# DecaYale/SYN3R

Measured on AMD Instinct MI355X. Metric: llff_3view_train_loop_iters_per_sec, higher is better.
Workload: dtype f32 raster / f16 UNet (f32 accumulate); 1 GPU; LLFF fern-like 3-view block: 50 raster fwd+bwd iters (l1 loss) (200000 Gaussians, 1920x1080, SH3) + 1 SVD (step,pass): CFG UNet fwd [2,14,8,72,128] f16 + fused Euler step; frames=14, parallelism=scene-parallel x1

## Files before the change

include/syn3r_hip.h:

```cpp
#ifndef SYN3R_HIP_H
#define SYN3R_HIP_H

#include <stddef.h>
#include <stdint.h>

#ifdef __cplusplus
extern "C" {
#endif

#define SYN3R_OK 0
#define SYN3R_E_INVALID (-1)
#define SYN3R_E_WORKSPACE (-2)
#define SYN3R_E_HIP (-3)

#define SYN3R_F32 0
#define SYN3R_F16 1

const char* syn3r_last_error(void);
int syn3r_version(void);
const char* syn3r_arch(void);

int syn3r_trace_enable(int on);
void* syn3r_trace_session(void);
int syn3r_trace_attach(void* session);
int syn3r_trace_filter(const char* substrings);
int syn3r_trace_report(char* buf, size_t cap);


size_t syn3r_inverse_warp_workspace_bytes(int nb);
int syn3r_inverse_warp(const float* img, const float* depth, const float* depth_pseudo,
                       const float* pose12, const float* pose21, const float* K, const float* Kinv,
                       float bandwidth, int nb, int H, int W,
                       float* warped_img, float* warped_depth, uint8_t* mask_warp, uint8_t* mask_depth,
                       uint8_t* mask, float* warped_masked_img, uint8_t* mask_inv,
                       uint8_t* mask_depth_strict, uint8_t* mask_reproj, float* soft_mask_reproj,
                       float* reproj_error, void* workspace, size_t workspace_bytes, void* stream);

int syn3r_reproj_error(const float* depth1, const float* depth2, const float* T12, const float* T21,
                       const float* K1, const float* K1inv, const float* K2, int H, int W, float* err,
                       void* stream);

int syn3r_warp_post(const uint8_t* mask_reproj, const float* warped_img, const float* soft_mask_reproj,
                    int n, int H, int W, int h, int w, uint8_t* ero, float* cond_image, float* cond_ori,
                    float* soft, float* masks, float* soft_pool, void* stream);

int syn3r_fuse_uncertainty(const float* cond_ori, const float* gs_images, const float* soft, int n, int H, int W,
                           int h, int w, float* uncertainty, float* cond_image, float* masks, void* stream);

size_t syn3r_forward_warp_workspace_bytes(int H, int W);
int syn3r_forward_warp(const double* frame1, const uint8_t* mask1, const double* depth1, const double* T,
                       const double* K1inv, const double* K2, int H, int W, uint8_t* warped, uint8_t* mask2,
                       double* flow12, void* workspace, size_t workspace_bytes, void* stream);


size_t syn3r_step_workspace_bytes(int F, int C, int h, int w);
int syn3r_step_interp(const void* model_output, int vdtype, const void* sample, int sdtype,
                      const float* cond, const float* mask, const double* lambda_row, float sigma,
                      float dt, float c_out, float denom, float sqrt_sigma, float lr, int compute_grad,
                      void* prev_sample, float* pred_x0, float* grad, int F, int C, int h, int w,
                      void* workspace, size_t workspace_bytes, void* stream);

int syn3r_step_replace(const void* model_output, int vdtype, const void* sample, int sdtype,
                       const float* cond, const float* mask, const double* lambda_row, float sigma,
                       float dt, float c_out, float denom, void* prev_sample, float* pred_x0,
                       int F, int C, int h, int w, void* workspace, size_t workspace_bytes, void* stream);

size_t syn3r_raster_geom_bytes(int N);
size_t syn3r_raster_image_bytes(int H, int W);
size_t syn3r_raster_binning_bytes(long long P);

int syn3r_raster_preprocess(int N, int sh_degree, int sh_coeffs, const float* means3D, const float* scales,
                            const float* rotations, const float* opacities, const float* shs,
                            const float* confidence, float scale_modifier, const float* viewmatrix,
                            const float* projmatrix, const float* campos, float tanfovx, float tanfovy, int H,
                            int W, int* radii, void* geom, size_t geom_bytes, long long* num_rendered_host,
                            void* stream);
int syn3r_raster_preprocess_raw(int N, int sh_degree, int sh_coeffs, const float* means3D, const float* log_scales,
                                const float* raw_rotations, const float* opacity_logits, const float* shs,
                                const float* confidence, float scale_modifier, const float* viewmatrix,
                                const float* projmatrix, const float* campos, float tanfovx, float tanfovy, int H,
                                int W, int* radii, void* geom, size_t geom_bytes, long long* num_rendered_host,
                                void* stream);

int syn3r_raster_render(int N, int H, int W, const float* bg, const int* radii, void* geom, size_t geom_bytes,
                        void* binning, size_t binning_bytes, void* image, size_t image_bytes, long long P,
                        float* out_color, float* out_depth, float* out_alpha, unsigned** point_list_out,
                        void* stream);

size_t syn3r_raster_backward_workspace_bytes(int N);
int syn3r_raster_backward(int N, int sh_degree, int sh_coeffs, long long P, const float* means3D,
                          const float* scales, const float* rotations, const float* opacities, const float* shs,
                          const float* confidence, float scale_modifier, const float* viewmatrix,
                          const float* projmatrix, const float* campos, float tanfovx, float tanfovy, int H, int W,
                          const float* bg, const int* radii, void* geom, size_t geom_bytes,
                          const unsigned* point_list, void* image, size_t image_bytes, const float* dL_dcolor,
                          const float* dL_ddepth, const float* dL_dalpha, float* dL_dmeans3D, float* dL_dscales,
                          float* dL_drotations, float* dL_dopacities, float* dL_dshs, float* dL_dmeans2D,
                          float* dL_dconfidence, void* workspace, size_t workspace_bytes, void* stream);
int syn3r_raster_backward_raw(int N, int sh_degree, int sh_coeffs, long long P, const float* means3D,
                              const float* log_scales, const float* raw_rotations, const float* opacity_logits,
                              const float* shs, const float* confidence, float scale_modifier, const float* viewmatrix,
                              const float* projmatrix, const float* campos, float tanfovx, float tanfovy, int H, int W,
                              const float* bg, const int* radii, void* geom, size_t geom_bytes,
                              const unsigned* point_list, void* image, size_t image_bytes, const float* dL_dcolor,
                              const float* dL_ddepth, const float* dL_dalpha, float* dL_dmeans3D, float* dL_dlog_scales,
                              float* dL_draw_rotations, float* dL_dopacity_logits, float* dL_dshs, float* dL_dmeans2D,
                              float* dL_dconfidence, void* workspace, size_t workspace_bytes, void* stream);

size_t syn3r_sort_pairs_workspace_bytes(long long n);
int syn3r_sort_pairs(unsigned long long* keys, unsigned* vals, unsigned long long* keys_tmp, unsigned* vals_tmp,
                     long long n, int nbits, void* workspace, size_t workspace_bytes, int* result_in_tmp,
                     void* stream);


int syn3r_gemm_f16(const void* A, long long lda, const void* W, void* out, long long ldc, const void* bias,
                   const void* rowvec, long long ldrv, int rows_per_vec, int rv_group_rows, const void* residual, long long ldr,
                   const void* aux, long long ldaux, float s_acc, float s_res, float s_aux, int M, int N, int K,
                   void* gn_partials, size_t gn_partials_bytes, int* gn_written, void* stream);

int syn3r_gemm_2src_supported(int M, int N, int K1, int K2, long long lda1, long long lda2);
int syn3r_gemm_2src_f16(const void* A1, long long lda1, int K1, const void* A2, long long lda2, int K2, const void* W,
                        void* out, long long ldc, const void* bias, int M, int N, void* gn_partials, size_t gn_partials_bytes,
                        int* gn_written, void* stream);

int syn3r_gemm_set_tile(int bm);

int syn3r_gemm_set_splitk_workspace(void* workspace, size_t bytes);

int syn3r_gemm_geglu_f16(const void* A, long long lda, const void* Wpacked, const void* bias_packed, void* out,
                         long long ldc, int M, int D, int K, void* stream);

size_t syn3r_feedforward_workspace_bytes(int M, int D);
int syn3r_feedforward_f16(const void* x, long long ldx, const void* w1_packed, const void* b1_packed, int D,
                          const void* w2, const void* b2, void* out, long long ldc, const void* residual,
                          long long ldr, const void* aux, long long ldaux, float s_acc, float s_res, float s_aux,
                          int M, int C_in, int C_out, void* workspace, size_t workspace_bytes, void* stream);

int syn3r_feedforward_p64_supported(int M, int D, int C_in);
int syn3r_feedforward_p64_f16(const void* x, long long ldx, const void* w1_packed64, const void* b1_packed64, int D,
                              const void* w2, const void* b2, void* out, long long ldc, const void* residual,
                              long long ldr, const void* aux, long long ldaux, float s_acc, float s_res, float s_aux,
                              int M, int C_in, int C_out, void* workspace, size_t workspace_bytes, void* stream);

int syn3r_feedforward_fused_f16(const void* x, long long ldx, const void* w1_chunked, const void* b1_chunked, int D,
                                const void* w2, const void* b2, void* out, long long ldc, const void* residual,
                                long long ldr, const void* aux, long long ldaux, float s_acc, float s_res, float s_aux,
                                int M, int C, void* stream);

int syn3r_feedforward_fused_ln_f16(const void* x, long long ldx, const void* ln_gamma, const void* ln_beta, float ln_eps,
                                   const void* w1_chunked, const void* b1_chunked, int D, const void* w2, const void* b2,
                                   void* out, long long ldc, const void* residual, long long ldr, const void* aux,
                                   long long ldaux, float s_acc, float s_res, float s_aux, int M, int C, void* stream);

int syn3r_feedforward_fused_addln_f16(const void* x, long long ldx, const void* addvec, int rows_per_vec, const void* ln_gamma,
                                      const void* ln_beta, float ln_eps, const void* w1_chunked, const void* b1_chunked, int D,
                                      const void* w2, const void* b2, void* out, long long ldc, const void* aux, long long ldaux,
                                      float s_acc, float s_res, float s_aux, int M, int C, void* stream);

int syn3r_layernorm_linear320_f16(const void* x, long long ldx, const void* ln_gamma, const void* ln_beta, float ln_eps,
                                  const void* W, void* out, long long ldc, int M, int N, int C, void* stream);

int syn3r_conv2d3x3_f16(const void* X, const void* W, void* out, long long ldc, const void* bias,
                        const void* rowvec, long long ldrv, int rows_per_vec, const void* residual, long long ldr,
                        float s_acc, float s_res, int NB, int Hi, int Wi, int Cin, int Cout, int stride, int upsample,
                        int pad_lo, void* gn_partials, size_t gn_partials_bytes, int* gn_written, void* stream);

int syn3r_tconv3_f16(const void* X, const void* W, void* out, long long ldc, const void* bias, const void* rowvec,
                     long long ldrv, int rows_per_vec, const void* residual, long long ldr, float s_acc, float s_res,
                     int B, int F, int HW, int Cin, int Cout, void* gn_partials, size_t gn_partials_bytes, int* gn_written,
                     void* stream);

int syn3r_attention_f16(const void* q, const void* k, const void* v, long long ld, void* out, long long ldo,
                        int nseq, int S, int heads, void* stream);

int syn3r_attention_temporal_f16(const void* q, const void* k, const void* v, long long ld, void* out,
                                 long long ldo, int B, int F, int HW, int heads, void* stream);

size_t syn3r_groupnorm_workspace_bytes(int samples, int rows);
int syn3r_groupnorm_f16(const void* x, void* y, int samples, int rows, int C, const void* gamma, const void* beta,
                        float eps, int silu, void* workspace, size_t workspace_bytes, void* stream);
int syn3r_groupnorm_2src_f16(const void* x1, int C1, const void* x2, int C2, void* y, int samples, int rows,
                             const void* gamma, const void* beta, float eps, int silu, void* workspace,
                             size_t workspace_bytes, void* stream);
size_t syn3r_gn_partials_bytes(int M, int N);
int syn3r_groupnorm_pre_f16(const void* x1, int C1, const void* part1, const void* x2, int C2, const void* part2, void* y,
                            int samples, int rows, const void* gamma, const void* beta, float eps, int silu,
                            void* workspace, size_t workspace_bytes, void* stream);

int syn3r_layernorm_f16(const void* x, void* y, void* xsum, const void* addvec, int rows_per_vec, long long M,
                        int C, const void* gamma, const void* beta, float eps, void* stream);

int syn3r_geglu_f16(const void* x, void* y, long long M, int D, void* stream);

int syn3r_softmax_rows_f16(const void* x, void* y, long long M, int N, long long ld, float scale, void* stream);

int syn3r_time_conv_out(const void* x, long long ldx, const float* w, const float* bias, float* out, int B, int F,
                        long long HW, void* stream);


size_t syn3r_l1_loss_workspace_bytes(long long n);
int syn3r_l1_loss(const float* image, const float* target, long long n, float weight, float* loss, void* ws,
                  size_t ws_bytes, void* stream);
int syn3r_l1_loss_backward(const float* image, const float* target, long long n, float weight,
                           const float* grad_loss, float* grad_image, void* stream);

int syn3r_image_mse(const float* image, const float* target, long long n, float* mse, void* ws, size_t ws_bytes,
                    void* stream);

size_t syn3r_photo_loss_workspace_bytes(int C, int H, int W);
int syn3r_photo_loss(const float* image, const float* target, int C, int H, int W, float lambda_dssim, float weight,
                     float* loss3, void* ws, size_t ws_bytes, void* stream);
int syn3r_photo_loss_backward(const float* image, const float* target, int C, int H, int W, float lambda_dssim,
                              float weight, const float* grad_loss, const void* ws, float* grad_image, void* stream);
int syn3r_photo_loss_step(const float* image, const float* target, int C, int H, int W, float lambda_dssim, float weight,
                          const float* grad_loss, float* loss3, float* grad_image, void* ws, size_t ws_bytes, void* stream);

#define SYN3R_DCORR_MIN 0
#define SYN3R_DCORR_A 1
#define SYN3R_DCORR_B 2
size_t syn3r_depth_corr_loss_workspace_bytes(long long n);
int syn3r_depth_corr_loss(const float* depth, const float* prior, long long n, float weight, float offset, int mode, float* parts,
                          void* ws, size_t ws_bytes, void* stream);
int syn3r_depth_corr_loss_backward(const float* depth, const float* prior, long long n, float weight, float offset, int mode,
                                   const float* grad_loss, const void* ws, size_t ws_bytes, float* grad_depth, void* stream);
int syn3r_depth_corr_loss_step(const float* depth, const float* prior, long long n, float weight, float offset, int mode,
                               const float* grad_loss, float* parts, float* grad_depth, void* ws, size_t ws_bytes, void* stream);

int syn3r_adam_step(float* param, const float* grad, float* exp_avg, float* exp_avg_sq, long long n, float lr,
                    float beta1, float beta2, float eps, int step, void* stream);
int syn3r_adam_step_multi(int count, float* const* params, const float* const* grads, float* const* exp_avgs,
                          float* const* exp_avg_sqs, const long long* numels, const float* lrs, float beta1, float beta2,
                          const float* epss, const int* steps, void* stream);

int syn3r_gaussian_activate(int N, const float* log_scales, const float* rotations, const float* opacity_logits, float* scales,
                            float* rotations_n, float* opacities, void* stream);
int syn3r_gaussian_activate_backward(int N, const float* rotations, const float* scales, const float* rotations_n,
                                     const float* opacities, const float* d_scales, const float* d_rotations_n,
                                     const float* d_opacities, float* d_log_scales, float* d_rotations, float* d_opacity_logits,
                                     void* stream);

int syn3r_densification_stats(int N, const int* radii, const float* viewspace_grad, float* grad_accum, float* denom,
                              float* max_radii, void* stream);

size_t syn3r_knn3_workspace_bytes(int n);
int syn3r_knn3_mean_dist2(const float* points, int n, float* out, void* ws, size_t ws_bytes, void* stream);

size_t syn3r_knn3_graph_workspace_bytes(int n);
int syn3r_knn3_graph(const float* points, int n, float* dist2, int* index, void* ws, size_t ws_bytes, void* stream);

size_t syn3r_gaussian_unpool_workspace_bytes(int n);
int syn3r_gaussian_unpool_count(const float* dist2, const float* log_scales, int n, float score_thresh, float log_scale_thresh,
                                int* count, void* ws, size_t ws_bytes, void* stream);
int syn3r_gaussian_unpool_emit(const float* xyz, const float* log_scales, const float* opacity_logits, const float* confidence,
                               const int* index, int n, int n_sources, int capacity, float* out_xyz, float* out_log_scales,
                               float* out_opacity_logits, float* out_rotations, float* out_confidence, const void* ws,
                               size_t ws_bytes, void* stream);

int syn3r_conv2d3x3_act_f16(const void* X, const void* W, void* out, const void* bias, int relu, const void* relu_mask,
                            int NB, int Hi, int Wi, int Cin, int Cout, void* stream);
int syn3r_lpips_image_f16(const float* img, int H, int W, void* out, void* stream);
int syn3r_lpips_image_bwd(const void* grad64, int H, int W, float loss_scale, float* d_img, void* stream);
int syn3r_maxpool2_f16(const void* x, int H, int W, int C, void* y, void* stream);
int syn3r_maxpool2_bwd_f16(const void* x, const void* gy, int H, int W, int C, void* gx, void* stream);
size_t syn3r_lpips_layer_workspace_bytes(long long P, int C);
int syn3r_lpips_layer_f16(const void* a, const void* b, const float* w, long long P, int C, int accumulate, float* value,
                          void* ws, size_t ws_bytes, void* stream);
int syn3r_lpips_layer_bwd_f16(const void* a, const void* b, const float* w, long long P, int C, float gscale, int accumulate,
                              void* grad_a, void* stream);
int syn3r_conv2d3x3_split_f16(const void* X, const void* W, void* out, long long ld_out, const void* bias, int relu, int split_out,
                              const void* relu_mask, long long ld_mask, int NB, int Hi, int Wi, int Cin, int Cout, void* stream);
int syn3r_lpips_image_split_f16(const float* img, int H, int W, void* out, void* stream);
int syn3r_maxpool2_split_f16(const void* x, int H, int W, int C, void* y, void* stream);
int syn3r_maxpool2_bwd_split_f16(const void* x, const void* gy, int H, int W, int C, void* gx, void* stream);
int syn3r_lpips_layer_split_f16(const void* a, const void* b, const float* w, long long P, int C, int accumulate, float* value,
                                void* ws, size_t ws_bytes, void* stream);
int syn3r_lpips_layer_bwd_split_f16(const void* a, const void* b, const float* w, long long P, int C, float gscale, int accumulate,
                                    void* grad_a, void* stream);

size_t syn3r_pcd_outlier_workspace_bytes(int n);
int syn3r_pcd_statistical_outlier(const double* points, int n, int nb_neighbors, double std_ratio, double* avg_dist,
                                  unsigned char* keep, double* stats, void* ws, size_t ws_bytes, void* stream);

int syn3r_flow_cycle_mask(const float* flow_fw, const float* flow_bw, int n, int H, int W, float thresh, float* mask, float* dist,
                          void* stream);

typedef struct syn3r_unet syn3r_unet;
int syn3r_unet_create(const char* weights_dir, const char* variant, syn3r_unet** out);
int syn3r_unet_destroy(syn3r_unet* unet);
size_t syn3r_unet_workspace_bytes(syn3r_unet* unet, int B, int F, int h, int w, int ehs_rows);
int syn3r_unet_forward(syn3r_unet* unet, const void* sample, double timestep, const void* encoder_hidden_states, int ehs_rows,
                       const float* added_time_ids, void* out, int B, int F, int h, int w, int ctx_group, void* workspace,
                       size_t workspace_bytes, void* stream);

#ifdef __cplusplus
}
#endif
#endif
```

syn3r_amd/_lib.py:

```python
from __future__ import annotations

import ctypes as C
from pathlib import Path

import torch

_LIB_PATH = Path(__file__).resolve().parent / "lib" / "libsyn3r_hip.so"
_lib = None

c_f = C.c_float
c_i = C.c_int
c_p = C.c_void_p
c_sz = C.c_size_t
c_ll = C.c_longlong
c_d = C.c_double

F32, F16 = 0, 1

SIGNATURES = {
    "syn3r_last_error": (C.c_char_p, []),
    "syn3r_version": (c_i, []),
    "syn3r_arch": (C.c_char_p, []),
    "syn3r_trace_enable": (c_i, [c_i]),
    "syn3r_trace_filter": (c_i, [C.c_char_p]),
    "syn3r_trace_report": (c_i, [C.c_char_p, c_sz]),
    "syn3r_trace_session": (c_p, []),
    "syn3r_trace_attach": (c_i, [c_p]),
    "syn3r_inverse_warp_workspace_bytes": (c_sz, [c_i]),
    "syn3r_inverse_warp": (c_i, [c_p, c_p, c_p, c_p, c_p, c_p, c_p, c_f, c_i, c_i, c_i,
                                 c_p, c_p, c_p, c_p, c_p, c_p, c_p, c_p, c_p, c_p, c_p, c_p, c_sz, c_p]),
    "syn3r_reproj_error": (c_i, [c_p, c_p, c_p, c_p, c_p, c_p, c_p, c_i, c_i, c_p, c_p]),
    "syn3r_warp_post": (c_i, [c_p, c_p, c_p, c_i, c_i, c_i, c_i, c_i, c_p, c_p, c_p, c_p, c_p, c_p, c_p]),
    "syn3r_fuse_uncertainty": (c_i, [c_p, c_p, c_p, c_i, c_i, c_i, c_i, c_i, c_p, c_p, c_p, c_p]),
    "syn3r_forward_warp_workspace_bytes": (c_sz, [c_i, c_i]),
    "syn3r_forward_warp": (c_i, [c_p, c_p, c_p, c_p, c_p, c_p, c_i, c_i, c_p, c_p, c_p, c_p, c_sz, c_p]),
    "syn3r_step_workspace_bytes": (c_sz, [c_i, c_i, c_i, c_i]),
    "syn3r_step_interp": (c_i, [c_p, c_i, c_p, c_i, c_p, c_p, c_p, c_f, c_f, c_f, c_f, c_f, c_f, c_i,
                                c_p, c_p, c_p, c_i, c_i, c_i, c_i, c_p, c_sz, c_p]),
    "syn3r_step_replace": (c_i, [c_p, c_i, c_p, c_i, c_p, c_p, c_p, c_f, c_f, c_f, c_f,
                                 c_p, c_p, c_i, c_i, c_i, c_i, c_p, c_sz, c_p]),
    "syn3r_raster_geom_bytes": (c_sz, [c_i]),
    "syn3r_raster_image_bytes": (c_sz, [c_i, c_i]),
    "syn3r_raster_binning_bytes": (c_sz, [c_ll]),
    "syn3r_raster_preprocess": (c_i, [c_i, c_i, c_i, c_p, c_p, c_p, c_p, c_p, c_p, c_f, c_p, c_p, c_p, c_f, c_f,
                                      c_i, c_i, c_p, c_p, c_sz, C.POINTER(c_ll), c_p]),
    "syn3r_raster_preprocess_raw": (c_i, [c_i, c_i, c_i, c_p, c_p, c_p, c_p, c_p, c_p, c_f, c_p, c_p, c_p, c_f, c_f,
                                          c_i, c_i, c_p, c_p, c_sz, C.POINTER(c_ll), c_p]),
    "syn3r_raster_render": (c_i, [c_i, c_i, c_i, c_p, c_p, c_p, c_sz, c_p, c_sz, c_p, c_sz, c_ll, c_p, c_p, c_p,
                                  C.POINTER(c_p), c_p]),
    "syn3r_raster_backward_workspace_bytes": (c_sz, [c_i]),
    "syn3r_raster_backward": (c_i, [c_i, c_i, c_i, c_ll, c_p, c_p, c_p, c_p, c_p, c_p, c_f, c_p, c_p, c_p, c_f, c_f,
                                    c_i, c_i, c_p, c_p, c_p, c_sz, c_p, c_p, c_sz, c_p, c_p, c_p, c_p, c_p, c_p, c_p,
                                    c_p, c_p, c_p, c_p, c_sz, c_p]),
    "syn3r_raster_backward_raw": (c_i, [c_i, c_i, c_i, c_ll, c_p, c_p, c_p, c_p, c_p, c_p, c_f, c_p, c_p, c_p, c_f, c_f,
                                        c_i, c_i, c_p, c_p, c_p, c_sz, c_p, c_p, c_sz, c_p, c_p, c_p, c_p, c_p, c_p, c_p,
                                        c_p, c_p, c_p, c_p, c_sz, c_p]),
    "syn3r_sort_pairs_workspace_bytes": (c_sz, [c_ll]),
    "syn3r_sort_pairs": (c_i, [c_p, c_p, c_p, c_p, c_ll, c_i, c_p, c_sz, C.POINTER(c_i), c_p]),
    "syn3r_gaussian_activate": (c_i, [c_i, c_p, c_p, c_p, c_p, c_p, c_p, c_p]),
    "syn3r_gaussian_activate_backward": (c_i, [c_i, c_p, c_p, c_p, c_p, c_p, c_p, c_p, c_p, c_p, c_p, c_p]),
    "syn3r_densification_stats": (c_i, [c_i, c_p, c_p, c_p, c_p, c_p, c_p]),
    "syn3r_gemm_f16": (c_i, [c_p, c_ll, c_p, c_p, c_ll, c_p, c_p, c_ll, c_i, c_i, c_p, c_ll, c_p, c_ll, c_f, c_f, c_f,
                             c_i, c_i, c_i, c_p, c_sz, C.POINTER(c_i), c_p]),
    "syn3r_gemm_set_tile": (c_i, [c_i]),
    "syn3r_gemm_geglu_f16": (c_i, [c_p, c_ll, c_p, c_p, c_p, c_ll, c_i, c_i, c_i, c_p]),
    "syn3r_feedforward_workspace_bytes": (c_sz, [c_i, c_i]),
    "syn3r_feedforward_f16": (c_i, [c_p, c_ll, c_p, c_p, c_i, c_p, c_p, c_p, c_ll, c_p, c_ll, c_p, c_ll, c_f, c_f, c_f,
                                    c_i, c_i, c_i, c_p, c_sz, c_p]),
    "syn3r_feedforward_p64_f16": (c_i, [c_p, c_ll, c_p, c_p, c_i, c_p, c_p, c_p, c_ll, c_p, c_ll, c_p, c_ll, c_f, c_f, c_f,
                                    c_i, c_i, c_i, c_p, c_sz, c_p]),
    "syn3r_feedforward_p64_supported": (c_i, [c_i, c_i, c_i]),
    "syn3r_feedforward_fused_f16": (c_i, [c_p, c_ll, c_p, c_p, c_i, c_p, c_p, c_p, c_ll, c_p, c_ll, c_p, c_ll, c_f, c_f, c_f,
                                          c_i, c_i, c_p]),
    "syn3r_feedforward_fused_ln_f16": (c_i, [c_p, c_ll, c_p, c_p, c_f, c_p, c_p, c_i, c_p, c_p, c_p, c_ll, c_p, c_ll, c_p, c_ll,
                                             c_f, c_f, c_f, c_i, c_i, c_p]),
    "syn3r_feedforward_fused_addln_f16": (c_i, [c_p, c_ll, c_p, c_i, c_p, c_p, c_f, c_p, c_p, c_i, c_p, c_p, c_p, c_ll, c_p, c_ll,
                                                c_f, c_f, c_f, c_i, c_i, c_p]),
    "syn3r_layernorm_linear320_f16": (c_i, [c_p, c_ll, c_p, c_p, c_f, c_p, c_p, c_ll, c_i, c_i, c_i, c_p]),
    "syn3r_conv2d3x3_f16": (c_i, [c_p, c_p, c_p, c_ll, c_p, c_p, c_ll, c_i, c_p, c_ll, c_f, c_f,
                                  c_i, c_i, c_i, c_i, c_i, c_i, c_i, c_i, c_p, c_sz, C.POINTER(c_i), c_p]),
    "syn3r_tconv3_f16": (c_i, [c_p, c_p, c_p, c_ll, c_p, c_p, c_ll, c_i, c_p, c_ll, c_f, c_f,
                               c_i, c_i, c_i, c_i, c_i, c_p, c_sz, C.POINTER(c_i), c_p]),
    "syn3r_attention_f16": (c_i, [c_p, c_p, c_p, c_ll, c_p, c_ll, c_i, c_i, c_i, c_p]),
    "syn3r_attention_temporal_f16": (c_i, [c_p, c_p, c_p, c_ll, c_p, c_ll, c_i, c_i, c_i, c_i, c_p]),
    "syn3r_groupnorm_workspace_bytes": (c_sz, [c_i, c_i]),
    "syn3r_groupnorm_f16": (c_i, [c_p, c_p, c_i, c_i, c_i, c_p, c_p, c_f, c_i, c_p, c_sz, c_p]),
    "syn3r_groupnorm_2src_f16": (c_i, [c_p, c_i, c_p, c_i, c_p, c_i, c_i, c_p, c_p, c_f, c_i, c_p, c_sz, c_p]),
    "syn3r_groupnorm_pre_f16": (c_i, [c_p, c_i, c_p, c_p, c_i, c_p, c_p, c_i, c_i, c_p, c_p, c_f, c_i, c_p, c_sz, c_p]),
    "syn3r_gn_partials_bytes": (c_sz, [c_i, c_i]),
    "syn3r_gemm_2src_supported": (c_i, [c_i, c_i, c_i, c_i, c_ll, c_ll]),
    "syn3r_gemm_2src_f16": (c_i, [c_p, c_ll, c_i, c_p, c_ll, c_i, c_p, c_p, c_ll, c_p, c_i, c_i, c_p, c_sz, C.POINTER(c_i), c_p]),
    "syn3r_layernorm_f16": (c_i, [c_p, c_p, c_p, c_p, c_i, c_ll, c_i, c_p, c_p, c_f, c_p]),
    "syn3r_geglu_f16": (c_i, [c_p, c_p, c_ll, c_i, c_p]),
    "syn3r_softmax_rows_f16": (c_i, [c_p, c_p, c_ll, c_i, c_ll, c_f, c_p]),
    "syn3r_time_conv_out": (c_i, [c_p, c_ll, c_p, c_p, c_p, c_i, c_i, c_ll, c_p]),
    "syn3r_l1_loss_workspace_bytes": (c_sz, [c_ll]),
    "syn3r_l1_loss": (c_i, [c_p, c_p, c_ll, c_f, c_p, c_p, c_sz, c_p]),
    "syn3r_l1_loss_backward": (c_i, [c_p, c_p, c_ll, c_f, c_p, c_p, c_p]),
    "syn3r_image_mse": (c_i, [c_p, c_p, c_ll, c_p, c_p, c_sz, c_p]),
    "syn3r_photo_loss_workspace_bytes": (c_sz, [c_i, c_i, c_i]),
    "syn3r_photo_loss": (c_i, [c_p, c_p, c_i, c_i, c_i, c_f, c_f, c_p, c_p, c_sz, c_p]),
    "syn3r_photo_loss_backward": (c_i, [c_p, c_p, c_i, c_i, c_i, c_f, c_f, c_p, c_p, c_p, c_p]),
    "syn3r_photo_loss_step": (c_i, [c_p, c_p, c_i, c_i, c_i, c_f, c_f, c_p, c_p, c_p, c_p, c_sz, c_p]),
    "syn3r_depth_corr_loss_workspace_bytes": (c_sz, [c_ll]),
    "syn3r_depth_corr_loss": (c_i, [c_p, c_p, c_ll, c_f, c_f, c_i, c_p, c_p, c_sz, c_p]),
    "syn3r_depth_corr_loss_backward": (c_i, [c_p, c_p, c_ll, c_f, c_f, c_i, c_p, c_p, c_sz, c_p, c_p]),
    "syn3r_depth_corr_loss_step": (c_i, [c_p, c_p, c_ll, c_f, c_f, c_i, c_p, c_p, c_p, c_p, c_sz, c_p]),
    "syn3r_adam_step": (c_i, [c_p, c_p, c_p, c_p, c_ll, c_f, c_f, c_f, c_f, c_i, c_p]),
    "syn3r_adam_step_multi": (c_i, [c_i, c_p, c_p, c_p, c_p, c_p, c_p, c_f, c_f, c_p, c_p, c_p]),
    "syn3r_knn3_workspace_bytes": (c_sz, [c_i]),
    "syn3r_knn3_mean_dist2": (c_i, [c_p, c_i, c_p, c_p, c_sz, c_p]),
    "syn3r_knn3_graph_workspace_bytes": (c_sz, [c_i]),
    "syn3r_knn3_graph": (c_i, [c_p, c_i, c_p, c_p, c_p, c_sz, c_p]),
    "syn3r_gaussian_unpool_workspace_bytes": (c_sz, [c_i]),
    "syn3r_gaussian_unpool_count": (c_i, [c_p, c_p, c_i, c_f, c_f, c_p, c_p, c_sz, c_p]),
    "syn3r_gaussian_unpool_emit": (c_i, [c_p, c_p, c_p, c_p, c_p, c_i, c_i, c_i, c_p, c_p, c_p, c_p, c_p, c_p, c_sz, c_p]),
    "syn3r_conv2d3x3_act_f16": (c_i, [c_p, c_p, c_p, c_p, c_i, c_p, c_i, c_i, c_i, c_i, c_i, c_p]),
    "syn3r_lpips_image_f16": (c_i, [c_p, c_i, c_i, c_p, c_p]),
    "syn3r_lpips_image_bwd": (c_i, [c_p, c_i, c_i, c_f, c_p, c_p]),
    "syn3r_maxpool2_f16": (c_i, [c_p, c_i, c_i, c_i, c_p, c_p]),
    "syn3r_maxpool2_bwd_f16": (c_i, [c_p, c_p, c_i, c_i, c_i, c_p, c_p]),
    "syn3r_lpips_layer_workspace_bytes": (c_sz, [c_ll, c_i]),
    "syn3r_lpips_layer_f16": (c_i, [c_p, c_p, c_p, c_ll, c_i, c_i, c_p, c_p, c_sz, c_p]),
    "syn3r_lpips_layer_bwd_f16": (c_i, [c_p, c_p, c_p, c_ll, c_i, c_f, c_i, c_p, c_p]),
    "syn3r_conv2d3x3_split_f16": (c_i, [c_p, c_p, c_p, c_ll, c_p, c_i, c_i, c_p, c_ll, c_i, c_i, c_i, c_i, c_i, c_p]),
    "syn3r_lpips_image_split_f16": (c_i, [c_p, c_i, c_i, c_p, c_p]),
    "syn3r_maxpool2_split_f16": (c_i, [c_p, c_i, c_i, c_i, c_p, c_p]),
    "syn3r_maxpool2_bwd_split_f16": (c_i, [c_p, c_p, c_i, c_i, c_i, c_p, c_p]),
    "syn3r_lpips_layer_split_f16": (c_i, [c_p, c_p, c_p, c_ll, c_i, c_i, c_p, c_p, c_sz, c_p]),
    "syn3r_lpips_layer_bwd_split_f16": (c_i, [c_p, c_p, c_p, c_ll, c_i, c_f, c_i, c_p, c_p]),
    "syn3r_pcd_outlier_workspace_bytes": (c_sz, [c_i]),
    "syn3r_pcd_statistical_outlier": (c_i, [c_p, c_i, c_i, c_d, c_p, c_p, c_p, c_p, c_sz, c_p]),
    "syn3r_flow_cycle_mask": (c_i, [c_p, c_p, c_i, c_i, c_i, c_f, c_p, c_p, c_p]),
    "syn3r_gemm_set_splitk_workspace": (c_i, [c_p, c_sz]),
    "syn3r_unet_create": (c_i, [C.c_char_p, C.c_char_p, C.POINTER(c_p)]),
    "syn3r_unet_destroy": (c_i, [c_p]),
    "syn3r_unet_workspace_bytes": (c_sz, [c_p, c_i, c_i, c_i, c_i, c_i]),
    "syn3r_unet_forward": (c_i, [c_p, c_p, c_d, c_p, c_i, c_p, c_p, c_i, c_i, c_i, c_i, c_i, c_p, c_sz, c_p]),
}


class Syn3rError(RuntimeError):
    pass


def lib_path() -> Path:
    return _LIB_PATH


def set_library_path(path) -> None:
    global _LIB_PATH
    if _lib is not None:
        raise Syn3rError("set_library_path() after the library was loaded")
    _LIB_PATH = Path(path).resolve()


def load():
    global _lib
    if _lib is not None:
        return _lib
    if not _LIB_PATH.exists():
        raise Syn3rError(
            f"{_LIB_PATH} is missing: build it with `python -m syn3r_amd.build` "
            "(there is no CPU fallback for the SYN3R hot path)")
    lib = C.CDLL(str(_LIB_PATH))
    for name, (res, args) in SIGNATURES.items():
        fn = getattr(lib, name)
        fn.restype = res
        fn.argtypes = args
    _lib = lib
    return lib


def check(rc: int, what: str) -> None:
    if rc != 0:
        msg = load().syn3r_last_error().decode("utf-8", "replace")
        raise Syn3rError(f"{what} failed (code {rc}): {msg}")


def require_gpu(*tensors: torch.Tensor) -> torch.device:
    dev = None
    for t in tensors:
        if t is None:
            continue
        if not t.is_cuda:
            raise Syn3rError("syn3r_amd HIP path needs tensors on a HIP device (no CPU fallback); "
                             f"got a tensor on {t.device}")
        if dev is None:
            dev = t.device
        elif t.device != dev:
            raise Syn3rError(f"tensors on different devices: {dev} vs {t.device}")
    if dev is None:
        raise Syn3rError("no tensors given")
    return dev


def ptr(t: torch.Tensor | None) -> int | None:
    if t is None:
        return None
    if not t.is_contiguous():
        raise Syn3rError("non-contiguous tensor passed to the C-ABI")
    return t.data_ptr()


def stream_ptr(dev: torch.device) -> int:
    return torch.cuda.current_stream(dev).cuda_stream


def dtype_tag(t: torch.Tensor) -> int:
    if t.dtype == torch.float16:
        return F16
    if t.dtype == torch.float32:
        return F32
    raise Syn3rError(f"unsupported dtype {t.dtype}")


def host_f32(values) -> "C.Array":
    flat = [float(v) for v in values]
    return (C.c_float * len(flat))(*flat)


def host_f64(values) -> "C.Array":
    flat = [float(v) for v in values]
    return (C.c_double * len(flat))(*flat)


_ws_cache: dict = {}


def workspace(dev: torch.device, nbytes: int, tag: str = "") -> torch.Tensor:
    key = (dev.index, torch.cuda.current_stream(dev).cuda_stream, tag)
    buf = _ws_cache.get(key)
    if buf is None or buf.numel() < nbytes:
        buf = torch.empty(max(int(nbytes), 256), dtype=torch.uint8, device=dev)
        _ws_cache[key] = buf
    return buf


_active_trace = None


def join_active_trace() -> None:
    load().syn3r_trace_attach(_active_trace)


class kernel_trace:

    def __init__(self, only: str = "", detail: bool = False):
        self.only = only
        self.detail = detail

    def __enter__(self):
        global _active_trace
        lib = load()
        lib.syn3r_trace_filter(self.only.encode())
        lib.syn3r_trace_enable(2 if self.detail else 1)
        _active_trace = lib.syn3r_trace_session()
        self.result = {}
        return self

    def __exit__(self, *exc):
        global _active_trace
        lib = load()
        _active_trace = None
        lib.syn3r_trace_enable(0)
        buf = C.create_string_buffer(1 << 18)
        lib.syn3r_trace_report(buf, len(buf))
        for line in buf.value.decode().splitlines():
            name, calls, ms = line.rsplit(" ", 2)
            self.result[name] = (int(calls), float(ms))
        return False
```

syn3r_amd/csrc/raster_bin.hip:

```cpp
#include "common.h"
#include "raster_common.h"

using namespace syn3r;

namespace syn3r {

size_t binning_bytes(long long P) {
    size_t n = (size_t)(P > 0 ? P : 1);
    return 2 * align256(n * 8) + 2 * align256(n * 4) + sort_scratch_bytes(n) + 256;
}

BinningState carve_binning(void* buf, long long P) {
    size_t n = (size_t)(P > 0 ? P : 1);
    char* p = (char*)buf;
    BinningState b;
    b.keys_a = (unsigned long long*)p; p += align256(n * 8);
    b.keys_b = (unsigned long long*)p; p += align256(n * 8);
    b.vals_a = (unsigned*)p; p += align256(n * 4);
    b.vals_b = (unsigned*)p; p += align256(n * 4);
    b.sort_scratch = p;
    return b;
}

}

namespace {

__global__ void __launch_bounds__(256) k_dup_tiles(int N, const unsigned* __restrict__ order,
                                                   const float* __restrict__ means2D, const int* __restrict__ radii,
                                                   const unsigned* __restrict__ offsets, int gx, int gy,
                                                   unsigned* __restrict__ keys, unsigned* __restrict__ vals,
                                                   unsigned cap, unsigned* __restrict__ header,
                                                   uint2* __restrict__ ranges, int tiles) {
    const int i = blockIdx.x * 256 + threadIdx.x;
    for (int t = i; t < tiles; t += gridDim.x * 256) ranges[t] = make_uint2(0u, 0u);
    const int lane = threadIdx.x & 63;
    const bool valid = i < N;
    unsigned id = valid ? order[i] : 0u;
    int r = valid ? radii[id] : 0;
    int x0 = 0, y0 = 0, x1 = 0, y1 = 0;
    if (r > 0) tile_rect(means2D[2 * (size_t)id], means2D[2 * (size_t)id + 1], r, gx, gy, x0, y0, x1, y1);
    const int w = x1 - x0;
    const unsigned cnt = (unsigned)(w * (y1 - y0));
    const unsigned incl = wave_scan_incl(cnt);
    const unsigned local = incl - cnt;
    const unsigned total = __shfl(incl, 63, 64);
    const int first = blockIdx.x * 256 + (threadIdx.x & ~63);
    const unsigned base = first < N ? offsets[first] : 0u;
    const float inv_w = w > 0 ? 1.0f / (float)w : 0.0f;
    for (unsigned t = 0; t < total; t += 64) {
        const unsigned p = t + lane;
        int j = 0;
#pragma unroll
        for (int step = 32; step > 0; step >>= 1) {
            unsigned lc = __shfl(local, j + step, 64);
            if (lc <= p) j += step;
        }
        const unsigned k = p - __shfl(local, j, 64);
        const int xj = __shfl(x0, j, 64), yj = __shfl(y0, j, 64), wj = __shfl(w, j, 64);
        const float iwj = __shfl(inv_w, j, 64);
        const unsigned idj = __shfl(id, j, 64);
        if (p < total) {
            const int ty = (int)(((float)k + 0.5f) * iwj);
            int tyc = ty;
            if ((unsigned)(tyc * wj) > k) --tyc;
            else if ((unsigned)((tyc + 1) * wj) <= k) ++tyc;
            const int tx = (int)k - tyc * wj;
            const unsigned o = base + p;
            if (o < cap) {
                keys[o] = (unsigned)((yj + tyc) * gx + xj + tx);
                vals[o] = idj;
            } else {
                header[1] = 1u;
            }
        }
    }
}

__global__ void __launch_bounds__(256) k_tile_ranges(long long P_cap, const unsigned* __restrict__ header,
                                                     const unsigned* __restrict__ keys,
                                                     uint2* __restrict__ ranges) {
    long long P = (long long)header[0];
    if (P > P_cap) P = P_cap;
    long long i = (long long)blockIdx.x * 256 + threadIdx.x;
    if (i >= P) return;
    unsigned cur = keys[i];
    if (i == 0) ranges[cur].x = 0;
    else {
        unsigned prev = keys[i - 1];
        if (cur != prev) {
            ranges[prev].y = (unsigned)i;
            ranges[cur].x = (unsigned)i;
        }
    }
    if (i == P - 1) ranges[cur].y = (unsigned)P;
}

constexpr int kBinThreads = 512;
constexpr int kOffThreads = 1024;
#ifndef SYN3R_MAX_SUPER
#define SYN3R_MAX_SUPER 512
#endif
constexpr int kMaxSuper = SYN3R_MAX_SUPER;

struct BinPlan { int ss, sgx, sgy, nsuper, rounds, nchunks; bool ok; };
inline BinPlan bin_plan(int N, int gx, int gy) {
    BinPlan b;
    for (b.ss = 0; b.ss <= 3; ++b.ss) {
        const int side = 1 << b.ss;
        b.sgx = (gx + side - 1) / side; b.sgy = (gy + side - 1) / side;
        b.nsuper = b.sgx * b.sgy;
        if (b.nsuper <= kMaxSuper) break;
    }
    if (b.ss > 3) b.ss = 3;
    b.ok = b.nsuper <= kMaxSuper;
    const int max_chunks = b.ok ? (int)(kBinCounters / (size_t)b.nsuper) : 1;
    const int units = (N + kBinThreads - 1) / kBinThreads;
    b.rounds = (units + max_chunks - 1) / max_chunks;
    if (b.rounds < 1) b.rounds = 1;
    b.nchunks = (units + b.rounds - 1) / b.rounds;
    return b;
}

inline bool hier_binning(int N, int gx, int gy) {
    static const int on = tune_env("SYN3R_BIN_HIER", 1);
    return on != 0 && bin_plan(N, gx, gy).ok;
}

struct BinRect { int x0, y0, x1, y1; };
__device__ __forceinline__ BinRect bin_rect(int i, int N, const float* __restrict__ means2D, const int* __restrict__ radii, int gx, int gy) {
    BinRect r; r.x0 = r.y0 = r.x1 = r.y1 = 0;
    if (i < N) {
        const int rad = radii[i];
        if (rad > 0) tile_rect(means2D[2 * (size_t)i], means2D[2 * (size_t)i + 1], rad, gx, gy, r.x0, r.y0, r.x1, r.y1);
    }
    return r;
}
__device__ __forceinline__ unsigned short clip_rect(const BinRect& q, int sx, int sy, int ss) {
    const int bx = sx << ss, by = sy << ss, side = 1 << ss;
    const int rx0 = max(q.x0 - bx, 0), rx1 = min(q.x1 - bx, side), ry0 = max(q.y0 - by, 0), ry1 = min(q.y1 - by, side);
    return (unsigned short)(rx0 | (rx1 << 4) | (ry0 << 8) | (ry1 << 12));
}

__global__ void __launch_bounds__(kBinThreads) k_super_count(int N, const float* __restrict__ means2D, const int* __restrict__ radii,
                                                             int gx, int gy, int ss, int sgx, int nsuper, int rounds, int nchunks,
                                                             unsigned* __restrict__ counters, unsigned* __restrict__ header) {
    __shared__ unsigned tot[kMaxSuper];
    for (int s = threadIdx.x; s < nsuper; s += kBinThreads) tot[s] = 0u;
    __syncthreads();
    int pairs = 0;
    for (int r = 0; r < rounds; ++r) {
        const int i = (blockIdx.x * rounds + r) * kBinThreads + threadIdx.x;
        const BinRect q = bin_rect(i, N, means2D, radii, gx, gy);
        if (q.x1 > q.x0 && q.y1 > q.y0) {
            pairs += (q.x1 - q.x0) * (q.y1 - q.y0);
            const int side1 = (1 << ss) - 1, sx0 = q.x0 >> ss, sx1 = (q.x1 + side1) >> ss, sy0 = q.y0 >> ss, sy1 = (q.y1 + side1) >> ss;
            for (int sy = sy0; sy < sy1; ++sy)
                for (int sx = sx0; sx < sx1; ++sx) atomicAdd(&tot[sy * sgx + sx], 1u);
        }
    }
    __syncthreads();
    for (int s = threadIdx.x; s < nsuper; s += kBinThreads) counters[(size_t)blockIdx.x * nsuper + s] = tot[s];
    __shared__ unsigned pairs_s;
    if (threadIdx.x == 0) pairs_s = 0u;
    __syncthreads();
    pairs = wave_sum_i(pairs);
    if ((threadIdx.x & 63) == 0 && pairs) atomicAdd(&pairs_s, (unsigned)pairs);
    __syncthreads();
    if (threadIdx.x == 0 && pairs_s) atomicAdd(&header[3], pairs_s);
}

__global__ void __launch_bounds__(kBinThreads) k_super_append(int N, const float* __restrict__ depths, const float* __restrict__ means2D,
                                                              const int* __restrict__ radii, int gx, int gy, int ss, int sgx, int nsuper,
                                                              int rounds, int nchunks, const unsigned* __restrict__ counters,
                                                              unsigned* __restrict__ sstart, unsigned cap,
                                                              unsigned long long* __restrict__ skeys, unsigned* __restrict__ header) {
    __shared__ unsigned run[kMaxSuper];
    __shared__ unsigned tot_s[kMaxSuper], pre_s[kMaxSuper];
    __shared__ unsigned part_tot[kMaxSuper > kBinThreads ? kMaxSuper : kBinThreads], part_pre[kMaxSuper > kBinThreads ? kMaxSuper : kBinThreads];
    const int lane = threadIdx.x & 63, wv = threadIdx.x >> 6;
    {
        const int PARTS = max(1, min(8, kBinThreads / nsuper));
        const int per = (nchunks + PARTS - 1) / PARTS;
        for (int w = threadIdx.x; w < nsuper * PARTS; w += kBinThreads) {
            const int s_ = w % nsuper, part = w / nsuper;
            const int c0 = part * per, c1 = min(nchunks, c0 + per);
            unsigned tot = 0, pre = 0;
            constexpr int UN = 32;
            for (int cb = c0; cb < c1; cb += UN) {
                unsigned c[UN];
#pragma unroll
                for (int u = 0; u < UN; ++u) c[u] = cb + u < c1 ? counters[(size_t)(cb + u) * nsuper + s_] : 0u;
#pragma unroll
                for (int u = 0; u < UN; ++u) { tot += c[u]; pre += cb + u < (int)blockIdx.x ? c[u] : 0u; }
            }
            part_tot[w] = tot; part_pre[w] = pre;
        }
        __syncthreads();
        for (int s_ = threadIdx.x; s_ < nsuper; s_ += kBinThreads) {
            unsigned tot = 0, pre = 0;
            for (int k = 0; k < PARTS; ++k) { tot += part_tot[k * nsuper + s_]; pre += part_pre[k * nsuper + s_]; }
            tot_s[s_] = tot; pre_s[s_] = pre;
        }
        __syncthreads();
        if (wv == 0) {
            constexpr int PER = kMaxSuper / 64;
            unsigned c[PER], sum = 0;
#pragma unroll
            for (int k = 0; k < PER; ++k) { const int s_ = lane * PER + k; c[k] = s_ < nsuper ? tot_s[s_] : 0u; sum += c[k]; }
            const unsigned incl = wave_scan_incl(sum);
            unsigned ex = incl - sum;
#pragma unroll
            for (int k = 0; k < PER; ++k) {
                const int s_ = lane * PER + k;
                if (s_ < nsuper) {
                    run[s_] = ex + pre_s[s_];
                    if (blockIdx.x == 0) sstart[s_] = ex;
                }
                ex += c[k];
            }
            if (blockIdx.x == 0 && lane == 63) { sstart[nsuper] = incl; header[2] = incl; }
        }
        __syncthreads();
    }
    for (int r = 0; r < rounds; ++r) {
        const int i = (blockIdx.x * rounds + r) * kBinThreads + threadIdx.x;
        const BinRect q = bin_rect(i, N, means2D, radii, gx, gy);
        if (q.x1 > q.x0 && q.y1 > q.y0) {
            const unsigned long long key = ((unsigned long long)__float_as_uint(depths[i]) << 32) | (unsigned)i;
            const int side1 = (1 << ss) - 1, sx0 = q.x0 >> ss, sx1 = (q.x1 + side1) >> ss, sy0 = q.y0 >> ss, sy1 = (q.y1 + side1) >> ss;
            for (int sy = sy0; sy < sy1; ++sy)
                for (int sx = sx0; sx < sx1; ++sx) {
                    const unsigned o = atomicAdd(&run[sy * sgx + sx], 1u);
                    if (o < cap) skeys[o] = key;
                    else header[1] = 1u;
                }
        }
    }
}

__device__ __forceinline__ void super_range(int s, const unsigned* __restrict__ sstart, unsigned cap, unsigned& b, unsigned& e) {
    b = min(sstart[s], cap); e = min(sstart[s + 1], cap);
}

constexpr int kSortLds = 4096;
constexpr int kSuperSortThreads = 1024;
__device__ __forceinline__ void cmpx(unsigned long long& a, unsigned long long& b) { if (a > b) { const unsigned long long t = a; a = b; b = t; } }
__device__ __forceinline__ int pair_lo(int t, int j) { return (t << 1) - (t & (j - 1)); }
__device__ __forceinline__ void bitonic_dists(unsigned long long* buf, int m, int j) {
    for (; j >= 2; j >>= 2) {
        const int jh = j >> 1;
        for (int t = threadIdx.x; t < (m >> 2); t += kSuperSortThreads) {
            const int e0 = pair_lo(pair_lo(t, jh), j);
            unsigned long long a = buf[e0], b = buf[e0 + jh], c = buf[e0 + j], d = buf[e0 + j + jh];
            cmpx(a, c); cmpx(b, d);
            cmpx(a, b); cmpx(c, d);
            buf[e0] = a; buf[e0 + jh] = b; buf[e0 + j] = c; buf[e0 + j + jh] = d;
        }
        __syncthreads();
    }
    if (j == 1) {
        for (int t = threadIdx.x; t < (m >> 1); t += kSuperSortThreads) cmpx(buf[2 * t], buf[2 * t + 1]);
        __syncthreads();
    }
}
__device__ __forceinline__ void bitonic_merge(unsigned long long* buf, int m, int k) {
    if (k == 2) {
        for (int t = threadIdx.x; t < (m >> 1); t += kSuperSortThreads) cmpx(buf[2 * t], buf[2 * t + 1]);
        __syncthreads();
        return;
    }
    const int q = k >> 2;
    for (int t = threadIdx.x; t < (m >> 2); t += kSuperSortThreads) {
        const int off = t & (q - 1), blk = (t - off) << 2;
        const int ia = blk + off, ib = ia + q, ird = blk + (k - 1 - off), irc = ird - q;
        unsigned long long a = buf[ia], b = buf[ib], c = buf[irc], d = buf[ird];
        cmpx(a, d); cmpx(b, c);
        cmpx(a, b); cmpx(c, d);
        buf[ia] = a; buf[ib] = b; buf[irc] = c; buf[ird] = d;
    }
    __syncthreads();
    bitonic_dists(buf, m, q >> 1);
}

__device__ __forceinline__ bool rect_has(unsigned r, int rx, int ry) {
    return rx >= (int)(r & 15u) && rx < (int)((r >> 4) & 15u) && ry >= (int)((r >> 8) & 15u) && ry < (int)(r >> 12);
}

constexpr int kBinUnroll = 8;
__device__ __forceinline__ void tile_quarter(unsigned b, unsigned e, int q, unsigned& qb, unsigned& qe) {
    const unsigned len = (e - b + 3u) / 4u;
    qb = min(e, b + (unsigned)q * len); qe = min(e, qb + len);
}

__device__ __forceinline__ void super_tile_counts(int sx, int sy, int ss, int gx, int gy, unsigned n, const unsigned short* srect_b,
                                                  unsigned* __restrict__ tcount) {
    const int lane = threadIdx.x & 63, wv = threadIdx.x >> 6, side = 1 << ss;
    const unsigned len = (n + 3u) / 4u;
    for (int it = wv; it < side * side * 4; it += kSuperSortThreads / 64) {
        const int ti = it >> 2, q = it & 3;
        const int rx = ti & (side - 1), ry = ti >> ss;
        const int tx = (sx << ss) + rx, ty = (sy << ss) + ry;
        if (tx >= gx || ty >= gy) continue;
        const unsigned lo = min(n, (unsigned)q * len), hi = min(n, lo + len);
        unsigned cnt = 0;
        for (unsigned i0 = lo; i0 < hi; i0 += 256) {
            unsigned short r[4];
#pragma unroll
            for (int u = 0; u < 4; ++u) r[u] = srect_b[min(i0 + u * 64 + lane, hi - 1u)];
#pragma unroll
            for (int u = 0; u < 4; ++u) cnt += (i0 + u * 64 + lane < hi && rect_has(r[u], rx, ry)) ? 1u : 0u;
        }
#pragma unroll
        for (int o = 32; o > 0; o >>= 1) cnt += __shfl_xor(cnt, o, 64);
        if (lane == 0) tcount[4 * ((size_t)ty * gx + tx) + q] = cnt;
    }
}

__global__ void __launch_bounds__(kSuperSortThreads, 8) k_super_sort(int N, const float* __restrict__ means2D, const int* __restrict__ radii,
                                                                  int gx, int gy, int ss, int sgx, const unsigned* __restrict__ sstart, unsigned cap,
                                                                  unsigned long long* __restrict__ skeys, unsigned* __restrict__ sid,
                                                                  unsigned short* __restrict__ srect, unsigned* __restrict__ tcount) {
    extern __shared__ __attribute__((aligned(16))) unsigned long long sk[];
    const int s_ = blockIdx.x, sx = s_ % sgx, sy = s_ / sgx;
    unsigned b, e;
    super_range(s_, sstart, cap, b, e);
    const int n = (int)(e - b);
    if (n == 0) { super_tile_counts(sx, sy, ss, gx, gy, 0u, srect, tcount); return; }
    unsigned long long* gk = skeys + b;
    const unsigned long long INF = ~0ull;
    int m = 1;
    while (m < n) m <<= 1;
    const unsigned long long* sorted;
    if (m <= kSortLds) {
        for (int i = threadIdx.x; i < m; i += kSuperSortThreads) sk[i] = i < n ? gk[i] : INF;
        __syncthreads();
        for (int k = 2; k <= m; k <<= 1) bitonic_merge(sk, m, k);
        sorted = sk;
    } else {
        for (int p0 = 0; p0 < n; p0 += kSortLds) {
            for (int i = threadIdx.x; i < kSortLds; i += kSuperSortThreads) sk[i] = p0 + i < n ? gk[p0 + i] : INF;
            __syncthreads();
            for (int k = 2; k <= kSortLds; k <<= 1) bitonic_merge(sk, kSortLds, k);
            for (int i = threadIdx.x; i < kSortLds; i += kSuperSortThreads) if (p0 + i < n) gk[p0 + i] = sk[i];
            __syncthreads();
        }
        for (int k = kSortLds << 1; k <= m; k <<= 1) {
            const int h = k >> 1;
            for (int t = threadIdx.x; t < (m >> 1); t += kSuperSortThreads) {
                const int off = t & (h - 1), l = pair_lo(t, h), r = l - off + (k - 1 - off);
                if (r < n) { unsigned long long a = gk[l], c = gk[r]; if (a > c) { gk[l] = c; gk[r] = a; } }
            }
            __syncthreads();
            for (int j = k >> 2; j >= kSortLds; j >>= 1) {
                for (int t = threadIdx.x; t < (m >> 1); t += kSuperSortThreads) {
                    const int l = pair_lo(t, j), r = l + j;
                    if (r < n) { unsigned long long a = gk[l], c = gk[r]; if (a > c) { gk[l] = c; gk[r] = a; } }
                }
                __syncthreads();
            }
            for (int p0 = 0; p0 < n; p0 += kSortLds) {
                for (int i = threadIdx.x; i < kSortLds; i += kSuperSortThreads) sk[i] = p0 + i < n ? gk[p0 + i] : INF;
                __syncthreads();
                bitonic_dists(sk, kSortLds, kSortLds >> 1);
                for (int i = threadIdx.x; i < kSortLds; i += kSuperSortThreads) if (p0 + i < n) gk[p0 + i] = sk[i];
                __syncthreads();
            }
        }
        sorted = gk;
    }
    if (sorted == sk) {
        unsigned short clip[kSortLds / kSuperSortThreads];
#pragma unroll
        for (int u = 0; u < kSortLds / kSuperSortThreads; ++u) {
            const int i = threadIdx.x + u * kSuperSortThreads;
            clip[u] = 0;
            if (i < n) {
                const unsigned id = (unsigned)sk[i];
                const BinRect q = bin_rect((int)id, N, means2D, radii, gx, gy);
                clip[u] = clip_rect(q, sx, sy, ss);
                sid[b + i] = id;
                srect[b + i] = clip[u];
            }
        }
        __syncthreads();
        unsigned short* sr = (unsigned short*)sk;
#pragma unroll
        for (int u = 0; u < kSortLds / kSuperSortThreads; ++u) {
            const int i = threadIdx.x + u * kSuperSortThreads;
            if (i < n) sr[i] = clip[u];
        }
        __syncthreads();
        super_tile_counts(sx, sy, ss, gx, gy, (unsigned)n, sr, tcount);
        return;
    }
    for (int i = threadIdx.x; i < n; i += kSuperSortThreads) {
        const unsigned id = (unsigned)sorted[i];
        const BinRect q = bin_rect((int)id, N, means2D, radii, gx, gy);
        sid[b + i] = id;
        srect[b + i] = clip_rect(q, sx, sy, ss);
    }
    __syncthreads();
    super_tile_counts(sx, sy, ss, gx, gy, (unsigned)n, srect + b, tcount);
}

__global__ void __launch_bounds__(kOffThreads) k_tile_offsets(int tiles, const unsigned* __restrict__ tcount, unsigned cap,
                                                              uint2* __restrict__ ranges, unsigned* __restrict__ header,
                                                              unsigned* __restrict__ tile_order) {
    __shared__ unsigned smem[kOffThreads / 64 + 1];
    __shared__ unsigned bh[256];
    if (tile_order) { for (int k = threadIdx.x; k < 256; k += kOffThreads) bh[k] = 0u; __syncthreads(); }
    constexpr int PER = 8;
    unsigned carry = 0;
    for (int start = 0; start < tiles; start += kOffThreads * PER) {
        const int t0 = start + threadIdx.x * PER;
        unsigned c[PER], sum = 0;
#pragma unroll
        for (int k = 0; k < PER; ++k) {
            c[k] = 0u;
            if (t0 + k < tiles) { const uint4 q4 = ((const uint4*)tcount)[t0 + k]; c[k] = (q4.x + q4.y) + (q4.z + q4.w); }
            sum += c[k];
        }
        unsigned total;
        unsigned ex = block_exclusive_scan<kOffThreads / 64>(sum, smem, total) + carry;
#pragma unroll
        for (int k = 0; k < PER; ++k) {
            if (t0 + k < tiles) ranges[t0 + k] = c[k] ? make_uint2(min(ex, cap), min(ex + c[k], cap)) : make_uint2(0u, 0u);
            if (tile_order && t0 + k < tiles) atomicAdd(&bh[255u - min(255u, c[k] >> 5)], 1u);
            ex += c[k];
        }
        carry += total;
    }
    if (tile_order) {
        __syncthreads();
        if (threadIdx.x < 64) {
            const int l = threadIdx.x;
            unsigned c[4], sum = 0;
#pragma unroll
            for (int k = 0; k < 4; ++k) { c[k] = bh[4 * l + k]; sum += c[k]; }
            unsigned ex = wave_scan_incl(sum) - sum;
#pragma unroll
            for (int k = 0; k < 4; ++k) { bh[4 * l + k] = ex; ex += c[k]; }
        }
        __syncthreads();
        for (int t = threadIdx.x; t < tiles; t += kOffThreads) {
            const uint4 q4 = ((const uint4*)tcount)[t];
            const unsigned c = (q4.x + q4.y) + (q4.z + q4.w);
            tile_order[atomicAdd(&bh[255u - min(255u, c >> 5)], 1u)] = (unsigned)t;
        }
    }
    if (threadIdx.x == 0) {
        const bool over = carry > cap || header[2] > cap;
        header[0] = over ? max(carry, max(header[3], header[2])) : carry;
        if (over) header[1] = 1u;
    }
}

__global__ void __launch_bounds__(256) k_tile_write(int gx, int tiles, int ss, int sgx, const unsigned* __restrict__ sstart, unsigned cap,
                                                    const unsigned* __restrict__ sid, const unsigned short* __restrict__ srect,
                                                    const uint2* __restrict__ ranges, const unsigned* __restrict__ tcount,
                                                    unsigned* __restrict__ point_list) {
    const int t = blockIdx.x, q = threadIdx.x >> 6, lane = threadIdx.x & 63;
    const int tx = t % gx, ty = t / gx;
    unsigned b, e;
    super_range((ty >> ss) * sgx + (tx >> ss), sstart, cap, b, e);
    tile_quarter(b, e, q, b, e);
    const int rx = tx & ((1 << ss) - 1), ry = ty & ((1 << ss) - 1);
    const unsigned long long lt = (1ull << lane) - 1ull;
    const uint4 q4 = ((const uint4*)tcount)[t];
    unsigned pos = ranges[t].x + (q > 0 ? q4.x : 0u) + (q > 1 ? q4.y : 0u) + (q > 2 ? q4.z : 0u);
    for (unsigned i0 = b; i0 < e; i0 += 64 * kBinUnroll) {
        unsigned short r[kBinUnroll];
        unsigned id[kBinUnroll];
#pragma unroll
        for (int u = 0; u < kBinUnroll; ++u) {
            const unsigned i = i0 + u * 64 + lane;
            r[u] = i < e ? srect[i] : (unsigned short)0;
            id[u] = i < e ? sid[i] : 0u;
        }
#pragma unroll
        for (int u = 0; u < kBinUnroll; ++u) {
            const bool hit = rect_has(r[u], rx, ry);
            const unsigned long long m = __ballot(hit);
            if (hit) {
                const unsigned o = pos + (unsigned)__popcll(m & lt);
                if (o < cap) point_list[o] = id[u];
            }
            pos += (unsigned)__popcll(m);
        }
    }
}

int bits_for(unsigned v) { int b = 0; while (v) { ++b; v >>= 1; } return b; }

}

namespace syn3r {

bool raster_tiles_ordered(int N, int gx, int gy) {
    static const int order_env = tune_env("SYN3R_TILE_ORDER", 1);
    return order_env != 0 && hier_binning(N, gx, gy);
}

int raster_bin_prepare(const GeomState& g, int N, int gx, int gy, bool want_count, hipStream_t stream) {
    if (!hier_binning(N, gx, gy)) {
        int in_b = 0;
        int rc = argsort_depth_u32(g.dkeys_a, g.order_a, g.dkeys_b, g.order_b, (size_t)N, g.sort_scratch, stream, &in_b);
        if (rc) return rc;
        if ((in_b ? g.order_b : g.order_a) != g.order) { set_error("raster_preprocess: unexpected argsort parity"); return SYN3R_E_INVALID; }
        return exclusive_scan_u32(g.tiles_touched, g.point_offsets, (size_t)N, g.header, g.scan_scratch, stream, g.order);
    }
    if (want_count) return exclusive_scan_u32(g.tiles_touched, g.point_offsets, (size_t)N, g.header, g.scan_scratch, stream);
    return SYN3R_OK;
}

int raster_bin_lists(const GeomState& g, const ImageState& im, const BinningState& bn, const int* radii, int N, int gx, int gy,
                     long long P, hipStream_t stream, unsigned** point_list_out, const unsigned** tile_order_out) {
    const size_t tiles = (size_t)gx * gy;
    unsigned* point_list = bn.vals_a;
    unsigned* tile_order = nullptr;
    if (P == 0) {
        if (int rc = check_hip(hipMemsetAsync(im.ranges, 0, tiles * 8, stream), "memset ranges")) return rc;
    } else if (hier_binning(N, gx, gy)) {
        SYN3R_REQUIRE(P < (1ll << 30), "raster_render: pair capacity %lld: the super-tile sort indexes a list with 31-bit integers (2^30 pairs at most)", P);
        const BinPlan bp = bin_plan(N, gx, gy);
        unsigned* counters = im.bin_counters;
        unsigned* sid = bn.vals_b;
        unsigned short* srect = (unsigned short*)bn.keys_a;
        unsigned* sstart = counters + kBinCounters;
        unsigned long long* skeys = bn.keys_b;
        static DevOnce once;
        if (int rc = set_max_lds(once, (const void*)k_super_sort, kSortLds * 8, "hipFuncSetAttribute(super_sort)")) return rc;
        SYN3R_LAUNCH(k_super_count, dim3(bp.nchunks), dim3(kBinThreads), 0, stream, N, (const float*)g.means2D, radii, gx, gy, bp.ss, bp.sgx,
                     bp.nsuper, bp.rounds, bp.nchunks, counters, g.header);
        SYN3R_LAUNCH(k_super_append, dim3(bp.nchunks), dim3(kBinThreads), 0, stream, N, (const float*)g.depths, (const float*)g.means2D, radii,
                     gx, gy, bp.ss, bp.sgx, bp.nsuper, bp.rounds, bp.nchunks, (const unsigned*)counters, sstart, (unsigned)P, skeys, g.header);
        SYN3R_LAUNCH(k_super_sort, dim3(bp.nsuper), dim3(kSuperSortThreads), kSortLds * 8, stream, N, (const float*)g.means2D, radii, gx, gy,
                     bp.ss, bp.sgx, (const unsigned*)sstart, (unsigned)P, skeys, sid, srect, im.tile_counts);
        if (raster_tiles_ordered(N, gx, gy)) tile_order = im.tile_order;
        SYN3R_LAUNCH(k_tile_offsets, dim3(1), dim3(kOffThreads), 0, stream, (int)tiles, (const unsigned*)im.tile_counts, (unsigned)P,
                     im.ranges, g.header, tile_order);
        SYN3R_LAUNCH(k_tile_write, dim3((unsigned)tiles), dim3(256), 0, stream, gx, (int)tiles, bp.ss, bp.sgx,
                     (const unsigned*)sstart, (unsigned)P, (const unsigned*)sid, (const unsigned short*)srect,
                     (const uint2*)im.ranges, (const unsigned*)im.tile_counts, point_list);
    } else {
        unsigned* tk_a = (unsigned*)bn.keys_a;
        unsigned* tk_b = (unsigned*)bn.keys_b;
        SYN3R_LAUNCH(k_dup_tiles, dim3(ceil_div(N, 256)), dim3(256), 0, stream, N, g.order, g.means2D, radii,
                           g.point_offsets, gx, gy, tk_a, bn.vals_a, (unsigned)P, g.header, im.ranges, (int)tiles);
        int in_b = 0;
        int rc = sort_pairs_by_tile_u32(tk_a, bn.vals_a, tk_b, bn.vals_b, (size_t)P, bits_for((unsigned)tiles - 1),
                                        bn.sort_scratch, stream, &in_b, g.header);
        if (rc) return rc;
        const unsigned* keys = in_b ? tk_b : tk_a;
        point_list = in_b ? bn.vals_b : bn.vals_a;
        SYN3R_LAUNCH(k_tile_ranges, dim3(ceil_div(P, 256)), dim3(256), 0, stream, P, g.header, keys, im.ranges);
    }
    *point_list_out = point_list;
    *tile_order_out = tile_order;
    return SYN3R_OK;
}

}
```

syn3r_amd/csrc/raster_common.h:

```cpp
#pragma once
#include <hip/hip_runtime.h>
#include <stdint.h>
#include <stddef.h>

namespace syn3r {

constexpr int kTileX = 16;
constexpr int kTileY = 16;
constexpr int kTilePix = kTileX * kTileY;
constexpr float kNearClip = 0.2f;
constexpr float kFovGuard = 1.3f;
constexpr float kLowPass = 0.3f;
constexpr float kAlphaMin = 1.0f / 255.0f;
constexpr float kAlphaMax = 0.99f;
constexpr float kTransmittanceMin = 1e-4f;
constexpr float kLog2e = 1.4426950408889634f;

struct alignas(16) Splat {
    float x, y;
    float cxx, cxy, cyy;
    float opacity;
    float r, g, b;
    float depth;
    float pad0, pad1;
};
static_assert(sizeof(Splat) == 48, "Splat must be 48 bytes");

struct GeomState {
    unsigned* header;
    float* depths;
    float* means2D;
    float* cov3D;
    float* conic_opacity;
    float* rgb;
    unsigned* clamped;
    unsigned* tiles_touched;
    unsigned* point_offsets;
    Splat* splats;
    unsigned* dkeys_a;
    unsigned* dkeys_b;
    unsigned* order_a;
    unsigned* order_b;
    unsigned* order;
    void* sort_scratch;
    void* scan_scratch;
};

#ifndef SYN3R_BIN_COUNTERS
#define SYN3R_BIN_COUNTERS 65536
#endif
constexpr size_t kBinCounters = SYN3R_BIN_COUNTERS;
constexpr size_t kMaxSuperSlots = 4096;
struct ImageState {
    uint2* ranges;
    unsigned* n_contrib;
    float* final_T;
    unsigned* tile_counts;
    unsigned* bin_counters;
    unsigned* tile_order;
};

struct BinningState {
    unsigned long long* keys_a;
    unsigned long long* keys_b;
    unsigned* vals_a;
    unsigned* vals_b;
    void* sort_scratch;
};

inline size_t align256(size_t x) { return (x + 255) & ~(size_t)255; }

size_t scan_scratch_bytes(size_t n);
size_t sort_scratch_bytes(size_t n);
int exclusive_scan_u32(const unsigned* in, unsigned* out, size_t n, unsigned* total_out, void* scratch,
                       hipStream_t stream, const unsigned* perm = nullptr);
int argsort_depth_u32(unsigned* keys_a, unsigned* vals_a, unsigned* keys_b, unsigned* vals_b, size_t n, void* scratch,
                      hipStream_t stream, int* result_in_b);
int sort_pairs_by_tile_u32(unsigned* keys_a, unsigned* vals_a, unsigned* keys_b, unsigned* vals_b, size_t n, int nbits,
                           void* scratch, hipStream_t stream, int* result_in_b, const unsigned* n_dev);
int radix_sort_pairs(unsigned long long* keys_a, unsigned* vals_a, unsigned long long* keys_b, unsigned* vals_b,
                     size_t n, int nbits, void* scratch, hipStream_t stream, int* result_in_b,
                     const unsigned* n_dev = nullptr);

struct Camera {
    float view[16];
    float proj[16];
    float campos[3];
    float tanfovx, tanfovy, focal_x, focal_y;
    int H, W, grid_x, grid_y;
};

size_t geom_bytes(int N);
bool raster_tiles_ordered(int N, int gx, int gy);
size_t image_bytes(int H, int W);
size_t binning_bytes(long long P);
GeomState carve_geom(void* buf, int N);
void raster_fill_camera(Camera& cam, const float* view, const float* proj, const float* campos, float tanfovx, float tanfovy, int H, int W);
ImageState carve_image(void* buf, int H, int W);
BinningState carve_binning(void* buf, long long P);

int raster_bin_prepare(const GeomState& g, int N, int gx, int gy, bool want_count, hipStream_t stream);
int raster_bin_lists(const GeomState& g, const ImageState& im, const BinningState& bn, const int* radii, int N, int gx, int gy,
                     long long P, hipStream_t stream, unsigned** point_list, const unsigned** tile_order);

#ifdef __HIPCC__
__device__ __forceinline__ bool splat_reaches_rect(float mx, float my, float A, float B, float C, float op, float x0,
                                                   float x1, float y0, float y1) {
    if (!(A > 0.0f && C > 0.0f)) return true;
    const float thr = 2.0f * __logf(255.0f * op);
    const float dx0 = x0 - mx, dx1 = x1 - mx, dy0 = y0 - my, dy1 = y1 - my;
    const bool inx = dx0 <= 0.0f && dx1 >= 0.0f, iny = dy0 <= 0.0f && dy1 >= 0.0f;
    float qmin = 0.0f;
    if (!(inx && iny)) {
        qmin = 3.0e38f;
        if (!inx) {
            const float dx = dx0 > 0.0f ? dx0 : dx1;
            const float dy = fminf(fmaxf(-B * dx / C, dy0), dy1);
            qmin = A * dx * dx + 2.0f * B * dx * dy + C * dy * dy;
        }
        if (!iny) {
            const float dy = dy0 > 0.0f ? dy0 : dy1;
            const float dx = fminf(fmaxf(-B * dy / A, dx0), dx1);
            qmin = fminf(qmin, A * dx * dx + 2.0f * B * dx * dy + C * dy * dy);
        }
    }
    return qmin <= thr + (1.0e-3f + 1.0e-4f * thr);
}

__device__ __forceinline__ void tile_rect(float px, float py, int radius, int gx, int gy, int& x0, int& y0, int& x1,
                                          int& y1) {
    x0 = min(gx, max(0, (int)((px - radius) / kTileX)));
    y0 = min(gy, max(0, (int)((py - radius) / kTileY)));
    x1 = min(gx, max(0, (int)((px + radius + kTileX - 1) / kTileX)));
    y1 = min(gy, max(0, (int)((py + radius + kTileY - 1) / kTileY)));
}

typedef float f2 __attribute__((ext_vector_type(2)));
__device__ __forceinline__ f2 splat2(float s) { return (f2){s, s}; }
constexpr int kBlendThreads = 128;
struct BlendFrame {
    int px, py0, py1;
    bool in0, in1;
    float fx;
    f2 fy;
};
struct BlendHalf { float sx0, sx1, sy0, sy1; };
__device__ __forceinline__ BlendFrame blend_frame(unsigned tile, int wq, int lane, int H, int W, int gx) {
    const int tx = tile % gx, ty = tile / gx;
    const int lx = lane & 15, ly = wq * 8 + (lane >> 4);
    BlendFrame f;
    f.px = tx * kTileX + lx; f.py0 = ty * kTileY + ly; f.py1 = f.py0 + 4;
    f.in0 = f.px < W && f.py0 < H; f.in1 = f.px < W && f.py1 < H;
    f.fx = (float)f.px;
    f.fy = (f2){(float)f.py0, (float)f.py1};
    return f;
}
__device__ __forceinline__ BlendHalf blend_half(unsigned tile, int wq, int gx) {
    const int tx = tile % gx, ty = tile / gx;
    BlendHalf h;
    h.sx0 = (float)(tx * kTileX); h.sx1 = h.sx0 + 15.0f;
    h.sy0 = (float)(ty * kTileY + wq * 8); h.sy1 = h.sy0 + 7.0f;
    return h;
}
__device__ __forceinline__ void stage_splat(float4* sm, int slot, const float4& n0, const float4& n1, const float4& n2) {
    sm[slot * 3 + 0] = n0;
    sm[slot * 3 + 1] = n1;
    sm[slot * 3 + 2] = n2;
}
struct BlendEval { float dx; f2 dy, power, G; };
__device__ __forceinline__ BlendEval blend_eval(const float4& a, const float4& b, const BlendFrame& f) {
    BlendEval e;
    e.dx = a.x - f.fx;
    e.dy = splat2(a.y) - f.fy;
    const float hxx = -0.5f * a.z * e.dx * e.dx, bxy = a.w * e.dx;
    e.power = (-0.5f * b.x) * e.dy * e.dy - bxy * e.dy + hxx;
    const f2 pl = e.power * kLog2e;
    e.G = (f2){__builtin_amdgcn_exp2f(pl.x), __builtin_amdgcn_exp2f(pl.y)};
    return e;
}

constexpr float SH_C0 = 0.28209479177387814f;
constexpr float SH_C1 = 0.4886025119029199f;
static __constant__ float SH_C2[5] = {1.0925484305920792f, -1.0925484305920792f, 0.31539156525252005f,
                                      -1.0925484305920792f, 0.5462742152960396f};
static __constant__ float SH_C3[7] = {-0.5900435899266435f, 2.890611442640554f, -0.4570457994644658f, 0.3731763325901154f,
                                      -0.4570457994644658f, 1.445305721320277f, -0.5900435899266435f};
struct Rot3 { float R00, R01, R02, R10, R11, R12, R20, R21, R22; };
__device__ __forceinline__ Rot3 quat_rotation(float4 q) {
    const float qr = q.x, qx = q.y, qy = q.z, qz = q.w;
    Rot3 o;
    o.R00 = 1.f - 2.f * (qy * qy + qz * qz); o.R01 = 2.f * (qx * qy - qr * qz); o.R02 = 2.f * (qx * qz + qr * qy);
    o.R10 = 2.f * (qx * qy + qr * qz); o.R11 = 1.f - 2.f * (qx * qx + qz * qz); o.R12 = 2.f * (qy * qz - qr * qx);
    o.R20 = 2.f * (qx * qz - qr * qy); o.R21 = 2.f * (qy * qz + qr * qx); o.R22 = 1.f - 2.f * (qx * qx + qy * qy);
    return o;
}
struct EwaRows { float tx, ty, T00, T01, T02, T10, T11, T12; };
__device__ __forceinline__ EwaRows ewa_rows(const Camera& cam, float t_x, float t_y, float t_z) {
    const float limx = kFovGuard * cam.tanfovx, limy = kFovGuard * cam.tanfovy;
    EwaRows o;
    o.tx = fminf(limx, fmaxf(-limx, t_x / t_z)) * t_z;
    o.ty = fminf(limy, fmaxf(-limy, t_y / t_z)) * t_z;
    const float J00 = cam.focal_x / t_z, J02 = -(cam.focal_x * o.tx) / (t_z * t_z);
    const float J11 = cam.focal_y / t_z, J12 = -(cam.focal_y * o.ty) / (t_z * t_z);
    const float* v = cam.view;
    o.T00 = J00 * v[0] + J02 * v[2]; o.T01 = J00 * v[4] + J02 * v[6]; o.T02 = J00 * v[8] + J02 * v[10];
    o.T10 = J11 * v[1] + J12 * v[2]; o.T11 = J11 * v[5] + J12 * v[6]; o.T12 = J11 * v[9] + J12 * v[10];
    return o;
}

#ifdef SYN3R_RASTER_STATS
#define RASTER_STAT(arr, i, n) do { if (lane == 0) atomicAdd(&arr[i], (unsigned long long)(n)); } while (0)
#else
#define RASTER_STAT(arr, i, n)
#endif
#endif

}
```

syn3r_amd/csrc/raster_fwd.hip:

```cpp
#include "common.h"
#include "raster_common.h"

using namespace syn3r;

namespace syn3r {

size_t geom_bytes(int N) {
    size_t n = (size_t)N;
    size_t b = 256;
    b += align256(n * 4);
    b += align256(n * 8);
    b += align256(n * 24);
    b += align256(n * 16);
    b += align256(n * 12);
    b += align256(n * 4);
    b += align256(n * 4);
    b += align256(n * 4);
    b += align256(n * sizeof(Splat));
    b += 4 * align256(n * 4);
    b += align256(sort_scratch_bytes(n));
    b += scan_scratch_bytes(n);
    return b;
}

GeomState carve_geom(void* buf, int N) {
    size_t n = (size_t)N;
    char* p = (char*)buf;
    GeomState g;
    g.header = (unsigned*)p; p += 256;
    g.depths = (float*)p; p += align256(n * 4);
    g.means2D = (float*)p; p += align256(n * 8);
    g.cov3D = (float*)p; p += align256(n * 24);
    g.conic_opacity = (float*)p; p += align256(n * 16);
    g.rgb = (float*)p; p += align256(n * 12);
    g.clamped = (unsigned*)p; p += align256(n * 4);
    g.tiles_touched = (unsigned*)p; p += align256(n * 4);
    g.point_offsets = (unsigned*)p; p += align256(n * 4);
    g.splats = (Splat*)p; p += align256(n * sizeof(Splat));
    g.dkeys_a = (unsigned*)p; p += align256(n * 4);
    g.dkeys_b = (unsigned*)p; p += align256(n * 4);
    g.order_a = (unsigned*)p; p += align256(n * 4);
    g.order_b = (unsigned*)p; p += align256(n * 4);
    g.order = g.order_a;
    g.sort_scratch = p; p += align256(sort_scratch_bytes(n));
    g.scan_scratch = p;
    return g;
}

size_t image_bytes(int H, int W) {
    size_t tiles = (size_t)((W + kTileX - 1) / kTileX) * ((H + kTileY - 1) / kTileY);
    size_t px = (size_t)H * W;
    return align256(tiles * 8) + align256(px * 4) + align256(px * 4) + align256(tiles * 16) + align256((kBinCounters + kMaxSuperSlots) * 4) + align256(tiles * 4);
}

ImageState carve_image(void* buf, int H, int W) {
    size_t tiles = (size_t)((W + kTileX - 1) / kTileX) * ((H + kTileY - 1) / kTileY);
    size_t px = (size_t)H * W;
    char* p = (char*)buf;
    ImageState s;
    s.ranges = (uint2*)p; p += align256(tiles * 8);
    s.n_contrib = (unsigned*)p; p += align256(px * 4);
    s.final_T = (float*)p; p += align256(px * 4);
    s.tile_counts = (unsigned*)p; p += align256(tiles * 16);
    s.bin_counters = (unsigned*)p; p += align256((kBinCounters + kMaxSuperSlots) * 4);
    s.tile_order = (unsigned*)p;
    return s;
}


}

namespace {

__device__ __forceinline__ float3 xf43(const float* m, float3 p) {
    return make_float3(m[0] * p.x + m[4] * p.y + m[8] * p.z + m[12], m[1] * p.x + m[5] * p.y + m[9] * p.z + m[13],
                       m[2] * p.x + m[6] * p.y + m[10] * p.z + m[14]);
}
__device__ __forceinline__ float4 xf44(const float* m, float3 p) {
    return make_float4(m[0] * p.x + m[4] * p.y + m[8] * p.z + m[12], m[1] * p.x + m[5] * p.y + m[9] * p.z + m[13],
                       m[2] * p.x + m[6] * p.y + m[10] * p.z + m[14], m[3] * p.x + m[7] * p.y + m[11] * p.z + m[15]);
}

__device__ __forceinline__ float ndc2pix(float v, int S) { return ((v + 1.0f) * (float)S - 1.0f) * 0.5f; }

__device__ float3 sh_to_rgb(int D, int M, float3 pos, const float* campos, const float* __restrict__ sh,
                            unsigned& clamped) {
    float3 dir = make_float3(pos.x - campos[0], pos.y - campos[1], pos.z - campos[2]);
    float inv = 1.0f / sqrtf(dir.x * dir.x + dir.y * dir.y + dir.z * dir.z);
    dir.x *= inv; dir.y *= inv; dir.z *= inv;
    auto c = [&](int k) { return make_float3(sh[3 * k], sh[3 * k + 1], sh[3 * k + 2]); };
    auto mad = [](float3& a, float s, float3 b) { a.x += s * b.x; a.y += s * b.y; a.z += s * b.z; };
    float3 res = make_float3(0, 0, 0);
    mad(res, SH_C0, c(0));
    if (D > 0) {
        float x = dir.x, y = dir.y, z = dir.z;
        mad(res, -SH_C1 * y, c(1));
        mad(res, SH_C1 * z, c(2));
        mad(res, -SH_C1 * x, c(3));
        if (D > 1) {
            float xx = x * x, yy = y * y, zz = z * z, xy = x * y, yz = y * z, xz = x * z;
            mad(res, SH_C2[0] * xy, c(4));
            mad(res, SH_C2[1] * yz, c(5));
            mad(res, SH_C2[2] * (2.0f * zz - xx - yy), c(6));
            mad(res, SH_C2[3] * xz, c(7));
            mad(res, SH_C2[4] * (xx - yy), c(8));
            if (D > 2) {
                mad(res, SH_C3[0] * y * (3.0f * xx - yy), c(9));
                mad(res, SH_C3[1] * xy * z, c(10));
                mad(res, SH_C3[2] * y * (4.0f * zz - xx - yy), c(11));
                mad(res, SH_C3[3] * z * (2.0f * zz - 3.0f * xx - 3.0f * yy), c(12));
                mad(res, SH_C3[4] * x * (4.0f * zz - xx - yy), c(13));
                mad(res, SH_C3[5] * z * (xx - yy), c(14));
                mad(res, SH_C3[6] * x * (xx - 3.0f * yy), c(15));
            }
        }
    }
    res.x += 0.5f; res.y += 0.5f; res.z += 0.5f;
    clamped = (res.x < 0.0f ? 1u : 0u) | (res.y < 0.0f ? 2u : 0u) | (res.z < 0.0f ? 4u : 0u);
    return make_float3(fmaxf(res.x, 0.0f), fmaxf(res.y, 0.0f), fmaxf(res.z, 0.0f));
}

__global__ void __launch_bounds__(256) k_preprocess(int N, int D, int M, const float* __restrict__ means3D,
                                                    const float* __restrict__ scales,
                                                    const float* __restrict__ rots,
                                                    const float* __restrict__ opacities,
                                                    const float* __restrict__ shs, const float* __restrict__ conf,
                                                    float scale_mod, Camera cam, int* __restrict__ radii,
                                                    GeomState g, int raw) {
    int i = blockIdx.x * 256 + threadIdx.x;
    if (i >= N) return;
    if (i < 4) g.header[i] = 0u;
    radii[i] = 0;
    g.tiles_touched[i] = 0;
    g.dkeys_a[i] = 0xFFFFFFFFu;
    float3 p = make_float3(means3D[3 * i], means3D[3 * i + 1], means3D[3 * i + 2]);
    float3 t = xf43(cam.view, p);
    if (t.z <= kNearClip) return;
    float4 ph = xf44(cam.proj, p);
    float pw = 1.0f / (ph.w + 0.0000001f);
    float ndcx = ph.x * pw, ndcy = ph.y * pw;

    float s0 = scales[3 * i], s1 = scales[3 * i + 1], s2 = scales[3 * i + 2];
    float4 q4 = make_float4(rots[4 * i], rots[4 * i + 1], rots[4 * i + 2], rots[4 * i + 3]);
    if (raw) {
        s0 = act_exp(s0); s1 = act_exp(s1); s2 = act_exp(s2);
        q4 = act_quat(q4, act_quat_inv_norm(q4));
    }
    float sx = scale_mod * s0, sy = scale_mod * s1, sz = scale_mod * s2;
    const Rot3 k = quat_rotation(q4);
    float m00 = k.R00 * sx, m01 = k.R01 * sy, m02 = k.R02 * sz;
    float m10 = k.R10 * sx, m11 = k.R11 * sy, m12 = k.R12 * sz;
    float m20 = k.R20 * sx, m21 = k.R21 * sy, m22 = k.R22 * sz;
    float c0 = m00 * m00 + m01 * m01 + m02 * m02;
    float c1 = m00 * m10 + m01 * m11 + m02 * m12;
    float c2 = m00 * m20 + m01 * m21 + m02 * m22;
    float c3 = m10 * m10 + m11 * m11 + m12 * m12;
    float c4 = m10 * m20 + m11 * m21 + m12 * m22;
    float c5 = m20 * m20 + m21 * m21 + m22 * m22;
    float* cv = g.cov3D + 6 * (size_t)i;
    cv[0] = c0; cv[1] = c1; cv[2] = c2; cv[3] = c3; cv[4] = c4; cv[5] = c5;

    const EwaRows w = ewa_rows(cam, t.x, t.y, t.z);
    const float T00 = w.T00, T01 = w.T01, T02 = w.T02, T10 = w.T10, T11 = w.T11, T12 = w.T12;
    float a0 = c0 * T00 + c1 * T01 + c2 * T02, a1 = c1 * T00 + c3 * T01 + c4 * T02, a2 = c2 * T00 + c4 * T01 + c5 * T02;
    float b0 = c0 * T10 + c1 * T11 + c2 * T12, b1 = c1 * T10 + c3 * T11 + c4 * T12, b2 = c2 * T10 + c4 * T11 + c5 * T12;
    float cxx = T00 * a0 + T01 * a1 + T02 * a2 + kLowPass;
    float cxy = T00 * b0 + T01 * b1 + T02 * b2;
    float cyy = T10 * b0 + T11 * b1 + T12 * b2 + kLowPass;

    float det = cxx * cyy - cxy * cxy;
    if (det == 0.0f) return;
    float det_inv = 1.0f / det;
    float conx = cyy * det_inv, cony = -cxy * det_inv, conz = cxx * det_inv;
    float mid = 0.5f * (cxx + cyy);
    float sq = sqrtf(fmaxf(0.1f, mid * mid - det));
    float lambda1 = mid + sq, lambda2 = mid - sq;
    int radius = (int)ceilf(3.0f * sqrtf(fmaxf(lambda1, lambda2)));
    float px = ndc2pix(ndcx, cam.W), py = ndc2pix(ndcy, cam.H);
    int x0, y0, x1, y1;
    tile_rect(px, py, radius, cam.grid_x, cam.grid_y, x0, y0, x1, y1);
    int area = (x1 - x0) * (y1 - y0);
    if (area == 0) return;

    unsigned cl;
    float3 rgb = sh_to_rgb(D, M, p, cam.campos, shs + (size_t)i * M * 3, cl);
    float op = raw ? act_sigmoid(opacities[i]) : opacities[i];
    float cf = conf ? conf[i] : 1.0f;
    g.depths[i] = t.z;
    g.dkeys_a[i] = __float_as_uint(t.z);
    radii[i] = radius;
    g.means2D[2 * (size_t)i] = px;
    g.means2D[2 * (size_t)i + 1] = py;
    float* co = g.conic_opacity + 4 * (size_t)i;
    co[0] = conx; co[1] = cony; co[2] = conz; co[3] = op;
    g.rgb[3 * (size_t)i] = rgb.x; g.rgb[3 * (size_t)i + 1] = rgb.y; g.rgb[3 * (size_t)i + 2] = rgb.z;
    g.clamped[i] = cl;
    g.tiles_touched[i] = (unsigned)area;
    Splat s;
    s.x = px; s.y = py; s.cxx = conx; s.cxy = cony; s.cyy = conz; s.opacity = op * cf;
    s.r = rgb.x; s.g = rgb.y; s.b = rgb.z; s.depth = t.z; s.pad0 = 0.f; s.pad1 = 0.f;
    g.splats[i] = s;
}

constexpr int kFwdThreads = kBlendThreads;
#ifdef SYN3R_RASTER_STATS
__device__ unsigned long long g_fwd_stats[4];
#endif

__global__ void __launch_bounds__(kFwdThreads) k_render(int H, int W, int gx, int gy, const uint2* __restrict__ ranges,
                                                        const unsigned* __restrict__ point_list,
                                                        const Splat* __restrict__ splats, float bg0, float bg1,
                                                        float bg2, unsigned* __restrict__ n_contrib,
                                                        float* __restrict__ final_T, float* __restrict__ out_color,
                                                        float* __restrict__ out_depth, float* __restrict__ out_alpha,
                                                        const unsigned* __restrict__ tile_order) {
    __shared__ float4 sm[kFwdThreads * 3];
    const unsigned tile = tile_order ? tile_order[blockIdx.x] : xcd_remap(blockIdx.x, (unsigned)(gx * gy));
    const int wq = threadIdx.x >> 6, lane = threadIdx.x & 63;
    const BlendFrame f = blend_frame(tile, wq, lane, H, W, gx);
    const uint2 range = ranges[tile];
    const int total = (int)(range.y - range.x);
    const int rounds = (total + kFwdThreads - 1) / kFwdThreads;

    bool done0 = !f.in0, done1 = !f.in1;
    f2 T = (f2){1.0f, 1.0f}, Cr = (f2){0.f, 0.f}, Cg = Cr, Cb = Cr, Dp = Cr;
    unsigned last0 = 0, last1 = 0;
    int todo = total;
    const BlendHalf hf = blend_half(tile, wq, gx);
    float4 n0, n1, n2;
    bool have = false;
    auto fetch = [&](int rd) {
        const int idx = rd * kFwdThreads + threadIdx.x;
        have = idx < total;
        if (have) {
            const float4* src = (const float4*)(splats + point_list[range.x + idx]);
            n0 = src[0]; n1 = src[1]; n2 = src[2];
        }
    };
    fetch(0);
    for (int rd = 0; rd < rounds; ++rd, todo -= kFwdThreads) {
        if (__syncthreads_count(done0 && done1) == kFwdThreads) break;
        if (have) stage_splat(sm, threadIdx.x, n0, n1, n2);
        fetch(rd + 1);
        __syncthreads();
        const int cnt = min(kFwdThreads, todo);
        for (int c0 = 0; c0 < cnt; c0 += 64) {
            if (__ballot(!(done0 && done1)) == 0ull) break;
            bool hit = false;
            if (c0 + lane < cnt) {
                const float4 a = sm[(c0 + lane) * 3], b = sm[(c0 + lane) * 3 + 1];
                hit = splat_reaches_rect(a.x, a.y, a.z, a.w, b.x, b.y, hf.sx0, hf.sx1, hf.sy0, hf.sy1);
            }
            unsigned long long m = __ballot(hit);
            RASTER_STAT(g_fwd_stats, 0, min(64, cnt - c0));
            RASTER_STAT(g_fwd_stats, 1, __popcll(m));
            while (m) {
                const int j = c0 + (int)__builtin_ctzll(m);
                m &= m - 1;
                const float4 a = sm[j * 3], b = sm[j * 3 + 1], c = sm[j * 3 + 2];
                const BlendEval e = blend_eval(a, b, f);
                const f2 power = e.power, araw = b.y * e.G;
                const float al0 = fminf(kAlphaMax, araw.x), al1 = fminf(kAlphaMax, araw.y);
                const f2 w_raw = (f2){al0, al1} * T;
                const f2 test_T = T - w_raw;
                const bool c0_ = !done0 && power.x <= 0.0f && al0 >= kAlphaMin;
                const bool c1_ = !done1 && power.y <= 0.0f && al1 >= kAlphaMin;
                if (c0_ && test_T.x < kTransmittanceMin) done0 = true;
                if (c1_ && test_T.y < kTransmittanceMin) done1 = true;
                const bool t0 = c0_ && !done0, t1 = c1_ && !done1;
#ifdef SYN3R_RASTER_STATS
                { unsigned long long b0 = __ballot(t0), b1 = __ballot(t1); RASTER_STAT(g_fwd_stats, 2, (b0 | b1) != 0ull); RASTER_STAT(g_fwd_stats, 3, __popcll(b0) + __popcll(b1)); }
#endif
                const f2 w = (f2){t0 ? w_raw.x : 0.0f, t1 ? w_raw.y : 0.0f};
                Cr += b.z * w; Cg += b.w * w; Cb += c.x * w; Dp += c.y * w;
                T -= w;
                const unsigned here = (unsigned)(rd * kFwdThreads + j + 1);
                last0 = t0 ? here : last0;
                last1 = t1 ? here : last1;
            }
        }
    }
    const size_t hw = (size_t)H * W;
    if (f.in0) {
        const size_t pix = (size_t)f.py0 * W + f.px;
        final_T[pix] = T.x;
        n_contrib[pix] = last0;
        out_color[pix] = Cr.x + T.x * bg0;
        out_color[hw + pix] = Cg.x + T.x * bg1;
        out_color[2 * hw + pix] = Cb.x + T.x * bg2;
        out_depth[pix] = Dp.x;
        out_alpha[pix] = 1.0f - T.x;
    }
    if (f.in1) {
        const size_t pix = (size_t)f.py1 * W + f.px;
        final_T[pix] = T.y;
        n_contrib[pix] = last1;
        out_color[pix] = Cr.y + T.y * bg0;
        out_color[hw + pix] = Cg.y + T.y * bg1;
        out_color[2 * hw + pix] = Cb.y + T.y * bg2;
        out_depth[pix] = Dp.y;
        out_alpha[pix] = 1.0f - T.y;
    }
}

}

namespace syn3r {
void raster_fill_camera(Camera& cam, const float* view, const float* proj, const float* campos, float tanfovx,
                        float tanfovy, int H, int W) {
    for (int i = 0; i < 16; ++i) { cam.view[i] = view[i]; cam.proj[i] = proj[i]; }
    for (int i = 0; i < 3; ++i) cam.campos[i] = campos[i];
    cam.tanfovx = tanfovx; cam.tanfovy = tanfovy;
    cam.focal_x = W / (2.0f * tanfovx);
    cam.focal_y = H / (2.0f * tanfovy);
    cam.H = H; cam.W = W;
    cam.grid_x = (W + kTileX - 1) / kTileX;
    cam.grid_y = (H + kTileY - 1) / kTileY;
}
}

extern "C" size_t syn3r_raster_geom_bytes(int N) { return SYN3R_DIM_OK(N) ? geom_bytes(N) : 0; }
extern "C" size_t syn3r_raster_image_bytes(int H, int W) { return (SYN3R_SIDE_OK(H) && SYN3R_SIDE_OK(W)) ? image_bytes(H, W) : 0; }
extern "C" size_t syn3r_raster_binning_bytes(long long P) { return P >= 0 ? binning_bytes(P) : 0; }

static int raster_preprocess(int raw, int N, int sh_degree, int sh_coeffs, const float* means3D,
                             const float* scales, const float* rotations, const float* opacities,
                             const float* shs, const float* confidence, float scale_modifier,
                             const float* viewmatrix, const float* projmatrix, const float* campos,
                             float tanfovx, float tanfovy, int H, int W, int* radii, void* geom,
                             size_t geom_bytes_, long long* num_rendered_host, void* stream_) {
    SYN3R_REQUIRE(SYN3R_DIM_OK(N) && SYN3R_SIDE_OK(H) && SYN3R_SIDE_OK(W), "raster_preprocess: bad sizes N=%d H=%d W=%d", N, H, W);
    SYN3R_REQUIRE(sh_degree >= 0 && sh_degree <= 3, "raster_preprocess: sh_degree %d not in 0..3", sh_degree);
    SYN3R_REQUIRE(sh_coeffs >= (sh_degree + 1) * (sh_degree + 1) && sh_coeffs <= 1024,
                  "raster_preprocess: sh_degree %d needs >= %d coefficients, got %d", sh_degree,
                  (sh_degree + 1) * (sh_degree + 1), sh_coeffs);
    SYN3R_REQUIRE(means3D && scales && rotations && opacities && shs && viewmatrix && projmatrix && campos && radii,
                  "raster_preprocess: null argument");
    SYN3R_REQUIRE(tanfovx > 0 && tanfovy > 0, "raster_preprocess: bad field of view");
    if (!geom || geom_bytes_ < geom_bytes(N)) {
        set_error("raster_preprocess: geometry buffer %zu < %zu", geom_bytes_, geom_bytes(N));
        return SYN3R_E_WORKSPACE;
    }
    hipStream_t stream = (hipStream_t)stream_;
    GeomState g = carve_geom(geom, N);
    Camera cam;
    raster_fill_camera(cam, viewmatrix, projmatrix, campos, tanfovx, tanfovy, H, W);
    SYN3R_LAUNCH(k_preprocess, dim3(ceil_div(N, 256)), dim3(256), 0, stream, N, sh_degree, sh_coeffs, means3D,
                       scales, rotations, opacities, shs, confidence, scale_modifier, cam, radii, g, raw);
    int rc = raster_bin_prepare(g, N, cam.grid_x, cam.grid_y, num_rendered_host != nullptr, stream);
    if (rc) return rc;
    SYN3R_LAUNCH_CHECK("raster_preprocess launch");
    if (num_rendered_host) {
        unsigned total = 0;
        rc = check_hip(hipMemcpyAsync(&total, g.header, 4, hipMemcpyDeviceToHost, stream), "num_rendered copy");
        if (rc) return rc;
        rc = check_hip(hipStreamSynchronize(stream), "num_rendered sync");
        if (rc) return rc;
        *num_rendered_host = (long long)total;
    }
    return SYN3R_OK;
}

extern "C" int syn3r_raster_preprocess(int N, int sh_degree, int sh_coeffs, const float* means3D,
                                       const float* scales, const float* rotations, const float* opacities,
                                       const float* shs, const float* confidence, float scale_modifier,
                                       const float* viewmatrix, const float* projmatrix, const float* campos,
                                       float tanfovx, float tanfovy, int H, int W, int* radii, void* geom,
                                       size_t geom_bytes_, long long* num_rendered_host, void* stream_) {
    return raster_preprocess(0, N, sh_degree, sh_coeffs, means3D, scales, rotations, opacities, shs, confidence, scale_modifier,
                             viewmatrix, projmatrix, campos, tanfovx, tanfovy, H, W, radii, geom, geom_bytes_, num_rendered_host,
                             stream_);
}

extern "C" int syn3r_raster_preprocess_raw(int N, int sh_degree, int sh_coeffs, const float* means3D,
                                           const float* log_scales, const float* raw_rotations, const float* opacity_logits,
                                           const float* shs, const float* confidence, float scale_modifier,
                                           const float* viewmatrix, const float* projmatrix, const float* campos,
                                           float tanfovx, float tanfovy, int H, int W, int* radii, void* geom,
                                           size_t geom_bytes_, long long* num_rendered_host, void* stream_) {
    return raster_preprocess(1, N, sh_degree, sh_coeffs, means3D, log_scales, raw_rotations, opacity_logits, shs, confidence,
                             scale_modifier, viewmatrix, projmatrix, campos, tanfovx, tanfovy, H, W, radii, geom, geom_bytes_,
                             num_rendered_host, stream_);
}

extern "C" int syn3r_raster_render(int N, int H, int W, const float* bg, const int* radii, void* geom,
                                   size_t geom_bytes_, void* binning, size_t binning_bytes_, void* image,
                                   size_t image_bytes_, long long P, float* out_color, float* out_depth,
                                   float* out_alpha, unsigned** point_list_out, void* stream_) {
    SYN3R_REQUIRE(N > 0 && H > 0 && W > 0 && P >= 0 && P < (1ll << 31), "raster_render: bad sizes N=%d H=%d W=%d P=%lld",
                  N, H, W, P);
    SYN3R_REQUIRE(bg && radii && out_color && out_depth && out_alpha, "raster_render: null argument");
    if (!geom || geom_bytes_ < geom_bytes(N) || !image || image_bytes_ < image_bytes(H, W) || !binning ||
        binning_bytes_ < binning_bytes(P)) {
        set_error("raster_render: state buffer too small (geom %zu/%zu image %zu/%zu binning %zu/%zu)", geom_bytes_,
                  geom_bytes(N), image_bytes_, image_bytes(H, W), binning_bytes_, binning_bytes(P));
        return SYN3R_E_WORKSPACE;
    }
    hipStream_t stream = (hipStream_t)stream_;
    GeomState g = carve_geom(geom, N);
    ImageState im = carve_image(image, H, W);
    BinningState bn = carve_binning(binning, P);
    const int gx = (W + kTileX - 1) / kTileX, gy = (H + kTileY - 1) / kTileY;
    const size_t tiles = (size_t)gx * gy;
    unsigned* point_list = nullptr;
    const unsigned* tile_order = nullptr;
    if (int rc = raster_bin_lists(g, im, bn, radii, N, gx, gy, P, stream, &point_list, &tile_order)) return rc;
    SYN3R_LAUNCH(k_render, dim3((unsigned)tiles), dim3(kFwdThreads), 0, stream, H, W, gx, gy, im.ranges, point_list,
                       g.splats, bg[0], bg[1], bg[2], im.n_contrib, im.final_T, out_color, out_depth, out_alpha, tile_order);
    SYN3R_LAUNCH_CHECK("raster_render launch");
    if (point_list_out) *point_list_out = point_list;
    return SYN3R_OK;
}

#ifdef SYN3R_RASTER_STATS
extern "C" __attribute__((visibility("default"))) int syn3r_debug_fwd_stats(unsigned long long* out4, int reset) {
    int rc = (int)hipMemcpyFromSymbol(out4, HIP_SYMBOL(g_fwd_stats), sizeof(unsigned long long) * 4);
    if (reset) { unsigned long long z[4] = {0, 0, 0, 0}; rc |= (int)hipMemcpyToSymbol(HIP_SYMBOL(g_fwd_stats), z, sizeof(z)); }
    return rc;
}
#endif
```

syn3r_amd/csrc/train.hip:

```cpp
#include "common.h"

using namespace syn3r;

namespace {

constexpr int kThreads = 256;
constexpr int kMaxBlocks = 2048;

template <bool SQ>
__device__ __forceinline__ float dist_term(float d) { return SQ ? d * d : fabsf(d); }

template <bool SQ>
__global__ void __launch_bounds__(kThreads) k_l1_partial(const float* __restrict__ a, const float* __restrict__ b,
                                                        long long n, float* __restrict__ partial) {
    float s = 0.0f;
    const long long n4 = n >> 2;
    const float4* a4 = (const float4*)a;
    const float4* b4 = (const float4*)b;
    for (long long i = (long long)blockIdx.x * kThreads + threadIdx.x; i < n4; i += (long long)gridDim.x * kThreads) {
        float4 x = a4[i], y = b4[i];
        s += (dist_term<SQ>(x.x - y.x) + dist_term<SQ>(x.y - y.y)) + (dist_term<SQ>(x.z - y.z) + dist_term<SQ>(x.w - y.w));
    }
    if (blockIdx.x == 0) {
        long long i = (n4 << 2) + threadIdx.x;
        if (i < n) s += dist_term<SQ>(a[i] - b[i]);
    }
    s = wave_sum(s);
    __shared__ float ws[kThreads / 64];
    if ((threadIdx.x & 63) == 0) ws[threadIdx.x >> 6] = s;
    __syncthreads();
    if (threadIdx.x == 0) partial[blockIdx.x] = (ws[0] + ws[1]) + (ws[2] + ws[3]);
}

__global__ void __launch_bounds__(kThreads) k_l1_final(const float* __restrict__ partial, int nblocks, float scale,
                                                      float* __restrict__ loss) {
    double s = 0.0;
    for (int i = threadIdx.x; i < nblocks; i += kThreads) s += (double)partial[i];
    s = wave_sum_d(s);
    __shared__ double ws[kThreads / 64];
    if ((threadIdx.x & 63) == 0) ws[threadIdx.x >> 6] = s;
    __syncthreads();
    if (threadIdx.x == 0) *loss = (float)(((ws[0] + ws[1]) + (ws[2] + ws[3])) * (double)scale);
}

__global__ void __launch_bounds__(kThreads) k_l1_grad(const float* __restrict__ a, const float* __restrict__ b,
                                                     long long n, float scale, const float* __restrict__ go,
                                                     float* __restrict__ grad) {
    const float g = scale * (go ? *go : 1.0f);
    auto sgn = [g](float d) { return d > 0.0f ? g : (d < 0.0f ? -g : 0.0f); };
    const long long n4 = n >> 2;
    const float4* a4 = (const float4*)a;
    const float4* b4 = (const float4*)b;
    float4* g4 = (float4*)grad;
    for (long long i = (long long)blockIdx.x * kThreads + threadIdx.x; i < n4; i += (long long)gridDim.x * kThreads) {
        float4 x = a4[i], y = b4[i];
        g4[i] = make_float4(sgn(x.x - y.x), sgn(x.y - y.y), sgn(x.z - y.z), sgn(x.w - y.w));
    }
    if (blockIdx.x == 0) {
        long long i = (n4 << 2) + threadIdx.x;
        if (i < n) grad[i] = sgn(a[i] - b[i]);
    }
}

__global__ void __launch_bounds__(kThreads) k_adam(float* __restrict__ p, const float* __restrict__ g,
                                                  float* __restrict__ m, float* __restrict__ v, long long n,
                                                  float w1 , float beta2, float w2 ,
                                                  float bc2_sqrt, float eps, float neg_step) {
    long long i = (long long)blockIdx.x * kThreads + threadIdx.x;
    if (i >= n) return;
    const float gi = g[i];
    float mi = m[i], vi = v[i];
    mi = mi + w1 * (gi - mi);
    vi = vi * beta2 + (w2 * gi) * gi;
    const float denom = sqrtf(vi) / bc2_sqrt + eps;
    p[i] = p[i] + neg_step * (mi / denom);
    m[i] = mi;
    v[i] = vi;
}

constexpr int kAdamMulti = 8;
struct AdamTable {
    float* p[kAdamMulti]; const float* g[kAdamMulti]; float* m[kAdamMulti]; float* v[kAdamMulti];
    long long n[kAdamMulti];
    float neg_step[kAdamMulti], eps[kAdamMulti], bc2_sqrt[kAdamMulti];
    unsigned blk0[kAdamMulti + 1];
    int count;
    float w1, beta2, w2;
};
__global__ void __launch_bounds__(kThreads) k_adam_multi(AdamTable t) {
    int k = 0;
#pragma unroll
    for (int q = 1; q < kAdamMulti; ++q) k += (q < t.count && blockIdx.x >= t.blk0[q]) ? 1 : 0;
    const long long i = (long long)(blockIdx.x - t.blk0[k]) * kThreads + threadIdx.x;
    if (i >= t.n[k]) return;
    float* __restrict__ p = t.p[k]; const float* __restrict__ g = t.g[k]; float* __restrict__ m = t.m[k]; float* __restrict__ v = t.v[k];
    const float gi = g[i];
    float mi = m[i], vi = v[i];
    mi = mi + t.w1 * (gi - mi);
    vi = vi * t.beta2 + (t.w2 * gi) * gi;
    const float denom = sqrtf(vi) / t.bc2_sqrt[k] + t.eps[k];
    p[i] = p[i] + t.neg_step[k] * (mi / denom);
    m[i] = mi;
    v[i] = vi;
}

__global__ void __launch_bounds__(kThreads) k_activate(int N, const float* __restrict__ log_scale, const float* __restrict__ rot,
                                                       const float* __restrict__ logit, float* __restrict__ scale,
                                                       float* __restrict__ rot_n, float* __restrict__ opacity) {
    const int i = blockIdx.x * kThreads + threadIdx.x;
    if (i >= N) return;
#pragma unroll
    for (int c = 0; c < 3; ++c) scale[3 * i + c] = act_exp(log_scale[3 * i + c]);
    const float4 q = *(const float4*)(rot + 4 * i);
    *(float4*)(rot_n + 4 * i) = act_quat(q, act_quat_inv_norm(q));
    opacity[i] = act_sigmoid(logit[i]);
}

__global__ void __launch_bounds__(kThreads) k_activate_bwd(int N, const float* __restrict__ rot, const float* __restrict__ scale,
                                                           const float* __restrict__ rot_n, const float* __restrict__ opacity,
                                                           const float* __restrict__ d_scale, const float* __restrict__ d_rot_n,
                                                           const float* __restrict__ d_opacity, float* __restrict__ d_log_scale,
                                                           float* __restrict__ d_rot, float* __restrict__ d_logit) {
    const int i = blockIdx.x * kThreads + threadIdx.x;
    if (i >= N) return;
#pragma unroll
    for (int c = 0; c < 3; ++c) d_log_scale[3 * i + c] = d_scale[3 * i + c] * scale[3 * i + c];
    const float4 q = *(const float4*)(rot + 4 * i), h = *(const float4*)(rot_n + 4 * i), g = *(const float4*)(d_rot_n + 4 * i);
    *(float4*)(d_rot + 4 * i) = act_quat_bwd(h, g, act_quat_inv_norm(q));
    d_logit[i] = act_sigmoid_bwd(opacity[i], d_opacity[i]);
}

__global__ void __launch_bounds__(kThreads) k_densify_stats(int N, const int* __restrict__ radii, const float* __restrict__ vgrad,
                                                           float* __restrict__ accum, float* __restrict__ denom,
                                                           float* __restrict__ max_radii) {
    const int i = blockIdx.x * kThreads + threadIdx.x;
    if (i >= N) return;
    const int r = radii[i];
    if (r <= 0) return;
    const float gx = vgrad[3 * i], gy = vgrad[3 * i + 1];
    accum[i] += sqrtf(gx * gx + gy * gy);
    denom[i] += 1.0f;
    max_radii[i] = fmaxf(max_radii[i], (float)r);
}

constexpr int kWin = 11, kHalo = 5, kTile = 32, kReg = kTile + 2 * kHalo;
constexpr int kRun = 4, kSpan = kRun + kWin - 1;
constexpr int kLead = 8 - kHalo;
constexpr int kPhotoItems = kReg * (kTile / kRun);
constexpr int kPhotoThreads = 256;
struct SsimWindow { float g[kWin]; };
struct PhotoTile { int c, x0, y0; unsigned id; };
__device__ __forceinline__ PhotoTile photo_tile(int gx, int gy) {
    const unsigned nblk = gridDim.x, bid = blockIdx.x;
    const unsigned q = nblk / 8, r = nblk % 8, xcd = bid % 8, k = bid / 8;
    const unsigned t = (xcd < r ? xcd * (q + 1) : r * (q + 1) + (xcd - r) * q) + k;
    PhotoTile o;
    o.id = t;
    o.c = (int)(t / (unsigned)(gx * gy));
    const unsigned rem = t - (unsigned)o.c * (unsigned)(gx * gy);
    o.y0 = (int)(rem / (unsigned)gx) * kTile;
    o.x0 = (int)(rem % (unsigned)gx) * kTile;
    return o;
}
typedef float f2 __attribute__((ext_vector_type(2)));
__device__ __forceinline__ f2 fma2(f2 a, f2 b, f2 c) { return __builtin_elementwise_fma(a, b, c); }

__device__ __forceinline__ float block_sum_photo(float v, float* red) {
    v = wave_sum(v);
    if ((threadIdx.x & 63) == 0) red[threadIdx.x >> 6] = v;
    __syncthreads();
    float t = (red[0] + red[1]) + (red[2] + red[3]);
    __syncthreads();
    return t;
}

template <bool VEC>
__device__ __forceinline__ void photo_load20(float (&v)[20], const float* __restrict__ plane, int y, int x, int H, int W) {
    const bool row = y >= 0 && y < H;
    const float* src = plane + (size_t)min(max(y, 0), H - 1) * W;
    if constexpr (VEC) {
        float4 t[5];
#pragma unroll
        for (int q = 0; q < 5; ++q) t[q] = *(const float4*)(src + min(max(x + 4 * q, 0), W - 4));
#pragma unroll
        for (int q = 0; q < 5; ++q) {
            const bool in = row && x + 4 * q >= 0 && x + 4 * q < W;
            v[4 * q] = in ? t[q].x : 0.0f; v[4 * q + 1] = in ? t[q].y : 0.0f; v[4 * q + 2] = in ? t[q].z : 0.0f; v[4 * q + 3] = in ? t[q].w : 0.0f;
        }
    } else {
        float t[20];
#pragma unroll
        for (int e = 0; e < 20; ++e) t[e] = src[min(max(x + e, 0), W - 1)];
#pragma unroll
        for (int e = 0; e < 20; ++e) v[e] = (row && x + e >= 0 && x + e < W) ? t[e] : 0.0f;
    }
}

template <bool VEC>
__global__ void __launch_bounds__(kPhotoThreads) k_photo_fwd(const float* __restrict__ img, const float* __restrict__ gt, int H,
                                                   int W, int C, SsimWindow win, float* __restrict__ maps,
                                                   float* __restrict__ partial) {
    __shared__ __attribute__((aligned(16))) f2 hA[kReg][kTile], hB[kReg][kTile];
    __shared__ __attribute__((aligned(16))) float hC[kReg][kTile];
    __shared__ float red[kPhotoThreads / 64];
    const PhotoTile tl_ = photo_tile((W + kTile - 1) / kTile, (H + kTile - 1) / kTile);
    const int c = tl_.c, x0 = tl_.x0, y0 = tl_.y0;
    const size_t plane = (size_t)H * W;
    const float* a = img + c * plane;
    const float* b = gt + c * plane;
    float l1_sum = 0.f;
    for (int i = threadIdx.x; i < kPhotoItems; i += kPhotoThreads) {
        const int ry = i / (kTile / kRun), tx = (i - ry * (kTile / kRun)) * kRun;
        const int y = y0 + ry - kHalo;
        float p[20], q[20];
        photo_load20<VEC>(p, a, y, x0 + tx - 8, H, W);
        photo_load20<VEC>(q, b, y, x0 + tx - 8, H, W);
        f2 pq[kSpan], sq[kSpan];
        float pr[kSpan];
#pragma unroll
        for (int t = 0; t < kSpan; ++t) {
            pq[t] = (f2){p[kLead + t], q[kLead + t]};
            sq[t] = pq[t] * pq[t];
            pr[t] = pq[t].x * pq[t].y;
        }
        f2 mA[kRun], mB[kRun];
        float mC[kRun];
#pragma unroll
        for (int j = 0; j < kRun; ++j) { mA[j] = (f2){0.f, 0.f}; mB[j] = (f2){0.f, 0.f}; mC[j] = 0.f; }
#pragma unroll
        for (int k = 0; k < kWin; ++k) {
            const f2 w2 = (f2){win.g[k], win.g[k]};
#pragma unroll
            for (int j = 0; j < kRun; ++j) {
                mA[j] = fma2(w2, pq[j + k], mA[j]);
                mB[j] = fma2(w2, sq[j + k], mB[j]);
                mC[j] = __builtin_fmaf(win.g[k], pr[j + k], mC[j]);
            }
        }
        *(float4*)&hA[ry][tx] = make_float4(mA[0].x, mA[0].y, mA[1].x, mA[1].y);
        *(float4*)&hA[ry][tx + 2] = make_float4(mA[2].x, mA[2].y, mA[3].x, mA[3].y);
        *(float4*)&hB[ry][tx] = make_float4(mB[0].x, mB[0].y, mB[1].x, mB[1].y);
        *(float4*)&hB[ry][tx + 2] = make_float4(mB[2].x, mB[2].y, mB[3].x, mB[3].y);
        *(float4*)&hC[ry][tx] = make_float4(mC[0], mC[1], mC[2], mC[3]);
        if (ry >= kHalo && ry < kHalo + kTile && y < H) {
#pragma unroll
            for (int j = 0; j < kRun; ++j)
                if (x0 + tx + j < W) l1_sum += fabsf(pq[kHalo + j].x - pq[kHalo + j].y);
        }
    }
    __syncthreads();
    const int tx = threadIdx.x & (kTile - 1), ty = (threadIdx.x >> 5) * kRun;
    const int x = x0 + tx;
    f2 mA[kRun], mB[kRun];
    float mC[kRun];
    {
        f2 vA[kSpan], vB[kSpan];
        float vC[kSpan];
#pragma unroll
        for (int t = 0; t < kSpan; ++t) { vA[t] = hA[ty + t][tx]; vB[t] = hB[ty + t][tx]; vC[t] = hC[ty + t][tx]; }
#pragma unroll
        for (int j = 0; j < kRun; ++j) { mA[j] = (f2){0.f, 0.f}; mB[j] = (f2){0.f, 0.f}; mC[j] = 0.f; }
#pragma unroll
        for (int k = 0; k < kWin; ++k) {
            const f2 w2 = (f2){win.g[k], win.g[k]};
#pragma unroll
            for (int j = 0; j < kRun; ++j) {
                mA[j] = fma2(w2, vA[j + k], mA[j]);
                mB[j] = fma2(w2, vB[j + k], mB[j]);
                mC[j] = __builtin_fmaf(win.g[k], vC[j + k], mC[j]);
            }
        }
    }
    float ssim_sum = 0.f;
    const size_t n = (size_t)C * plane;
#pragma unroll
    for (int j = 0; j < kRun; ++j) {
        const int y = y0 + ty + j;
        if (x < W && y < H) {
            const float mu1 = mA[j].x, mu2 = mA[j].y, e11 = mB[j].x, e22 = mB[j].y, e12 = mC[j];
            const float C1 = 0.01f * 0.01f, C2 = 0.03f * 0.03f;
            const float mu1s = mu1 * mu1, mu2s = mu2 * mu2, mu12 = mu1 * mu2;
            const float sg1 = e11 - mu1s, sg2 = e22 - mu2s, sg12 = e12 - mu12;
            const float A = 2.f * mu12 + C1, B = 2.f * sg12 + C2, Cc = mu1s + mu2s + C1, D = sg1 + sg2 + C2;
            const float invC = __builtin_amdgcn_rcpf(Cc), invD = __builtin_amdgcn_rcpf(D);
            const float inv = invC * invD;
            const float ssim = A * B * inv;
            const float d_sg1 = -ssim * invD;
            const float d_sg12 = 2.f * A * inv;
            const float d_mu1 = (2.f * mu2 * B * Cc - 2.f * mu1 * A * B) * inv * invC
                                - 2.f * mu1 * d_sg1 - mu2 * d_sg12;
            const size_t o = (size_t)c * plane + (size_t)y * W + x;
            maps[o] = d_mu1; maps[n + o] = d_sg1; maps[2 * n + o] = d_sg12;
            ssim_sum += ssim;
        }
    }
    const float ts = block_sum_photo(ssim_sum, red);
    const float tl = block_sum_photo(l1_sum, red);
    if (threadIdx.x == 0) {
        const size_t bid = tl_.id;
        partial[2 * bid] = tl;
        partial[2 * bid + 1] = ts;
    }
}

struct PhotoFinal { const float* partial; long long nblocks; double inv_n; float lam, weight; float* loss; };
__device__ __forceinline__ void photo_final(const PhotoFinal f) {
    static_assert(kPhotoThreads == 256, "photo_final: one sum per thread of a 256-thread block");
    double sl = 0.0, ss = 0.0;
    for (long long i = threadIdx.x; i < f.nblocks; i += 256) { sl += (double)f.partial[2 * i]; ss += (double)f.partial[2 * i + 1]; }
    sl = wave_sum_d(sl); ss = wave_sum_d(ss);
    __shared__ double w1[4], w2[4];
    if ((threadIdx.x & 63) == 0) { w1[threadIdx.x >> 6] = sl; w2[threadIdx.x >> 6] = ss; }
    __syncthreads();
    if (threadIdx.x == 0) {
        const double l1 = ((w1[0] + w1[1]) + (w1[2] + w1[3])) * f.inv_n, ssim = ((w2[0] + w2[1]) + (w2[2] + w2[3])) * f.inv_n;
        f.loss[0] = (float)((double)f.weight * ((1.0 - (double)f.lam) * l1 + (double)f.lam * (1.0 - ssim)));
        f.loss[1] = (float)l1;
        f.loss[2] = (float)ssim;
    }
}
__global__ void __launch_bounds__(256) k_photo_final(PhotoFinal f) { photo_final(f); }

template <bool VEC>
__global__ void __launch_bounds__(kPhotoThreads) k_photo_bwd(const float* __restrict__ img, const float* __restrict__ gt, int H,
                                                   int W, int C, SsimWindow win, const float* __restrict__ maps, float c_l1,
                                                   float c_ssim, const float* __restrict__ go,
                                                   float* __restrict__ grad, PhotoFinal fin) {
    __shared__ __attribute__((aligned(16))) f2 hA[kReg][kTile];
    if (fin.partial && blockIdx.x == 0) photo_final(fin);
    __shared__ __attribute__((aligned(16))) float hC[kReg][kTile];
    const PhotoTile tl_ = photo_tile((W + kTile - 1) / kTile, (H + kTile - 1) / kTile);
    const int c = tl_.c, x0 = tl_.x0, y0 = tl_.y0;
    const size_t plane = (size_t)H * W, n = (size_t)C * plane;
    const float* m0 = maps + c * plane;
    const int vtx = threadIdx.x & (kTile - 1), vty = (threadIdx.x >> 5) * kRun;
    float pv[kRun], qv[kRun];
#pragma unroll
    for (int j = 0; j < kRun; ++j) {
        const size_t o = (size_t)c * plane + (size_t)min(y0 + vty + j, H - 1) * W + min(x0 + vtx, W - 1);
        pv[j] = img[o];
        qv[j] = gt[o];
    }
    for (int i = threadIdx.x; i < kPhotoItems; i += kPhotoThreads) {
        const int ry = i / (kTile / kRun), tx = (i - ry * (kTile / kRun)) * kRun;
        const int y = y0 + ry - kHalo;
        float u0[20], u1[20], u2[20];
        photo_load20<VEC>(u0, m0, y, x0 + tx - 8, H, W);
        photo_load20<VEC>(u1, m0 + n, y, x0 + tx - 8, H, W);
        photo_load20<VEC>(u2, m0 + 2 * n, y, x0 + tx - 8, H, W);
        f2 mA[kRun];
        float mC[kRun];
#pragma unroll
        for (int j = 0; j < kRun; ++j) { mA[j] = (f2){0.f, 0.f}; mC[j] = 0.f; }
#pragma unroll
        for (int k = 0; k < kWin; ++k) {
            const f2 w2 = (f2){win.g[k], win.g[k]};
#pragma unroll
            for (int j = 0; j < kRun; ++j) {
                mA[j] = fma2(w2, (f2){u0[kLead + j + k], u1[kLead + j + k]}, mA[j]);
                mC[j] = __builtin_fmaf(win.g[k], u2[kLead + j + k], mC[j]);
            }
        }
        *(float4*)&hA[ry][tx] = make_float4(mA[0].x, mA[0].y, mA[1].x, mA[1].y);
        *(float4*)&hA[ry][tx + 2] = make_float4(mA[2].x, mA[2].y, mA[3].x, mA[3].y);
        *(float4*)&hC[ry][tx] = make_float4(mC[0], mC[1], mC[2], mC[3]);
    }
    __syncthreads();
    const int tx = vtx, ty = vty;
    const int x = x0 + tx;
    f2 gA[kRun];
    float gC[kRun];
    {
        f2 vA[kSpan];
        float vC[kSpan];
#pragma unroll
        for (int t = 0; t < kSpan; ++t) { vA[t] = hA[ty + t][tx]; vC[t] = hC[ty + t][tx]; }
#pragma unroll
        for (int j = 0; j < kRun; ++j) { gA[j] = (f2){0.f, 0.f}; gC[j] = 0.f; }
#pragma unroll
        for (int k = 0; k < kWin; ++k) {
            const f2 w2 = (f2){win.g[k], win.g[k]};
#pragma unroll
            for (int j = 0; j < kRun; ++j) {
                gA[j] = fma2(w2, vA[j + k], gA[j]);
                gC[j] = __builtin_fmaf(win.g[k], vC[j + k], gC[j]);
            }
        }
    }
    const float up = go ? *go : 1.0f;
#pragma unroll
    for (int j = 0; j < kRun; ++j) {
        const int y = y0 + ty + j;
        if (x >= W || y >= H) continue;
        const size_t o = (size_t)c * plane + (size_t)y * W + x;
        const float p = pv[j], q = qv[j], d = p - q;
        const float sgn = d > 0.0f ? 1.0f : (d < 0.0f ? -1.0f : 0.0f);
        grad[o] = up * (c_l1 * sgn - c_ssim * (gA[j].x + 2.0f * p * gA[j].y + q * gC[j]));
    }
}

int l1_blocks(long long n) {
    long long b = (n / 4 + kThreads * 8 - 1) / (kThreads * 8);
    if (b < 1) b = 1;
    if (b > kMaxBlocks) b = kMaxBlocks;
    return (int)b;
}

}

extern "C" size_t syn3r_l1_loss_workspace_bytes(long long n) { return n > 0 ? (size_t)kMaxBlocks * sizeof(float) : 0; }

extern "C" int syn3r_l1_loss(const float* image, const float* target, long long n, float weight, float* loss,
                             void* ws, size_t ws_bytes, void* stream_) {
    hipStream_t stream = (hipStream_t)stream_;
    SYN3R_REQUIRE(n > 0, "l1_loss: n must be positive");
    SYN3R_REQUIRE(image && target && loss && ws, "l1_loss: null pointer");
    SYN3R_REQUIRE(ws_bytes >= syn3r_l1_loss_workspace_bytes(n), "l1_loss: workspace too small");
    SYN3R_REQUIRE((((uintptr_t)image | (uintptr_t)target) & 15) == 0, "l1_loss: image/target must be 16-byte aligned");
    const int nb = l1_blocks(n);
    SYN3R_LAUNCH(k_l1_partial<false>, dim3(nb), dim3(kThreads), 0, stream, image, target, n, (float*)ws);
    SYN3R_LAUNCH(k_l1_final, dim3(1), dim3(kThreads), 0, stream, (const float*)ws, nb, weight / (float)n, loss);
    SYN3R_LAUNCH_CHECK("l1_loss launch");
    return SYN3R_OK;
}

extern "C" int syn3r_image_mse(const float* image, const float* target, long long n, float* mse, void* ws,
                               size_t ws_bytes, void* stream_) {
    hipStream_t stream = (hipStream_t)stream_;
    SYN3R_REQUIRE(n > 0, "image_mse: n must be positive");
    SYN3R_REQUIRE(image && target && mse && ws, "image_mse: null pointer");
    SYN3R_REQUIRE(ws_bytes >= syn3r_l1_loss_workspace_bytes(n), "image_mse: workspace too small");
    SYN3R_REQUIRE((((uintptr_t)image | (uintptr_t)target) & 15) == 0, "image_mse: image/target must be 16-byte aligned");
    const int nb = l1_blocks(n);
    SYN3R_LAUNCH(k_l1_partial<true>, dim3(nb), dim3(kThreads), 0, stream, image, target, n, (float*)ws);
    SYN3R_LAUNCH(k_l1_final, dim3(1), dim3(kThreads), 0, stream, (const float*)ws, nb, 1.0f / (float)n, mse);
    SYN3R_LAUNCH_CHECK("image_mse launch");
    return SYN3R_OK;
}

extern "C" int syn3r_l1_loss_backward(const float* image, const float* target, long long n, float weight,
                                      const float* grad_loss, float* grad_image, void* stream_) {
    hipStream_t stream = (hipStream_t)stream_;
    SYN3R_REQUIRE(n > 0, "l1_loss_backward: n must be positive");
    SYN3R_REQUIRE(image && target && grad_image, "l1_loss_backward: null pointer");
    SYN3R_REQUIRE((((uintptr_t)image | (uintptr_t)target | (uintptr_t)grad_image) & 15) == 0,
                  "l1_loss_backward: buffers must be 16-byte aligned");
    long long b = (n / 4 + kThreads * 4 - 1) / (kThreads * 4);
    if (b < 1) b = 1;
    if (b > 4 * kMaxBlocks) b = 4 * kMaxBlocks;
    SYN3R_LAUNCH(k_l1_grad, dim3((unsigned)b), dim3(kThreads), 0, stream, image, target, n, weight / (float)n,
                 grad_loss, grad_image);
    SYN3R_LAUNCH_CHECK("l1_loss_backward launch");
    return SYN3R_OK;
}

extern "C" int syn3r_adam_step(float* param, const float* grad, float* exp_avg, float* exp_avg_sq, long long n,
                               float lr, float beta1, float beta2, float eps, int step, void* stream_) {
    hipStream_t stream = (hipStream_t)stream_;
    SYN3R_REQUIRE(n > 0, "adam_step: n must be positive");
    SYN3R_REQUIRE(param && grad && exp_avg && exp_avg_sq, "adam_step: null pointer");
    SYN3R_REQUIRE(step >= 1, "adam_step: step is 1-based");
    SYN3R_REQUIRE(beta1 >= 0.5f && beta1 < 1.0f && beta2 >= 0.0f && beta2 < 1.0f, "adam_step: betas out of range");
    const double bc1 = 1.0 - pow((double)beta1, (double)step);
    const double bc2 = 1.0 - pow((double)beta2, (double)step);
    const float neg_step = (float)(-((double)lr / bc1));
    const float bc2_sqrt = (float)sqrt(bc2);
    long long b = (n + kThreads - 1) / kThreads;
    SYN3R_REQUIRE(b < (1ll << 31), "adam_step: tensor too large");
    SYN3R_LAUNCH(k_adam, dim3((unsigned)b), dim3(kThreads), 0, stream, param, grad, exp_avg, exp_avg_sq, n,
                 (float)(1.0 - (double)beta1), beta2, (float)(1.0 - (double)beta2), bc2_sqrt, eps, neg_step);
    SYN3R_LAUNCH_CHECK("adam_step launch");
    return SYN3R_OK;
}

extern "C" int syn3r_adam_step_multi(int count, float* const* params, const float* const* grads, float* const* exp_avgs,
                                     float* const* exp_avg_sqs, const long long* numels, const float* lrs, float beta1, float beta2,
                                     const float* epss, const int* steps, void* stream_) {
    hipStream_t stream = (hipStream_t)stream_;
    SYN3R_REQUIRE(count >= 1 && count <= kAdamMulti, "adam_step_multi: count=%d must be 1..%d", count, kAdamMulti);
    SYN3R_REQUIRE(params && grads && exp_avgs && exp_avg_sqs && numels && lrs && epss && steps, "adam_step_multi: null table");
    SYN3R_REQUIRE(beta1 >= 0.5f && beta1 < 1.0f && beta2 >= 0.0f && beta2 < 1.0f, "adam_step_multi: betas out of range");
    AdamTable t{};
    t.count = count;
    t.w1 = (float)(1.0 - (double)beta1); t.beta2 = beta2; t.w2 = (float)(1.0 - (double)beta2);
    long long blocks = 0;
    for (int k = 0; k < count; ++k) {
        SYN3R_REQUIRE(params[k] && grads[k] && exp_avgs[k] && exp_avg_sqs[k], "adam_step_multi: null pointer in tensor %d", k);
        SYN3R_REQUIRE(numels[k] > 0 && steps[k] >= 1, "adam_step_multi: tensor %d: n must be positive, step 1-based", k);
        const double bc1 = 1.0 - pow((double)beta1, (double)steps[k]);
        const double bc2 = 1.0 - pow((double)beta2, (double)steps[k]);
        t.p[k] = params[k]; t.g[k] = grads[k]; t.m[k] = exp_avgs[k]; t.v[k] = exp_avg_sqs[k]; t.n[k] = numels[k];
        t.neg_step[k] = (float)(-((double)lrs[k] / bc1)); t.bc2_sqrt[k] = (float)sqrt(bc2); t.eps[k] = epss[k];
        t.blk0[k] = (unsigned)blocks;
        blocks += (numels[k] + kThreads - 1) / kThreads;
        SYN3R_REQUIRE(blocks < (1ll << 31), "adam_step_multi: tensors too large");
    }
    for (int k = count; k <= kAdamMulti; ++k) t.blk0[k] = (unsigned)blocks;
    SYN3R_LAUNCH(k_adam_multi, dim3((unsigned)blocks), dim3(kThreads), 0, stream, t);
    SYN3R_LAUNCH_CHECK("adam_step_multi launch");
    return SYN3R_OK;
}

extern "C" int syn3r_gaussian_activate(int N, const float* log_scales, const float* rotations, const float* opacity_logits,
                                       float* scales, float* rotations_n, float* opacities, void* stream_) {
    SYN3R_REQUIRE(SYN3R_DIM_OK(N), "gaussian_activate: bad N=%d", N);
    SYN3R_REQUIRE(log_scales && rotations && opacity_logits && scales && rotations_n && opacities, "gaussian_activate: null pointer");
    SYN3R_REQUIRE((((uintptr_t)rotations | (uintptr_t)rotations_n) % 16) == 0, "gaussian_activate: quaternions must be 16-byte aligned");
    SYN3R_LAUNCH(k_activate, dim3((unsigned)((N + kThreads - 1) / kThreads)), dim3(kThreads), 0, (hipStream_t)stream_, N, log_scales,
                 rotations, opacity_logits, scales, rotations_n, opacities);
    SYN3R_LAUNCH_CHECK("gaussian_activate launch");
    return SYN3R_OK;
}

extern "C" int syn3r_gaussian_activate_backward(int N, const float* rotations, const float* scales, const float* rotations_n,
                                                const float* opacities, const float* d_scales, const float* d_rotations_n,
                                                const float* d_opacities, float* d_log_scales, float* d_rotations,
                                                float* d_opacity_logits, void* stream_) {
    SYN3R_REQUIRE(SYN3R_DIM_OK(N), "gaussian_activate_backward: bad N=%d", N);
    SYN3R_REQUIRE(rotations && scales && rotations_n && opacities && d_scales && d_rotations_n && d_opacities && d_log_scales &&
                  d_rotations && d_opacity_logits, "gaussian_activate_backward: null pointer");
    SYN3R_REQUIRE((((uintptr_t)rotations | (uintptr_t)rotations_n | (uintptr_t)d_rotations_n | (uintptr_t)d_rotations) % 16) == 0,
                  "gaussian_activate_backward: quaternion tensors must be 16-byte aligned");
    SYN3R_LAUNCH(k_activate_bwd, dim3((unsigned)((N + kThreads - 1) / kThreads)), dim3(kThreads), 0, (hipStream_t)stream_, N, rotations,
                 scales, rotations_n, opacities, d_scales, d_rotations_n, d_opacities, d_log_scales, d_rotations, d_opacity_logits);
    SYN3R_LAUNCH_CHECK("gaussian_activate_backward launch");
    return SYN3R_OK;
}

extern "C" int syn3r_densification_stats(int N, const int* radii, const float* viewspace_grad, float* grad_accum, float* denom,
                                         float* max_radii, void* stream_) {
    SYN3R_REQUIRE(SYN3R_DIM_OK(N), "densification_stats: bad N=%d", N);
    SYN3R_REQUIRE(radii && viewspace_grad && grad_accum && denom && max_radii, "densification_stats: null pointer");
    SYN3R_LAUNCH(k_densify_stats, dim3((unsigned)((N + kThreads - 1) / kThreads)), dim3(kThreads), 0, (hipStream_t)stream_, N, radii,
                 viewspace_grad, grad_accum, denom, max_radii);
    SYN3R_LAUNCH_CHECK("densification_stats launch");
    return SYN3R_OK;
}

static SsimWindow make_window() {
    SsimWindow w;
    double g[kWin], sum = 0.0;
    for (int i = 0; i < kWin; ++i) { g[i] = exp(-(double)((i - kWin / 2) * (i - kWin / 2)) / (2.0 * 1.5 * 1.5)); sum += g[i]; }
    for (int i = 0; i < kWin; ++i) w.g[i] = (float)(g[i] / sum);
    return w;
}

extern "C" size_t syn3r_photo_loss_workspace_bytes(int C, int H, int W) {
    if (C <= 0 || C > 65535 || !SYN3R_SIDE_OK(H) || !SYN3R_SIDE_OK(W)) return 0;
    const size_t n = (size_t)C * H * W;
    const size_t blocks = (size_t)C * ((H + kTile - 1) / kTile) * ((W + kTile - 1) / kTile);
    return 3 * n * sizeof(float) + ((2 * blocks * sizeof(float) + 255) / 256) * 256;
}

static int photo_forward(const char* who, const float* image, const float* target, int C, int H, int W, float lambda_dssim,
                         float weight, float* loss3, void* ws, size_t ws_bytes, hipStream_t stream, bool final_launch, PhotoFinal* fin) {
    SYN3R_REQUIRE(C > 0 && C <= 65535 && SYN3R_SIDE_OK(H) && SYN3R_SIDE_OK(W), "%s: bad sizes C=%d H=%d W=%d", who, C, H, W);
    SYN3R_REQUIRE(image && target && loss3 && ws, "%s: null pointer", who);
    SYN3R_REQUIRE(lambda_dssim >= 0.0f && lambda_dssim <= 1.0f, "%s: lambda_dssim must be in [0, 1]", who);
    SYN3R_REQUIRE(ws_bytes >= syn3r_photo_loss_workspace_bytes(C, H, W), "%s: workspace too small", who);
    const size_t n = (size_t)C * H * W;
    float* maps = (float*)ws;
    float* partial = maps + 3 * n;
    const long long tiles = (long long)((W + kTile - 1) / kTile) * ((H + kTile - 1) / kTile) * C;
    SYN3R_REQUIRE(tiles < (1ll << 31), "%s: %lld tiles exceed the grid limit", who, tiles);
    const dim3 grid((unsigned)tiles);
    const bool vec = W % 4 == 0 && (((uintptr_t)image | (uintptr_t)target) & 15) == 0;
    if (vec) SYN3R_LAUNCH(k_photo_fwd<true>, grid, dim3(kPhotoThreads), 0, stream, image, target, H, W, C, make_window(), maps, partial);
    else SYN3R_LAUNCH(k_photo_fwd<false>, grid, dim3(kPhotoThreads), 0, stream, image, target, H, W, C, make_window(), maps, partial);
    const PhotoFinal f{partial, (long long)grid.x, 1.0 / (double)n, lambda_dssim, weight, loss3};
    if (final_launch) SYN3R_LAUNCH(k_photo_final, dim3(1), dim3(256), 0, stream, f);
    if (fin) *fin = f;
    return SYN3R_OK;
}

static int photo_backward(const char* who, const float* image, const float* target, int C, int H, int W, float lambda_dssim,
                          float weight, const float* grad_loss, const void* ws, float* grad_image, hipStream_t stream, PhotoFinal fin) {
    SYN3R_REQUIRE(C > 0 && C <= 65535 && SYN3R_SIDE_OK(H) && SYN3R_SIDE_OK(W), "%s: bad sizes", who);
    SYN3R_REQUIRE(image && target && ws && grad_image, "%s: null pointer", who);
    const double n = (double)C * H * W;
    const long long tiles = (long long)((W + kTile - 1) / kTile) * ((H + kTile - 1) / kTile) * C;
    SYN3R_REQUIRE(tiles < (1ll << 31), "%s: %lld tiles exceed the grid limit", who, tiles);
    const dim3 grid((unsigned)tiles);
    const bool vec = W % 4 == 0 && ((uintptr_t)ws & 15) == 0;
    const float c_l1 = (float)((double)weight * (1.0 - (double)lambda_dssim) / n), c_ssim = (float)((double)weight * (double)lambda_dssim / n);
    if (vec) SYN3R_LAUNCH(k_photo_bwd<true>, grid, dim3(kPhotoThreads), 0, stream, image, target, H, W, C, make_window(), (const float*)ws,
                          c_l1, c_ssim, grad_loss, grad_image, fin);
    else SYN3R_LAUNCH(k_photo_bwd<false>, grid, dim3(kPhotoThreads), 0, stream, image, target, H, W, C, make_window(), (const float*)ws,
                      c_l1, c_ssim, grad_loss, grad_image, fin);
    return SYN3R_OK;
}

extern "C" int syn3r_photo_loss(const float* image, const float* target, int C, int H, int W, float lambda_dssim,
                                float weight, float* loss3, void* ws, size_t ws_bytes, void* stream_) {
    const int rc = photo_forward("photo_loss", image, target, C, H, W, lambda_dssim, weight, loss3, ws, ws_bytes, (hipStream_t)stream_,
                                 true, nullptr);
    if (rc) return rc;
    SYN3R_LAUNCH_CHECK("photo_loss launch");
    return SYN3R_OK;
}

extern "C" int syn3r_photo_loss_backward(const float* image, const float* target, int C, int H, int W,
                                         float lambda_dssim, float weight, const float* grad_loss, const void* ws,
                                         float* grad_image, void* stream_) {
    const int rc = photo_backward("photo_loss_backward", image, target, C, H, W, lambda_dssim, weight, grad_loss, ws, grad_image,
                                  (hipStream_t)stream_, PhotoFinal{});
    if (rc) return rc;
    SYN3R_LAUNCH_CHECK("photo_loss_backward launch");
    return SYN3R_OK;
}

extern "C" int syn3r_photo_loss_step(const float* image, const float* target, int C, int H, int W, float lambda_dssim,
                                     float weight, const float* grad_loss, float* loss3, float* grad_image, void* ws,
                                     size_t ws_bytes, void* stream_) {
    PhotoFinal fin{};
    int rc = photo_forward("photo_loss_step", image, target, C, H, W, lambda_dssim, weight, loss3, ws, ws_bytes, (hipStream_t)stream_,
                           false, &fin);
    if (rc) return rc;
    rc = photo_backward("photo_loss_step", image, target, C, H, W, lambda_dssim, weight, grad_loss, ws, grad_image,
                        (hipStream_t)stream_, fin);
    if (rc) return rc;
    SYN3R_LAUNCH_CHECK("photo_loss_step launch");
    return SYN3R_OK;
}
```

syn3r_amd/gs/train_ops.py:

```python
from __future__ import annotations

from typing import Iterable, List, Optional

import torch

from .. import _lib as L


def _l1_forward(image: torch.Tensor, target: torch.Tensor, weight: float):
    L.require_gpu(image, target)
    if image.shape != target.shape or image.dtype != torch.float32 or target.dtype != torch.float32:
        raise ValueError("l1_loss: image and target must be float32 tensors of the same shape")
    image, target = image.contiguous(), target.contiguous()
    lib = L.load()
    n = image.numel()
    loss = torch.empty((), dtype=torch.float32, device=image.device)
    ws = L.workspace(image.device, lib.syn3r_l1_loss_workspace_bytes(n), "l1")
    L.check(lib.syn3r_l1_loss(L.ptr(image), L.ptr(target), n, float(weight), L.ptr(loss), L.ptr(ws), ws.numel(),
                              L.stream_ptr(image.device)), "l1_loss")
    return loss, image, target


def _l1_backward(image: torch.Tensor, target: torch.Tensor, weight: float, grad_loss):
    go = grad_loss.to(torch.float32).contiguous() if grad_loss is not None else None
    grad = torch.empty_like(image)
    L.check(L.load().syn3r_l1_loss_backward(L.ptr(image), L.ptr(target), image.numel(), float(weight), L.ptr(go),
                                            L.ptr(grad), L.stream_ptr(image.device)), "l1_loss_backward")
    return grad


class _L1Loss(torch.autograd.Function):
    @staticmethod
    def forward(ctx, image: torch.Tensor, target: torch.Tensor, weight: float):
        loss, image, target = _l1_forward(image, target, weight)
        ctx.save_for_backward(image, target)
        ctx.weight = float(weight)
        return loss

    @staticmethod
    def backward(ctx, grad_loss: torch.Tensor):
        L.join_active_trace()
        image, target = ctx.saved_tensors
        return _l1_backward(image, target, ctx.weight, grad_loss), None, None


def l1_loss_step(image: torch.Tensor, target: torch.Tensor, weight: float = 1.0, grad_loss: torch.Tensor = None):
    loss, image, target = _l1_forward(image.detach(), target.detach(), weight)
    return loss, _l1_backward(image, target, weight, grad_loss)


def l1_loss(image: torch.Tensor, target: torch.Tensor, weight: float = 1.0) -> torch.Tensor:
    return _L1Loss.apply(image, target, weight)


class _PhotoLoss(torch.autograd.Function):
    @staticmethod
    def forward(ctx, image: torch.Tensor, target: torch.Tensor, lambda_dssim: float, weight: float):
        L.require_gpu(image, target)
        if image.shape != target.shape or image.dim() != 3 or image.dtype != torch.float32 or target.dtype != torch.float32:
            raise ValueError("photometric_loss: image and target must be float32 [C,H,W] tensors of the same shape")
        image, target = image.contiguous(), target.contiguous()
        lib = L.load()
        C_, H_, W_ = image.shape
        ws = torch.empty(lib.syn3r_photo_loss_workspace_bytes(C_, H_, W_), dtype=torch.uint8, device=image.device)
        out = torch.empty(3, dtype=torch.float32, device=image.device)
        L.check(lib.syn3r_photo_loss(L.ptr(image), L.ptr(target), C_, H_, W_, float(lambda_dssim), float(weight),
                                     L.ptr(out), L.ptr(ws), ws.numel(), L.stream_ptr(image.device)), "photo_loss")
        ctx.save_for_backward(image, target, ws)
        ctx.args = (float(lambda_dssim), float(weight))
        ctx.mark_non_differentiable(out)
        ctx.parts = out
        return out[0].clone(), out

    @staticmethod
    def backward(ctx, grad_loss: torch.Tensor, _grad_parts):
        L.join_active_trace()
        image, target, ws = ctx.saved_tensors
        lam, weight = ctx.args
        C_, H_, W_ = image.shape
        go = grad_loss.to(torch.float32).contiguous()
        grad = torch.empty_like(image)
        L.check(L.load().syn3r_photo_loss_backward(L.ptr(image), L.ptr(target), C_, H_, W_, lam, weight, L.ptr(go),
                                                   L.ptr(ws), L.ptr(grad), L.stream_ptr(image.device)),
                "photo_loss_backward")
        return grad, None, None, None


def photometric_loss(image: torch.Tensor, target: torch.Tensor, lambda_dssim: float = 0.2, weight: float = 1.0,
                     return_parts: bool = False):
    loss, parts = _PhotoLoss.apply(image, target, lambda_dssim, weight)
    return (loss, parts) if return_parts else loss


def photometric_loss_step(image: torch.Tensor, target: torch.Tensor, lambda_dssim: float = 0.2, weight: float = 1.0,
                          grad_loss: torch.Tensor = None):
    dev = L.require_gpu(image, target)
    if image.shape != target.shape or image.dim() != 3 or image.dtype != torch.float32 or target.dtype != torch.float32:
        raise ValueError("photometric_loss_step: image and target must be float32 [C,H,W] tensors of the same shape")
    image, target = image.detach().contiguous(), target.detach().contiguous()
    lib = L.load()
    C_, H_, W_ = image.shape
    ws = L.workspace(dev, lib.syn3r_photo_loss_workspace_bytes(C_, H_, W_), "photo_step")
    parts = torch.empty(3, dtype=torch.float32, device=dev)
    grad = torch.empty_like(image)
    go = grad_loss.to(torch.float32).contiguous() if grad_loss is not None else None
    L.check(lib.syn3r_photo_loss_step(L.ptr(image), L.ptr(target), C_, H_, W_, float(lambda_dssim), float(weight), L.ptr(go),
                                      L.ptr(parts), L.ptr(grad), L.ptr(ws), ws.numel(), L.stream_ptr(dev)), "photo_loss_step")
    return parts[0], parts, grad


_DCORR_MODES = {"min": 0, "A": 1, "B": 2}


def _dcorr_args(who: str, depth: torch.Tensor, prior: torch.Tensor, mode: str):
    L.require_gpu(depth, prior)
    if depth.dtype != torch.float32 or prior.dtype != torch.float32:
        raise ValueError(f"{who}: depth and prior must be float32")
    hw = lambda t: tuple(t.shape[1:]) if t.dim() == 3 and t.shape[0] == 1 else (tuple(t.shape) if t.dim() == 2 else None)
    if hw(depth) is None or hw(prior) is None or hw(depth) != hw(prior):
        raise ValueError(f"{who}: depth [1,H,W] or [H,W] and prior [H,W] or [1,H,W] of the same H, W; got "
                         f"{tuple(depth.shape)} and {tuple(prior.shape)}")
    if mode not in _DCORR_MODES:
        raise ValueError(f"{who}: mode must be one of {sorted(_DCORR_MODES)}, got {mode!r}")
    return depth.detach().contiguous(), prior.detach().contiguous(), _DCORR_MODES[mode]


class _DepthCorrLoss(torch.autograd.Function):
    @staticmethod
    def forward(ctx, depth: torch.Tensor, prior: torch.Tensor, weight: float, offset: float, mode: str):
        d, p, m = _dcorr_args("depth_correlation_loss", depth, prior, mode)
        lib = L.load()
        n = d.numel()
        ws = torch.empty(max(lib.syn3r_depth_corr_loss_workspace_bytes(n), 256), dtype=torch.uint8, device=d.device)
        parts = torch.empty(4, dtype=torch.float32, device=d.device)
        L.check(lib.syn3r_depth_corr_loss(L.ptr(d), L.ptr(p), n, float(weight), float(offset), m, L.ptr(parts), L.ptr(ws),
                                          ws.numel(), L.stream_ptr(d.device)), "depth_corr_loss")
        ctx.save_for_backward(d, p, ws)
        ctx.args = (float(weight), float(offset), m, depth.shape)
        ctx.mark_non_differentiable(parts)
        return parts[0].clone(), parts

    @staticmethod
    def backward(ctx, grad_loss: torch.Tensor, _grad_parts):
        L.join_active_trace()
        d, p, ws = ctx.saved_tensors
        weight, offset, m, shape = ctx.args
        go = grad_loss.to(torch.float32).contiguous()
        grad = torch.empty_like(d)
        L.check(L.load().syn3r_depth_corr_loss_backward(L.ptr(d), L.ptr(p), d.numel(), weight, offset, m, L.ptr(go), L.ptr(ws),
                                                        ws.numel(), L.ptr(grad), L.stream_ptr(d.device)), "depth_corr_loss_backward")
        return grad.reshape(shape), None, None, None, None


def depth_correlation_loss(depth: torch.Tensor, prior: torch.Tensor, weight: float = 1.0, offset: float = 200.0, mode: str = "min",
                           return_parts: bool = False):
    loss, parts = _DepthCorrLoss.apply(depth, prior, weight, offset, mode)
    return (loss, parts) if return_parts else loss


def depth_correlation_loss_step(depth: torch.Tensor, prior: torch.Tensor, weight: float = 1.0, offset: float = 200.0,
                                mode: str = "min", grad_loss: torch.Tensor = None, return_parts: bool = False):
    d, p, m = _dcorr_args("depth_correlation_loss_step", depth, prior, mode)
    dev = d.device
    lib = L.load()
    n = d.numel()
    ws = L.workspace(dev, lib.syn3r_depth_corr_loss_workspace_bytes(n), "dcorr_step")
    parts = torch.empty(4, dtype=torch.float32, device=dev)
    grad = torch.empty_like(d)
    go = grad_loss.to(torch.float32).contiguous() if grad_loss is not None else None
    L.check(lib.syn3r_depth_corr_loss_step(L.ptr(d), L.ptr(p), n, float(weight), float(offset), m, L.ptr(go), L.ptr(parts),
                                           L.ptr(grad), L.ptr(ws), ws.numel(), L.stream_ptr(dev)), "depth_corr_loss_step")
    return (parts[0], grad, parts) if return_parts else (parts[0], grad)


def image_metrics(image: torch.Tensor, target: torch.Tensor) -> torch.Tensor:
    L.require_gpu(image, target)
    image, target = image.detach().contiguous(), target.detach().contiguous()
    if image.shape != target.shape or image.dim() != 3 or image.dtype != torch.float32:
        raise ValueError("image_metrics: float32 [C,H,W] images of the same shape")
    lib = L.load()
    n = image.numel()
    mse = torch.empty((), dtype=torch.float32, device=image.device)
    ws = L.workspace(image.device, lib.syn3r_l1_loss_workspace_bytes(n), "l1")
    L.check(lib.syn3r_image_mse(L.ptr(image), L.ptr(target), n, L.ptr(mse), L.ptr(ws), ws.numel(),
                                L.stream_ptr(image.device)), "image_mse")
    _, parts = _PhotoLoss.apply(image, target, 1.0, 1.0)
    psnr = -10.0 * torch.log10(mse.clamp_min(1e-12))
    return torch.stack([psnr, parts[2]])


def knn3_mean_dist2(points: torch.Tensor) -> torch.Tensor:
    L.require_gpu(points)
    if points.dim() != 2 or points.shape[1] != 3 or points.dtype != torch.float32:
        raise ValueError("knn3_mean_dist2: points must be a float32 [n,3] tensor")
    pts = points.detach().contiguous()
    n = pts.shape[0]
    lib = L.load()
    out = torch.empty(n, dtype=torch.float32, device=pts.device)
    ws = L.workspace(pts.device, lib.syn3r_knn3_workspace_bytes(n), "knn3")
    L.check(lib.syn3r_knn3_mean_dist2(L.ptr(pts), n, L.ptr(out), L.ptr(ws), ws.numel(), L.stream_ptr(pts.device)), "knn3_mean_dist2")
    return out


def _cloud_arg(who: str, points: torch.Tensor) -> torch.Tensor:
    L.require_gpu(points)
    if points.dim() != 2 or points.shape[1] != 3 or points.dtype != torch.float32:
        raise ValueError(f"{who}: points must be a float32 [n,3] tensor")
    return points.detach().contiguous()


def knn3_graph(points: torch.Tensor):
    pts = _cloud_arg("knn3_graph", points)
    n = pts.shape[0]
    lib = L.load()
    dist2 = torch.empty((n, 3), dtype=torch.float32, device=pts.device)
    index = torch.empty((n, 3), dtype=torch.int32, device=pts.device)
    ws = L.workspace(pts.device, lib.syn3r_knn3_graph_workspace_bytes(n), "knn3")
    L.check(lib.syn3r_knn3_graph(L.ptr(pts), n, L.ptr(dist2), L.ptr(index), L.ptr(ws), ws.numel(), L.stream_ptr(pts.device)), "knn3_graph")
    return dist2, index


def proximity_unpool(xyz: torch.Tensor, log_scales: torch.Tensor, opacity_logits: torch.Tensor, confidence: torch.Tensor,
                     score_thresh: float, log_scale_thresh: float) -> dict:
    pts = _cloud_arg("proximity_unpool", xyz)
    L.require_gpu(pts, log_scales, opacity_logits, confidence)
    n, dev = pts.shape[0], pts.device
    f32 = lambda t: t.detach().contiguous()
    ls, op, conf = f32(log_scales), f32(opacity_logits).reshape(-1), f32(confidence).reshape(-1)
    if ls.shape != (n, 3) or op.shape != (n,) or conf.shape != (n,) or any(t.dtype != torch.float32 for t in (ls, op, conf)):
        raise ValueError(f"proximity_unpool: float32 log_scales [n,3], opacity_logits [n] and confidence [n] for n={n} points; got "
                         f"{tuple(log_scales.shape)}, {tuple(opacity_logits.shape)}, {tuple(confidence.shape)}")
    lib = L.load()
    dist2, index = knn3_graph(pts)
    count = torch.empty(1, dtype=torch.int32, device=dev)
    ws = L.workspace(dev, lib.syn3r_gaussian_unpool_workspace_bytes(n), "unpool")
    L.check(lib.syn3r_gaussian_unpool_count(L.ptr(dist2), L.ptr(ls), n, float(score_thresh), float(log_scale_thresh), L.ptr(count),
                                            L.ptr(ws), ws.numel(), L.stream_ptr(dev)), "gaussian_unpool_count")
    S = int(count.item())
    M = 3 * S
    new = lambda *shape: torch.empty(shape, dtype=torch.float32, device=dev)
    out = {"xyz": new(M, 3), "scaling": new(M, 3), "opacity": new(M), "rotation": new(M, 4), "confidence": new(M),
           "count": M, "sources": S}
    if S > 0:
        L.check(lib.syn3r_gaussian_unpool_emit(L.ptr(pts), L.ptr(ls), L.ptr(op), L.ptr(conf), L.ptr(index), n, S, M, L.ptr(out["xyz"]),
                                               L.ptr(out["scaling"]), L.ptr(out["opacity"]), L.ptr(out["rotation"]),
                                               L.ptr(out["confidence"]), L.ptr(ws), ws.numel(), L.stream_ptr(dev)),
                "gaussian_unpool_emit")
    return out


class FusedAdam:

    def __init__(self, param_groups: Iterable[dict], lr: float = 1e-3, betas=(0.9, 0.999), eps: float = 1e-8):
        self.param_groups: List[dict] = []
        for g in param_groups:
            g = dict(g)
            g["params"] = list(g["params"])
            g.setdefault("lr", lr)
            g.setdefault("betas", betas)
            g.setdefault("eps", eps)
            self.param_groups.append(g)
        self.state: dict = {}

    def zero_grad(self, set_to_none: bool = True):
        for g in self.param_groups:
            for p in g["params"]:
                if set_to_none:
                    p.grad = None
                elif p.grad is not None:
                    p.grad.zero_()

    @torch.no_grad()
    def step(self):
        import ctypes as C
        lib = L.load()
        batches: dict = {}
        for g in self.param_groups:
            b1, b2 = g["betas"]
            for p in g["params"]:
                if p.grad is None:
                    continue
                L.require_gpu(p)
                if p.dtype != torch.float32 or not p.is_contiguous():
                    raise ValueError("FusedAdam: parameters must be contiguous float32")
                st = self.state.get(p)
                if st is None:
                    st = self.state[p] = {"step": 0, "exp_avg": torch.zeros_like(p), "exp_avg_sq": torch.zeros_like(p)}
                st["step"] += 1
                grad = p.grad.contiguous()
                batches.setdefault((float(b1), float(b2), p.device), []).append((p, grad, st, float(g["lr"]), float(g["eps"])))
        for (b1, b2, dev), items in batches.items():
            for k0 in range(0, len(items), 8):
                chunk = items[k0:k0 + 8]
                n = len(chunk)
                ptrs = lambda sel: (C.c_void_p * n)(*[sel(it) for it in chunk])
                rc = lib.syn3r_adam_step_multi(
                    n, ptrs(lambda it: it[0].data_ptr()), ptrs(lambda it: it[1].data_ptr()), ptrs(lambda it: it[2]["exp_avg"].data_ptr()),
                    ptrs(lambda it: it[2]["exp_avg_sq"].data_ptr()), (C.c_longlong * n)(*[it[0].numel() for it in chunk]),
                    (C.c_float * n)(*[it[3] for it in chunk]), b1, b2, (C.c_float * n)(*[it[4] for it in chunk]),
                    (C.c_int * n)(*[int(it[2]["step"]) for it in chunk]), L.stream_ptr(dev))
                L.check(rc, "adam_step_multi")
```

syn3r_amd/raster/__init__.py:

```python
from __future__ import annotations

import ctypes as C
from typing import NamedTuple, Optional

import torch

from .. import _lib as L


class GaussianRasterizationSettings(NamedTuple):
    image_height: int
    image_width: int
    tanfovx: float
    tanfovy: float
    bg: torch.Tensor
    scale_modifier: float
    viewmatrix: torch.Tensor
    projmatrix: torch.Tensor
    sh_degree: int
    campos: torch.Tensor
    prefiltered: bool = False
    debug: bool = False


_host_cache: dict = {}


def _host_floats(m: torch.Tensor):
    import weakref
    key = id(m)
    hit = _host_cache.get(key)
    if hit is not None and hit[0]() is m and hit[1] == m._version:
        return hit[2]
    if len(_host_cache) > 1024:
        for k in [k for k, v in _host_cache.items() if v[0]() is None]:
            del _host_cache[k]
    vals = L.host_f32(m.detach().to("cpu", torch.float32).reshape(-1).tolist())
    _host_cache[key] = (weakref.ref(m), m._version, vals)
    return vals


def _host16(m: torch.Tensor):
    return _host_floats(m)


_HEADROOM = 2.0
_pair_mode = "sync"
_capacity: dict = {}
_pending: dict = {}


def set_pair_count_mode(mode: str) -> None:
    global _pair_mode
    if mode not in ("sync", "async"):
        raise ValueError("pair-count mode must be 'sync' or 'async'")
    _pair_mode = mode


def get_pair_count_mode() -> str:
    return _pair_mode


def _check_pending(key, wait: bool) -> int:
    queue = _pending.get(key)
    truncated = 0
    while queue:
        evt, host, cap = queue[0]
        if not (wait or len(queue) > 8 or evt.query()):
            break
        evt.synchronize()
        queue.pop(0)
        P, overflow = int(host[0]), int(host[1])
        _capacity[key] = max(_capacity.get(key, 0), int(P * _HEADROOM) + 4096)
        if overflow or P > cap:
            truncated += 1
    if queue is not None and not queue:
        del _pending[key]
    return truncated


def _overflow_error(n: int) -> "L.Syn3rError":
    return L.Syn3rError(f"rasteriser (async pair-count mode): {n} previous render(s) needed more (Gaussian, tile) pairs than "
                        "the binning buffer held; those images are invalid - capacity has been raised, render again")


def flush_pair_checks() -> int:
    total = 0
    for key in list(_pending):
        total += _check_pending(key, wait=True)
    if total:
        err = _overflow_error(total)
        err.truncated = total
        raise err
    return 0


def carry_capacity(old_key, new_key, scale: float) -> None:
    cap = _capacity.pop(old_key, None)
    _pending.pop(old_key, None)
    if cap is not None:
        _capacity[new_key] = max(_capacity.get(new_key, 0), int(cap * max(scale, 1.0)) + 4096)


def capacity_key(dev: torch.device, N: int, H: int, W: int):
    return (dev.index, int(N), int(H), int(W))


class RasterState:
    __slots__ = ("settings", "host", "P", "M", "plist", "has_conf", "opacity_shape", "raw_params", "tensors")


def rasterize_forward(means3D, shs, opacities, scales, rotations, confidence, settings: GaussianRasterizationSettings,
                      raw_params: bool = False):
    s = settings
    dev = L.require_gpu(means3D, shs, opacities, scales, rotations)
    lib = L.load()
    N = means3D.shape[0]
    H, W = int(s.image_height), int(s.image_width)
    if N == 0:
        raise ValueError("rasteriser needs at least one Gaussian")
    M = shs.shape[1]
    f32 = lambda t: t.detach().to(torch.float32).contiguous()
    m3, sh, op, sc, ro = f32(means3D), f32(shs), f32(opacities).reshape(-1), f32(scales), f32(rotations)
    cf = f32(confidence).reshape(-1) if confidence is not None else None
    if m3.shape != (N, 3) or sc.shape != (N, 3) or ro.shape != (N, 4) or op.shape != (N,) or sh.shape != (N, M, 3):
        raise ValueError("rasteriser: inconsistent Gaussian tensor shapes")
    view, proj = _host16(s.viewmatrix), _host16(s.projmatrix)
    campos = _host_floats(s.campos)
    bg = _host_floats(s.bg)
    stream = L.stream_ptr(dev)

    geom = torch.empty(lib.syn3r_raster_geom_bytes(N), dtype=torch.uint8, device=dev)
    image = torch.empty(lib.syn3r_raster_image_bytes(H, W), dtype=torch.uint8, device=dev)
    radii = torch.empty(N, dtype=torch.int32, device=dev)
    key = (dev.index, N, H, W)
    use_async = _pair_mode == "async" and not s.debug
    if use_async:
        n_trunc = _check_pending(key, wait=False)
        if n_trunc:
            err = _overflow_error(n_trunc)
            err.truncated = n_trunc
            raise err
    use_async = use_async and key in _capacity
    P = C.c_longlong(0)
    preprocess = lib.syn3r_raster_preprocess_raw if raw_params else lib.syn3r_raster_preprocess
    rc = preprocess(N, int(s.sh_degree), M, L.ptr(m3), L.ptr(sc), L.ptr(ro), L.ptr(op), L.ptr(sh),
                    L.ptr(cf), float(s.scale_modifier), view, proj, campos, float(s.tanfovx),
                    float(s.tanfovy), H, W, L.ptr(radii), L.ptr(geom), geom.numel(),
                    None if use_async else C.byref(P), stream)
    L.check(rc, "syn3r_raster_preprocess")
    if use_async:
        P = _capacity[key]
    else:
        P = int(P.value)
        _capacity[key] = max(_capacity.get(key, 0), int(P * _HEADROOM) + 4096)
    binning = torch.empty(lib.syn3r_raster_binning_bytes(P), dtype=torch.uint8, device=dev)
    color = torch.empty((3, H, W), dtype=torch.float32, device=dev)
    depth = torch.empty((1, H, W), dtype=torch.float32, device=dev)
    alpha = torch.empty((1, H, W), dtype=torch.float32, device=dev)
    plist = C.c_void_p(0)
    rc = lib.syn3r_raster_render(N, H, W, bg, L.ptr(radii), L.ptr(geom), geom.numel(), L.ptr(binning),
                                 binning.numel(), L.ptr(image), image.numel(), P, L.ptr(color), L.ptr(depth),
                                 L.ptr(alpha), C.byref(plist), stream)
    L.check(rc, "syn3r_raster_render")
    if use_async:
        host = torch.empty(2, dtype=torch.int32, pin_memory=True)
        host.copy_(geom[:8].view(torch.int32), non_blocking=True)
        evt = torch.cuda.Event()
        evt.record(torch.cuda.current_stream(dev))
        _pending.setdefault(key, []).append((evt, host, P))
    if s.debug:
        tiles = ((W + 15) // 16) * ((H + 15) // 16)
        a256 = lambda x: (x + 255) & ~255
        off = plist.value - binning.data_ptr() if P > 0 else 0
        _Rasterize.debug_state = dict(
            num_rendered=P,
            point_list=binning[off:off + 4 * P].view(torch.int32).clone(),
            ranges=image[:tiles * 8].view(torch.int32).reshape(tiles, 2).clone(),
            n_contrib=image[a256(tiles * 8):a256(tiles * 8) + 4 * H * W].view(torch.int32).reshape(H, W).clone(),
            depths=geom[256:256 + 4 * N].view(torch.float32).clone(),
        )
    st = RasterState()
    st.settings, st.host, st.P, st.M, st.plist = s, (view, proj, campos, bg), P, M, plist.value
    st.has_conf, st.opacity_shape, st.raw_params = cf is not None, opacities.shape, bool(raw_params)
    st.tensors = (m3, sc, ro, op, sh, cf if cf is not None else torch.empty(0, device=dev), radii, geom, binning, image)
    return color, radii, depth, alpha, st


def rasterize_backward(st: RasterState, g_color, g_depth=None, g_alpha=None):
    m3, sc, ro, op, sh, cf, radii, geom, binning, image = st.tensors
    s = st.settings
    lib = L.load()
    dev = m3.device
    N, M = m3.shape[0], st.M
    H, W = int(s.image_height), int(s.image_width)
    view, proj, campos, bg = st.host
    gc = g_color.detach().to(torch.float32).contiguous() if g_color is not None else torch.zeros((3, H, W), device=dev)
    gd = g_depth.detach().to(torch.float32).contiguous() if g_depth is not None else None
    ga = g_alpha.detach().to(torch.float32).contiguous() if g_alpha is not None else None
    new = lambda *shape: torch.empty(shape, dtype=torch.float32, device=dev)
    d_m3, d_sc, d_ro, d_op, d_sh, d_m2 = new(N, 3), new(N, 3), new(N, 4), new(N), new(N, M, 3), new(N, 3)
    d_cf = new(N) if st.has_conf else None
    ws = L.workspace(dev, lib.syn3r_raster_backward_workspace_bytes(N), "raster_bwd")
    backward = lib.syn3r_raster_backward_raw if st.raw_params else lib.syn3r_raster_backward
    rc = backward(
        N, int(s.sh_degree), M, st.P, L.ptr(m3), L.ptr(sc), L.ptr(ro), L.ptr(op), L.ptr(sh),
        L.ptr(cf) if st.has_conf else None, float(s.scale_modifier), view, proj, campos, float(s.tanfovx),
        float(s.tanfovy), H, W, bg, L.ptr(radii), L.ptr(geom), geom.numel(), st.plist, L.ptr(image), image.numel(),
        L.ptr(gc), L.ptr(gd), L.ptr(ga), L.ptr(d_m3), L.ptr(d_sc), L.ptr(d_ro), L.ptr(d_op), L.ptr(d_sh),
        L.ptr(d_m2), L.ptr(d_cf), L.ptr(ws), ws.numel(), L.stream_ptr(dev))
    L.check(rc, "syn3r_raster_backward")
    return d_m3, d_m2, d_sh, d_op.reshape(st.opacity_shape), d_sc, d_ro, d_cf


class _Rasterize(torch.autograd.Function):
    debug_state = None

    @staticmethod
    def forward(ctx, means3D, means2D, shs, opacities, scales, rotations, confidence, settings):
        color, radii, depth, alpha, st = rasterize_forward(means3D, shs, opacities, scales, rotations, confidence, settings)
        ctx.save_for_backward(*st.tensors)
        st.tensors = None
        ctx.state = st
        ctx.mark_non_differentiable(radii)
        ctx.set_materialize_grads(False)
        return color, radii, depth, alpha

    @staticmethod
    def backward(ctx, g_color, g_radii, g_depth, g_alpha):
        L.join_active_trace()
        st = ctx.state
        st.tensors = ctx.saved_tensors
        try:
            d_m3, d_m2, d_sh, d_op, d_sc, d_ro, d_cf = rasterize_backward(st, g_color, g_depth, g_alpha)
        finally:
            st.tensors = None
        return d_m3, d_m2, d_sh, d_op, d_sc, d_ro, d_cf, None


class GaussianRasterizer(torch.nn.Module):
    def __init__(self, raster_settings: GaussianRasterizationSettings):
        super().__init__()
        self.raster_settings = raster_settings

    def forward(self, means3D, means2D, opacities, shs=None, colors_precomp=None, scales=None, rotations=None,
                cov3D_precomp=None, confidence: Optional[torch.Tensor] = None):
        if (shs is None) == (colors_precomp is None):
            raise Exception("Please provide excatly one of either SHs or precomputed colors!")
        if colors_precomp is not None or cov3D_precomp is not None:
            raise NotImplementedError("precomputed colours / covariances are not used by the SYN3R hot path")
        if scales is None or rotations is None:
            raise Exception("Please provide scales and rotations")
        return _Rasterize.apply(means3D, means2D, shs, opacities, scales, rotations, confidence, self.raster_settings)


def sort_pairs(keys: torch.Tensor, vals: torch.Tensor, nbits: int = 64):
    dev = L.require_gpu(keys, vals)
    lib = L.load()
    n = keys.numel()
    k = keys.contiguous().clone()
    v = vals.contiguous().clone()
    kt, vt = torch.empty_like(k), torch.empty_like(v)
    ws = L.workspace(dev, lib.syn3r_sort_pairs_workspace_bytes(n), "sort")
    flag = C.c_int(0)
    rc = lib.syn3r_sort_pairs(L.ptr(k), L.ptr(v), L.ptr(kt), L.ptr(vt), n, nbits, L.ptr(ws), ws.numel(), C.byref(flag),
                              L.stream_ptr(dev))
    L.check(rc, "syn3r_sort_pairs")
    return (kt, vt) if flag.value else (k, v)
```

Measured before the change: 416.3 iters/s.

## Compact L1 sign map, fuse loss step, move tile histogram into super-sort

The L1 loss forward now writes a 2-bit-per-element sign map, and backward reads only that map instead of re-reading the image and target. A fused l1_loss_step computes the loss and the gradient in one pass. In the binning path, per-tile totals and the tile-size histogram are computed inside super_sort, so the single-block k_tile_offsets kernel does less work and fills tile_order in one pass. This adds an extra buffer, changes the workspace layout, and switches the workspace allocation from empty to zeros.

After: 411.9 iters/s. 1.0% lower.

```diff
diff --git a/include/syn3r_hip.h b/include/syn3r_hip.h
--- a/include/syn3r_hip.h
+++ b/include/syn3r_hip.h
@@ -201,8 +201,14 @@
 size_t syn3r_l1_loss_workspace_bytes(long long n);
 int syn3r_l1_loss(const float* image, const float* target, long long n, float weight, float* loss, void* ws,
                   size_t ws_bytes, void* stream);
+int syn3r_l1_loss_signs(const float* image, const float* target, long long n, float weight, float* loss,
+                        unsigned char* signs, void* ws, size_t ws_bytes, void* stream);
 int syn3r_l1_loss_backward(const float* image, const float* target, long long n, float weight,
                            const float* grad_loss, float* grad_image, void* stream);
+int syn3r_l1_loss_backward_signs(const unsigned char* signs, long long n, float weight, const float* grad_loss,
+                                 float* grad_image, void* stream);
+int syn3r_l1_loss_step(const float* image, const float* target, long long n, float weight, const float* grad_loss,
+                       float* loss, float* grad_image, void* ws, size_t ws_bytes, void* stream);
 
 int syn3r_image_mse(const float* image, const float* target, long long n, float* mse, void* ws, size_t ws_bytes,
                     void* stream);
diff --git a/syn3r_amd/_lib.py b/syn3r_amd/_lib.py
--- a/syn3r_amd/_lib.py
+++ b/syn3r_amd/_lib.py
@@ -96,7 +96,10 @@
     "syn3r_time_conv_out": (c_i, [c_p, c_ll, c_p, c_p, c_p, c_i, c_i, c_ll, c_p]),
     "syn3r_l1_loss_workspace_bytes": (c_sz, [c_ll]),
     "syn3r_l1_loss": (c_i, [c_p, c_p, c_ll, c_f, c_p, c_p, c_sz, c_p]),
+    "syn3r_l1_loss_signs": (c_i, [c_p, c_p, c_ll, c_f, c_p, c_p, c_p, c_sz, c_p]),
     "syn3r_l1_loss_backward": (c_i, [c_p, c_p, c_ll, c_f, c_p, c_p, c_p]),
+    "syn3r_l1_loss_backward_signs": (c_i, [c_p, c_ll, c_f, c_p, c_p, c_p]),
+    "syn3r_l1_loss_step": (c_i, [c_p, c_p, c_ll, c_f, c_p, c_p, c_p, c_p, c_sz, c_p]),
     "syn3r_image_mse": (c_i, [c_p, c_p, c_ll, c_p, c_p, c_sz, c_p]),
     "syn3r_photo_loss_workspace_bytes": (c_sz, [c_i, c_i, c_i]),
     "syn3r_photo_loss": (c_i, [c_p, c_p, c_i, c_i, c_i, c_f, c_f, c_p, c_p, c_sz, c_p]),
@@ -232,7 +235,7 @@
     key = (dev.index, torch.cuda.current_stream(dev).cuda_stream, tag)
     buf = _ws_cache.get(key)
     if buf is None or buf.numel() < nbytes:
-        buf = torch.empty(max(int(nbytes), 256), dtype=torch.uint8, device=dev)
+        buf = torch.zeros(max(int(nbytes), 256), dtype=torch.uint8, device=dev)
         _ws_cache[key] = buf
     return buf
 
diff --git a/syn3r_amd/csrc/raster_bin.hip b/syn3r_amd/csrc/raster_bin.hip
--- a/syn3r_amd/csrc/raster_bin.hip
+++ b/syn3r_amd/csrc/raster_bin.hip
@@ -144,8 +144,10 @@
 
 __global__ void __launch_bounds__(kBinThreads) k_super_count(int N, const float* __restrict__ means2D, const int* __restrict__ radii,
                                                              int gx, int gy, int ss, int sgx, int nsuper, int rounds, int nchunks,
-                                                             unsigned* __restrict__ counters, unsigned* __restrict__ header) {
+                                                             unsigned* __restrict__ counters, unsigned* __restrict__ header,
+                                                             unsigned* __restrict__ tile_hist) {
     __shared__ unsigned tot[kMaxSuper];
+    if (blockIdx.x == 0 && threadIdx.x < 256) tile_hist[threadIdx.x] = 0u;
     for (int s = threadIdx.x; s < nsuper; s += kBinThreads) tot[s] = 0u;
     __syncthreads();
     int pairs = 0;
@@ -294,9 +296,12 @@
 }
 
 __device__ __forceinline__ void super_tile_counts(int sx, int sy, int ss, int gx, int gy, unsigned n, const unsigned short* srect_b,
-                                                  unsigned* __restrict__ tcount) {
+                                                  unsigned* __restrict__ tcount, unsigned* __restrict__ ttotal, unsigned* __restrict__ thist) {
     const int lane = threadIdx.x & 63, wv = threadIdx.x >> 6, side = 1 << ss;
     const unsigned len = (n + 3u) / 4u;
+    __shared__ unsigned tot[64];
+    if (threadIdx.x < 64) tot[threadIdx.x] = 0u;
+    __syncthreads();
     for (int it = wv; it < side * side * 4; it += kSuperSortThreads / 64) {
         const int ti = it >> 2, q = it & 3;
         const int rx = ti & (side - 1), ry = ti >> ss;
@@ -313,20 +318,34 @@
         }
 #pragma unroll
         for (int o = 32; o > 0; o >>= 1) cnt += __shfl_xor(cnt, o, 64);
-        if (lane == 0) tcount[4 * ((size_t)ty * gx + tx) + q] = cnt;
+        if (lane == 0) {
+            tcount[4 * ((size_t)ty * gx + tx) + q] = cnt;
+            if (cnt) atomicAdd(&tot[ti], cnt);
+        }
+    }
+    __syncthreads();
+    if ((int)threadIdx.x < side * side) {
+        const int ti = threadIdx.x;
+        const int tx = (sx << ss) + (ti & (side - 1)), ty = (sy << ss) + (ti >> ss);
+        if (tx < gx && ty < gy) {
+            const unsigned c = tot[ti];
+            ttotal[(size_t)ty * gx + tx] = c;
+            atomicAdd(&thist[255u - min(255u, c >> 5)], 1u);
+        }
     }
 }
 
 __global__ void __launch_bounds__(kSuperSortThreads, 8) k_super_sort(int N, const float* __restrict__ means2D, const int* __restrict__ radii,
                                                                   int gx, int gy, int ss, int sgx, const unsigned* __restrict__ sstart, unsigned cap,
                                                                   unsigned long long* __restrict__ skeys, unsigned* __restrict__ sid,
-                                                                  unsigned short* __restrict__ srect, unsigned* __restrict__ tcount) {
+                                                                  unsigned short* __restrict__ srect, unsigned* __restrict__ tcount,
+                                                                  unsigned* __restrict__ ttotal, unsigned* __restrict__ thist) {
     extern __shared__ __attribute__((aligned(16))) unsigned long long sk[];
     const int s_ = blockIdx.x, sx = s_ % sgx, sy = s_ / sgx;
     unsigned b, e;
     super_range(s_, sstart, cap, b, e);
     const int n = (int)(e - b);
-    if (n == 0) { super_tile_counts(sx, sy, ss, gx, gy, 0u, srect, tcount); return; }
+    if (n == 0) { super_tile_counts(sx, sy, ss, gx, gy, 0u, srect, tcount, ttotal, thist); return; }
     unsigned long long* gk = skeys + b;
     const unsigned long long INF = ~0ull;
     int m = 1;
@@ -391,7 +410,7 @@
             if (i < n) sr[i] = clip[u];
         }
         __syncthreads();
-        super_tile_counts(sx, sy, ss, gx, gy, (unsigned)n, sr, tcount);
+        super_tile_counts(sx, sy, ss, gx, gy, (unsigned)n, sr, tcount, ttotal, thist);
         return;
     }
     for (int i = threadIdx.x; i < n; i += kSuperSortThreads) {
@@ -401,53 +420,53 @@
         srect[b + i] = clip_rect(q, sx, sy, ss);
     }
     __syncthreads();
-    super_tile_counts(sx, sy, ss, gx, gy, (unsigned)n, srect + b, tcount);
-}
-
-__global__ void __launch_bounds__(kOffThreads) k_tile_offsets(int tiles, const unsigned* __restrict__ tcount, unsigned cap,
-                                                              uint2* __restrict__ ranges, unsigned* __restrict__ header,
+    super_tile_counts(sx, sy, ss, gx, gy, (unsigned)n, srect + b, tcount, ttotal, thist);
+}
+
+__global__ void __launch_bounds__(kOffThreads) k_tile_offsets(int tiles, const unsigned* __restrict__ ttotal, const unsigned* __restrict__ thist,
+                                                              unsigned cap, uint2* __restrict__ ranges, unsigned* __restrict__ header,
                                                               unsigned* __restrict__ tile_order) {
     __shared__ unsigned smem[kOffThreads / 64 + 1];
     __shared__ unsigned bh[256];
-    if (tile_order) { for (int k = threadIdx.x; k < 256; k += kOffThreads) bh[k] = 0u; __syncthreads(); }
+    if (tile_order) {
+        if (threadIdx.x < 64) {
+            const int l = threadIdx.x;
+            const uint4 h4 = ((const uint4*)thist)[l];
+            const unsigned c[4] = {h4.x, h4.y, h4.z, h4.w};
+            unsigned ex = wave_scan_incl((c[0] + c[1]) + (c[2] + c[3])) - ((c[0] + c[1]) + (c[2] + c[3]));
+#pragma unroll
+            for (int k = 0; k < 4; ++k) { bh[4 * l + k] = ex; ex += c[k]; }
+        }
+        __syncthreads();
+    }
     constexpr int PER = 8;
     unsigned carry = 0;
     for (int start = 0; start < tiles; start += kOffThreads * PER) {
         const int t0 = start + threadIdx.x * PER;
         unsigned c[PER], sum = 0;
-#pragma unroll
-        for (int k = 0; k < PER; ++k) {
-            c[k] = 0u;
-            if (t0 + k < tiles) { const uint4 q4 = ((const uint4*)tcount)[t0 + k]; c[k] = (q4.x + q4.y) + (q4.z + q4.w); }
-            sum += c[k];
-        }
+        if (t0 + PER <= tiles) {
+            const uint4 a4 = ((const uint4*)(ttotal + t0))[0], b4 = ((const uint4*)(ttotal + t0))[1];
+            c[0] = a4.x; c[1] = a4.y; c[2] = a4.z; c[3] = a4.w; c[4] = b4.x; c[5] = b4.y; c[6] = b4.z; c[7] = b4.w;
+        } else {
+#pragma unroll
+            for (int k = 0; k < PER; ++k) c[k] = t0 + k < tiles ? ttotal[t0 + k] : 0u;
+        }
+#pragma unroll
+        for (int k = 0; k < PER; ++k) sum += c[k];
         unsigned total;
         unsigned ex = block_exclusive_scan<kOffThreads / 64>(sum, smem, total) + carry;
 #pragma unroll
         for (int k = 0; k < PER; ++k) {
-            if (t0 + k < tiles) ranges[t0 + k] = c[k] ? make_uint2(min(ex, cap), min(ex + c[k], cap)) : make_uint2(0u, 0u);
-            if (tile_order && t0 + k < tiles) atomicAdd(&bh[255u - min(255u, c[k] >> 5)], 1u);
+            if (t0 + k < tiles) {
+                ranges[t0 + k] = c[k] ? make_uint2(min(ex, cap), min(ex + c[k], cap)) : make_uint2(0u, 0u);
+                if (tile_order) {
+                    const unsigned o = atomicAdd(&bh[255u - min(255u, c[k] >> 5)], 1u);
+                    if (o < (unsigned)tiles) tile_order[o] = (unsigned)(t0 + k);
+                }
+            }
             ex += c[k];
         }
         carry += total;
-    }
-    if (tile_order) {
-        __syncthreads();
-        if (threadIdx.x < 64) {
-            const int l = threadIdx.x;
-            unsigned c[4], sum = 0;
-#pragma unroll
-            for (int k = 0; k < 4; ++k) { c[k] = bh[4 * l + k]; sum += c[k]; }
-            unsigned ex = wave_scan_incl(sum) - sum;
-#pragma unroll
-            for (int k = 0; k < 4; ++k) { bh[4 * l + k] = ex; ex += c[k]; }
-        }
-        __syncthreads();
-        for (int t = threadIdx.x; t < tiles; t += kOffThreads) {
-            const uint4 q4 = ((const uint4*)tcount)[t];
-            const unsigned c = (q4.x + q4.y) + (q4.z + q4.w);
-            tile_order[atomicAdd(&bh[255u - min(255u, c >> 5)], 1u)] = (unsigned)t;
-        }
     }
     if (threadIdx.x == 0) {
         const bool over = carry > cap || header[2] > cap;
@@ -532,14 +551,14 @@
         static DevOnce once;
         if (int rc = set_max_lds(once, (const void*)k_super_sort, kSortLds * 8, "hipFuncSetAttribute(super_sort)")) return rc;
         SYN3R_LAUNCH(k_super_count, dim3(bp.nchunks), dim3(kBinThreads), 0, stream, N, (const float*)g.means2D, radii, gx, gy, bp.ss, bp.sgx,
-                     bp.nsuper, bp.rounds, bp.nchunks, counters, g.header);
+                     bp.nsuper, bp.rounds, bp.nchunks, counters, g.header, im.tile_hist);
         SYN3R_LAUNCH(k_super_append, dim3(bp.nchunks), dim3(kBinThreads), 0, stream, N, (const float*)g.depths, (const float*)g.means2D, radii,
                      gx, gy, bp.ss, bp.sgx, bp.nsuper, bp.rounds, bp.nchunks, (const unsigned*)counters, sstart, (unsigned)P, skeys, g.header);
         SYN3R_LAUNCH(k_super_sort, dim3(bp.nsuper), dim3(kSuperSortThreads), kSortLds * 8, stream, N, (const float*)g.means2D, radii, gx, gy,
-                     bp.ss, bp.sgx, (const unsigned*)sstart, (unsigned)P, skeys, sid, srect, im.tile_counts);
+                     bp.ss, bp.sgx, (const unsigned*)sstart, (unsigned)P, skeys, sid, srect, im.tile_counts, im.tile_totals, im.tile_hist);
         if (raster_tiles_ordered(N, gx, gy)) tile_order = im.tile_order;
-        SYN3R_LAUNCH(k_tile_offsets, dim3(1), dim3(kOffThreads), 0, stream, (int)tiles, (const unsigned*)im.tile_counts, (unsigned)P,
-                     im.ranges, g.header, tile_order);
+        SYN3R_LAUNCH(k_tile_offsets, dim3(1), dim3(kOffThreads), 0, stream, (int)tiles, (const unsigned*)im.tile_totals, (const unsigned*)im.tile_hist,
+                     (unsigned)P, im.ranges, g.header, tile_order);
         SYN3R_LAUNCH(k_tile_write, dim3((unsigned)tiles), dim3(256), 0, stream, gx, (int)tiles, bp.ss, bp.sgx,
                      (const unsigned*)sstart, (unsigned)P, (const unsigned*)sid, (const unsigned short*)srect,
                      (const uint2*)im.ranges, (const unsigned*)im.tile_counts, point_list);
diff --git a/syn3r_amd/csrc/raster_common.h b/syn3r_amd/csrc/raster_common.h
--- a/syn3r_amd/csrc/raster_common.h
+++ b/syn3r_amd/csrc/raster_common.h
@@ -56,8 +56,10 @@
     unsigned* n_contrib;
     float* final_T;
     unsigned* tile_counts;
+    unsigned* tile_totals;
+    unsigned* tile_hist;
+    unsigned* tile_order;
     unsigned* bin_counters;
-    unsigned* tile_order;
 };
 
 struct BinningState {
diff --git a/syn3r_amd/csrc/raster_fwd.hip b/syn3r_amd/csrc/raster_fwd.hip
--- a/syn3r_amd/csrc/raster_fwd.hip
+++ b/syn3r_amd/csrc/raster_fwd.hip
@@ -50,7 +50,8 @@
 size_t image_bytes(int H, int W) {
     size_t tiles = (size_t)((W + kTileX - 1) / kTileX) * ((H + kTileY - 1) / kTileY);
     size_t px = (size_t)H * W;
-    return align256(tiles * 8) + align256(px * 4) + align256(px * 4) + align256(tiles * 16) + align256((kBinCounters + kMaxSuperSlots) * 4) + align256(tiles * 4);
+    return align256(tiles * 8) + align256(px * 4) + align256(px * 4) + align256(tiles * 16) + align256(tiles * 4) + align256(256 * 4) + align256(tiles * 4) +
+           align256((kBinCounters + kMaxSuperSlots) * 4);
 }
 
 ImageState carve_image(void* buf, int H, int W) {
@@ -62,8 +63,10 @@
     s.n_contrib = (unsigned*)p; p += align256(px * 4);
     s.final_T = (float*)p; p += align256(px * 4);
     s.tile_counts = (unsigned*)p; p += align256(tiles * 16);
-    s.bin_counters = (unsigned*)p; p += align256((kBinCounters + kMaxSuperSlots) * 4);
-    s.tile_order = (unsigned*)p;
+    s.tile_totals = (unsigned*)p; p += align256(tiles * 4);
+    s.tile_hist = (unsigned*)p; p += align256(256 * 4);
+    s.tile_order = (unsigned*)p; p += align256(tiles * 4);
+    s.bin_counters = (unsigned*)p;
     return s;
 }
 
diff --git a/syn3r_amd/csrc/train.hip b/syn3r_amd/csrc/train.hip
--- a/syn3r_amd/csrc/train.hip
+++ b/syn3r_amd/csrc/train.hip
@@ -10,37 +10,67 @@
 template <bool SQ>
 __device__ __forceinline__ float dist_term(float d) { return SQ ? d * d : fabsf(d); }
 
-template <bool SQ>
+__device__ __forceinline__ unsigned sign_code(float d) { return d > 0.0f ? 1u : (d < 0.0f ? 2u : 0u); }
+__device__ __forceinline__ float sign_value(unsigned code, float g) { return code == 1u ? g : (code == 2u ? -g : 0.0f); }
+
+struct L1Extra { unsigned char* signs; float* grad; float gscale; const float* go; };
+
+template <bool SQ, bool MAP, bool GRAD>
 __global__ void __launch_bounds__(kThreads) k_l1_partial(const float* __restrict__ a, const float* __restrict__ b,
-                                                        long long n, float* __restrict__ partial) {
+                                                        long long n, float* partial, unsigned* ticket, float scale,
+                                                        float* __restrict__ loss, L1Extra ex) {
     float s = 0.0f;
+    float g = 0.0f;
+    if constexpr (GRAD) g = ex.gscale * (ex.go ? *ex.go : 1.0f);
     const long long n4 = n >> 2;
     const float4* a4 = (const float4*)a;
     const float4* b4 = (const float4*)b;
     for (long long i = (long long)blockIdx.x * kThreads + threadIdx.x; i < n4; i += (long long)gridDim.x * kThreads) {
         float4 x = a4[i], y = b4[i];
-        s += (dist_term<SQ>(x.x - y.x) + dist_term<SQ>(x.y - y.y)) + (dist_term<SQ>(x.z - y.z) + dist_term<SQ>(x.w - y.w));
+        const float d0 = x.x - y.x, d1 = x.y - y.y, d2 = x.z - y.z, d3 = x.w - y.w;
+        s += (dist_term<SQ>(d0) + dist_term<SQ>(d1)) + (dist_term<SQ>(d2) + dist_term<SQ>(d3));
+        if constexpr (MAP) ex.signs[i] = (unsigned char)(sign_code(d0) | (sign_code(d1) << 2) | (sign_code(d2) << 4) | (sign_code(d3) << 6));
+        if constexpr (GRAD)
+            ((float4*)ex.grad)[i] = make_float4(sign_value(sign_code(d0), g), sign_value(sign_code(d1), g),
+                                                sign_value(sign_code(d2), g), sign_value(sign_code(d3), g));
     }
     if (blockIdx.x == 0) {
         long long i = (n4 << 2) + threadIdx.x;
-        if (i < n) s += dist_term<SQ>(a[i] - b[i]);
+        if (i < n) {
+            const float d = a[i] - b[i];
+            s += dist_term<SQ>(d);
+            if constexpr (GRAD) ex.grad[i] = sign_value(sign_code(d), g);
+        }
+        if constexpr (MAP) {
+            if (threadIdx.x == 0 && (n4 << 2) < n) {
+                unsigned byte = 0u;
+                for (long long j = n4 << 2; j < n; ++j) byte |= sign_code(a[j] - b[j]) << (2 * (int)(j - (n4 << 2)));
+                ex.signs[n4] = (unsigned char)byte;
+            }
+        }
     }
     s = wave_sum(s);
     __shared__ float ws[kThreads / 64];
+    __shared__ unsigned drawn;
     if ((threadIdx.x & 63) == 0) ws[threadIdx.x >> 6] = s;
     __syncthreads();
-    if (threadIdx.x == 0) partial[blockIdx.x] = (ws[0] + ws[1]) + (ws[2] + ws[3]);
-}
-
-__global__ void __launch_bounds__(kThreads) k_l1_final(const float* __restrict__ partial, int nblocks, float scale,
-                                                      float* __restrict__ loss) {
-    double s = 0.0;
-    for (int i = threadIdx.x; i < nblocks; i += kThreads) s += (double)partial[i];
-    s = wave_sum_d(s);
-    __shared__ double ws[kThreads / 64];
-    if ((threadIdx.x & 63) == 0) ws[threadIdx.x >> 6] = s;
-    __syncthreads();
-    if (threadIdx.x == 0) *loss = (float)(((ws[0] + ws[1]) + (ws[2] + ws[3])) * (double)scale);
+    const unsigned nb = gridDim.x;
+    if (threadIdx.x == 0) {
+        __hip_atomic_store(&partial[blockIdx.x], (ws[0] + ws[1]) + (ws[2] + ws[3]), __ATOMIC_RELAXED, __HIP_MEMORY_SCOPE_AGENT);
+        __threadfence();
+        drawn = atomicInc(ticket, nb - 1u);
+    }
+    __syncthreads();
+    if (drawn != nb - 1u) return;
+    __threadfence();
+    double t = 0.0;
+    for (unsigned i = threadIdx.x; i < nb; i += kThreads)
+        t += (double)__hip_atomic_load(&partial[i], __ATOMIC_RELAXED, __HIP_MEMORY_SCOPE_AGENT);
+    t = wave_sum_d(t);
+    __shared__ double wd[kThreads / 64];
+    if ((threadIdx.x & 63) == 0) wd[threadIdx.x >> 6] = t;
+    __syncthreads();
+    if (threadIdx.x == 0) *loss = (float)(((wd[0] + wd[1]) + (wd[2] + wd[3])) * (double)scale);
 }
 
 __global__ void __launch_bounds__(kThreads) k_l1_grad(const float* __restrict__ a, const float* __restrict__ b,
@@ -59,6 +89,21 @@
     if (blockIdx.x == 0) {
         long long i = (n4 << 2) + threadIdx.x;
         if (i < n) grad[i] = sgn(a[i] - b[i]);
+    }
+}
+
+__global__ void __launch_bounds__(kThreads) k_l1_grad_signs(const unsigned char* __restrict__ signs, long long n, float scale,
+                                                           const float* __restrict__ go, float* __restrict__ grad) {
+    const float g = scale * (go ? *go : 1.0f);
+    const long long n4 = n >> 2;
+    float4* g4 = (float4*)grad;
+    for (long long i = (long long)blockIdx.x * kThreads + threadIdx.x; i < n4; i += (long long)gridDim.x * kThreads) {
+        const unsigned c = signs[i];
+        g4[i] = make_float4(sign_value(c & 3u, g), sign_value((c >> 2) & 3u, g), sign_value((c >> 4) & 3u, g), sign_value(c >> 6, g));
+    }
+    if (blockIdx.x == 0) {
+        long long i = (n4 << 2) + threadIdx.x;
+        if (i < n) grad[i] = sign_value(((unsigned)signs[n4] >> (2 * threadIdx.x)) & 3u, g);
     }
 }
 
@@ -408,33 +453,61 @@
 
 }
 
-extern "C" size_t syn3r_l1_loss_workspace_bytes(long long n) { return n > 0 ? (size_t)kMaxBlocks * sizeof(float) : 0; }
+extern "C" size_t syn3r_l1_loss_workspace_bytes(long long n) { return n > 0 ? (size_t)kMaxBlocks * sizeof(float) + 16 : 0; }
+
+template <bool SQ, bool MAP, bool GRAD>
+static int l1_launch(const char* who, const float* image, const float* target, long long n, float scale, float* out, void* ws,
+                     size_t ws_bytes, hipStream_t stream, L1Extra ex) {
+    SYN3R_REQUIRE(n > 0, "%s: n must be positive", who);
+    SYN3R_REQUIRE(image && target && out && ws, "%s: null pointer", who);
+    SYN3R_REQUIRE(ws_bytes >= syn3r_l1_loss_workspace_bytes(n), "%s: workspace too small", who);
+    SYN3R_REQUIRE((((uintptr_t)image | (uintptr_t)target) & 15) == 0, "%s: image/target must be 16-byte aligned", who);
+    const int nb = l1_blocks(n);
+    SYN3R_LAUNCH_NAMED(SQ ? "k_l1_partial<true>" : "k_l1_partial<false>", (k_l1_partial<SQ, MAP, GRAD>), dim3(nb), dim3(kThreads), 0, stream, image, target, n, (float*)ws,
+                       (unsigned*)((float*)ws + kMaxBlocks), scale, out, ex);
+    SYN3R_LAUNCH_CHECK(who);
+    return SYN3R_OK;
+}
+
+extern "C" int syn3r_l1_loss_signs(const float* image, const float* target, long long n, float weight, float* loss,
+                                   unsigned char* signs, void* ws, size_t ws_bytes, void* stream_) {
+    const L1Extra ex{signs, nullptr, 0.0f, nullptr};
+    if (signs) return l1_launch<false, true, false>("l1_loss", image, target, n, weight / (float)n, loss, ws, ws_bytes, (hipStream_t)stream_, ex);
+    return l1_launch<false, false, false>("l1_loss", image, target, n, weight / (float)n, loss, ws, ws_bytes, (hipStream_t)stream_, ex);
+}
 
 extern "C" int syn3r_l1_loss(const float* image, const float* target, long long n, float weight, float* loss,
                              void* ws, size_t ws_bytes, void* stream_) {
-    hipStream_t stream = (hipStream_t)stream_;
-    SYN3R_REQUIRE(n > 0, "l1_loss: n must be positive");
-    SYN3R_REQUIRE(image && target && loss && ws, "l1_loss: null pointer");
-    SYN3R_REQUIRE(ws_bytes >= syn3r_l1_loss_workspace_bytes(n), "l1_loss: workspace too small");
-    SYN3R_REQUIRE((((uintptr_t)image | (uintptr_t)target) & 15) == 0, "l1_loss: image/target must be 16-byte aligned");
-    const int nb = l1_blocks(n);
-    SYN3R_LAUNCH(k_l1_partial<false>, dim3(nb), dim3(kThreads), 0, stream, image, target, n, (float*)ws);
-    SYN3R_LAUNCH(k_l1_final, dim3(1), dim3(kThreads), 0, stream, (const float*)ws, nb, weight / (float)n, loss);
-    SYN3R_LAUNCH_CHECK("l1_loss launch");
-    return SYN3R_OK;
+    return syn3r_l1_loss_signs(image, target, n, weight, loss, nullptr, ws, ws_bytes, stream_);
+}
+
+extern "C" int syn3r_l1_loss_step(const float* image, const float* target, long long n, float weight, const float* grad_loss,
+                                  float* loss, float* grad_image, void* ws, size_t ws_bytes, void* stream_) {
+    SYN3R_REQUIRE(grad_image && ((uintptr_t)grad_image & 15) == 0, "l1_loss_step: grad_image must be a 16-byte aligned pointer");
+    const L1Extra ex{nullptr, grad_image, weight / (float)n, grad_loss};
+    return l1_launch<false, false, true>("l1_loss_step", image, target, n, weight / (float)n, loss, ws, ws_bytes, (hipStream_t)stream_, ex);
 }
 
 extern "C" int syn3r_image_mse(const float* image, const float* target, long long n, float* mse, void* ws,
                                size_t ws_bytes, void* stream_) {
+    return l1_launch<true, false, false>("image_mse", image, target, n, 1.0f / (float)n, mse, ws, ws_bytes, (hipStream_t)stream_, L1Extra{});
+}
+
+static unsigned l1_grad_blocks(long long n) {
+    long long b = (n / 4 + kThreads * 4 - 1) / (kThreads * 4);
+    if (b < 1) b = 1;
+    if (b > 4 * kMaxBlocks) b = 4 * kMaxBlocks;
+    return (unsigned)b;
+}
+
+extern "C" int syn3r_l1_loss_backward_signs(const unsigned char* signs, long long n, float weight, const float* grad_loss,
+                                            float* grad_image, void* stream_) {
     hipStream_t stream = (hipStream_t)stream_;
-    SYN3R_REQUIRE(n > 0, "image_mse: n must be positive");
-    SYN3R_REQUIRE(image && target && mse && ws, "image_mse: null pointer");
-    SYN3R_REQUIRE(ws_bytes >= syn3r_l1_loss_workspace_bytes(n), "image_mse: workspace too small");
-    SYN3R_REQUIRE((((uintptr_t)image | (uintptr_t)target) & 15) == 0, "image_mse: image/target must be 16-byte aligned");
-    const int nb = l1_blocks(n);
-    SYN3R_LAUNCH(k_l1_partial<true>, dim3(nb), dim3(kThreads), 0, stream, image, target, n, (float*)ws);
-    SYN3R_LAUNCH(k_l1_final, dim3(1), dim3(kThreads), 0, stream, (const float*)ws, nb, 1.0f / (float)n, mse);
-    SYN3R_LAUNCH_CHECK("image_mse launch");
+    SYN3R_REQUIRE(n > 0, "l1_loss_backward_signs: n must be positive");
+    SYN3R_REQUIRE(signs && grad_image, "l1_loss_backward_signs: null pointer");
+    SYN3R_REQUIRE(((uintptr_t)grad_image & 15) == 0, "l1_loss_backward_signs: grad_image must be 16-byte aligned");
+    SYN3R_LAUNCH(k_l1_grad_signs, dim3(l1_grad_blocks(n)), dim3(kThreads), 0, stream, signs, n, weight / (float)n, grad_loss, grad_image);
+    SYN3R_LAUNCH_CHECK("l1_loss_backward_signs launch");
     return SYN3R_OK;
 }
 
@@ -445,10 +518,7 @@
     SYN3R_REQUIRE(image && target && grad_image, "l1_loss_backward: null pointer");
     SYN3R_REQUIRE((((uintptr_t)image | (uintptr_t)target | (uintptr_t)grad_image) & 15) == 0,
                   "l1_loss_backward: buffers must be 16-byte aligned");
-    long long b = (n / 4 + kThreads * 4 - 1) / (kThreads * 4);
-    if (b < 1) b = 1;
-    if (b > 4 * kMaxBlocks) b = 4 * kMaxBlocks;
-    SYN3R_LAUNCH(k_l1_grad, dim3((unsigned)b), dim3(kThreads), 0, stream, image, target, n, weight / (float)n,
+    SYN3R_LAUNCH(k_l1_grad, dim3(l1_grad_blocks(n)), dim3(kThreads), 0, stream, image, target, n, weight / (float)n,
                  grad_loss, grad_image);
     SYN3R_LAUNCH_CHECK("l1_loss_backward launch");
     return SYN3R_OK;
diff --git a/syn3r_amd/gs/train_ops.py b/syn3r_amd/gs/train_ops.py
--- a/syn3r_amd/gs/train_ops.py
+++ b/syn3r_amd/gs/train_ops.py
@@ -7,46 +7,50 @@
 from .. import _lib as L
 
 
-def _l1_forward(image: torch.Tensor, target: torch.Tensor, weight: float):
+def _l1_args(image: torch.Tensor, target: torch.Tensor):
     L.require_gpu(image, target)
     if image.shape != target.shape or image.dtype != torch.float32 or target.dtype != torch.float32:
         raise ValueError("l1_loss: image and target must be float32 tensors of the same shape")
-    image, target = image.contiguous(), target.contiguous()
-    lib = L.load()
-    n = image.numel()
-    loss = torch.empty((), dtype=torch.float32, device=image.device)
-    ws = L.workspace(image.device, lib.syn3r_l1_loss_workspace_bytes(n), "l1")
-    L.check(lib.syn3r_l1_loss(L.ptr(image), L.ptr(target), n, float(weight), L.ptr(loss), L.ptr(ws), ws.numel(),
-                              L.stream_ptr(image.device)), "l1_loss")
-    return loss, image, target
-
-
-def _l1_backward(image: torch.Tensor, target: torch.Tensor, weight: float, grad_loss):
-    go = grad_loss.to(torch.float32).contiguous() if grad_loss is not None else None
-    grad = torch.empty_like(image)
-    L.check(L.load().syn3r_l1_loss_backward(L.ptr(image), L.ptr(target), image.numel(), float(weight), L.ptr(go),
-                                            L.ptr(grad), L.stream_ptr(image.device)), "l1_loss_backward")
-    return grad
+    return image.contiguous(), target.contiguous()
 
 
 class _L1Loss(torch.autograd.Function):
     @staticmethod
     def forward(ctx, image: torch.Tensor, target: torch.Tensor, weight: float):
-        loss, image, target = _l1_forward(image, target, weight)
-        ctx.save_for_backward(image, target)
-        ctx.weight = float(weight)
+        image, target = _l1_args(image, target)
+        lib = L.load()
+        n, dev = image.numel(), image.device
+        loss = torch.empty((), dtype=torch.float32, device=dev)
+        signs = torch.empty(((n + 3) // 4 + 15) // 16 * 16, dtype=torch.uint8, device=dev)
+        ws = L.workspace(dev, lib.syn3r_l1_loss_workspace_bytes(n), "l1")
+        L.check(lib.syn3r_l1_loss_signs(L.ptr(image), L.ptr(target), n, float(weight), L.ptr(loss), L.ptr(signs), L.ptr(ws),
+                                        ws.numel(), L.stream_ptr(dev)), "l1_loss")
+        ctx.save_for_backward(signs)
+        ctx.weight, ctx.shape = float(weight), image.shape
         return loss
 
     @staticmethod
     def backward(ctx, grad_loss: torch.Tensor):
         L.join_active_trace()
-        image, target = ctx.saved_tensors
-        return _l1_backward(image, target, ctx.weight, grad_loss), None, None
+        signs, = ctx.saved_tensors
+        go = grad_loss.to(torch.float32).contiguous() if grad_loss is not None else None
+        grad = torch.empty(ctx.shape, dtype=torch.float32, device=signs.device)
+        L.check(L.load().syn3r_l1_loss_backward_signs(L.ptr(signs), grad.numel(), ctx.weight, L.ptr(go), L.ptr(grad),
+                                                      L.stream_ptr(signs.device)), "l1_loss_backward")
+        return grad, None, None
 
 
 def l1_loss_step(image: torch.Tensor, target: torch.Tensor, weight: float = 1.0, grad_loss: torch.Tensor = None):
-    loss, image, target = _l1_forward(image.detach(), target.detach(), weight)
-    return loss, _l1_backward(image, target, weight, grad_loss)
+    image, target = _l1_args(image.detach(), target.detach())
+    lib = L.load()
+    n, dev = image.numel(), image.device
+    loss = torch.empty((), dtype=torch.float32, device=dev)
+    grad = torch.empty_like(image)
+    go = grad_loss.to(torch.float32).contiguous() if grad_loss is not None else None
+    ws = L.workspace(dev, lib.syn3r_l1_loss_workspace_bytes(n), "l1")
+    L.check(lib.syn3r_l1_loss_step(L.ptr(image), L.ptr(target), n, float(weight), L.ptr(go), L.ptr(loss), L.ptr(grad), L.ptr(ws),
+                                   ws.numel(), L.stream_ptr(dev)), "l1_loss_step")
+    return loss, grad
 
 
 def l1_loss(image: torch.Tensor, target: torch.Tensor, weight: float = 1.0) -> torch.Tensor:
diff --git a/syn3r_amd/raster/__init__.py b/syn3r_amd/raster/__init__.py
--- a/syn3r_amd/raster/__init__.py
+++ b/syn3r_amd/raster/__init__.py
@@ -173,12 +173,17 @@
         tiles = ((W + 15) // 16) * ((H + 15) // 16)
         a256 = lambda x: (x + 255) & ~255
         off = plist.value - binning.data_ptr() if P > 0 else 0
+        counts_at = a256(tiles * 8) + 2 * a256(4 * H * W)
+        order_at = counts_at + a256(tiles * 16) + a256(tiles * 4) + 1024
         _Rasterize.debug_state = dict(
             num_rendered=P,
             point_list=binning[off:off + 4 * P].view(torch.int32).clone(),
             ranges=image[:tiles * 8].view(torch.int32).reshape(tiles, 2).clone(),
             n_contrib=image[a256(tiles * 8):a256(tiles * 8) + 4 * H * W].view(torch.int32).reshape(H, W).clone(),
             depths=geom[256:256 + 4 * N].view(torch.float32).clone(),
+            header=geom[:16].view(torch.int32).clone(),
+            tile_counts=image[counts_at:counts_at + tiles * 16].view(torch.int32).reshape(tiles, 4).clone(),
+            tile_order=image[order_at:order_at + tiles * 4].view(torch.int32).clone(),
         )
     st = RasterState()
     st.settings, st.host, st.P, st.M, st.plist = s, (view, proj, campos, bg), P, M, plist.value
```
